# AI-ON/Few-Shot-Music-Generation

Measured on AMD Instinct MI355X. Metric: episodes/s (LSTM-baseline train step, synthetic vocab=10k seq_len=128 5-way/5-shot h=512), higher is better.
Workload: dtype f32 (bf16x3-split products, fp32 accumulate)

## Files before the change

### few-shot-music-generation_amd/csrc/api_backward.hip

```cpp
#include "fsmg_model.h"

using namespace fsmg;
using namespace fsmg_host;

namespace fsmg_host {

int dhout_chunk(fsmg_model* h, const Lane& ln, int B, int t0, int t1, OpBatch* defer = nullptr) {
    ScopedTimer tm(h, "gemm_dhout");
    const int64_t r0 = (int64_t)t0 * B, m = (int64_t)(t1 - t0) * B;
    GemmArgs g{};
    g.A = dlogits_buf(h) + (size_t)r0 * h->V1p; g.lda = h->V1p; g.B = h->P + h->off_w; g.ldb = h->V1p;
    g.C = h->dH + (size_t)r0 * h->Hp; g.ldc = h->Hp; g.M = (int)m; g.N = h->Hp; g.K = h->V1p; g.ksplit = 1;
    if (h->fs_call) g.row_scale = h->crow + r0;
    return gemm(h, ln, OP_KC, OP_KC, g, defer);
}

GemmArgs dw_args(fsmg_model* h, int B) {
    GemmArgs g{};
    g.A = h->Hs[h->L - 1] + (size_t)B * h->Hp; g.lda = h->Hp; g.B = dlogits_buf(h); g.ldb = h->V1p;
    g.C = h->G + h->off_w; g.ldc = h->V1p; g.M = h->Hp; g.N = h->V1p; g.K = (int)((int64_t)h->T * B);
    g.colsum = h->G + h->off_d; g.ksplit = 1;
    if (h->fs_call) { g.A = h->Hsc; g.colsum_w = h->crow; }
    return g;
}
int dw_gemm(fsmg_model* h, const Lane& ln, int B, OpBatch* defer = nullptr) {
    ScopedTimer tm(h, "gemm_dw");
    return gemm(h, ln, OP_XC, OP_XC, dw_args(h, B), defer);
}

int bptt_fills(fsmg_model* h, OpBatch& fills, int B, bool xcd, bool rs, bool chain, int rpx) {
    const int T = h->T, Hp = h->Hp, G4 = h->G4;
    GEMMCK(fills.add(h->dC, 0u, (long long)B * Hp));
    if (xcd) {
        GEMMCK(fills.add(h->inboxX, 0xFFFFFFFFu, lstm_xcd_inbox_floats(B, Hp, rpx), h->d_inbox_dirty));
        GEMMCK(fills.add(h->tickets, 0u, (long long)8 * fsmg_model::TICKET_LAUNCHES));
        h->ticket_next = 0;
    } else if (rs) {
        GEMMCK(fills.add(h->inbox, 0xFFFFFFFFu, lstm_bwd_rs_inbox_floats(B, Hp)));
    } else if (chain) {
        const long long Bp16 = (B + 15) / 16 * 16;
        GEMMCK(fills.add(h->dzF_all, 0xFFFFFFFFu, (long long)T * Bp16 * G4));
    }
    return FSMG_OK;
}

int backward(fsmg_model* h, int B, int part) {
    ScopedRange rng_(part == 2 ? "fsmg.backward(2)" : "fsmg.backward");
    const int T = h->T, Hp = h->Hp, G4 = h->G4;
    const int64_t rows = (int64_t)T * B;
    const Lane mainl = main_lane(h);
    hipStream_t s = h->stream;
    const bool ov = use_overlap(h);
    const bool xcd = use_xcd(h, B, true);
    const bool rs = !xcd && h->persist && h->inbox != nullptr && lstm_bwd_rs_supported(B, Hp) && lstm_bwd_rs_inbox_floats(B, Hp) <= h->inbox_floats;
    const bool chain = xcd || rs || (h->persist && h->dzF_all != nullptr && lstm_bwd_chain_supported(B, Hp) &&
                              (int64_t)T * ((B + 15) / 16 * 16) * G4 <= h->dzfa_floats);
    if (!xcd && h->cs_stale) return fail(h, FSMG_ERR_STATE, "internal: backward pass on the column-split kernels with stale fragment copies of K_h (ensure_cs not called)");
    const int nch = ov ? (chain ? h->nchunk_persist : h->nchunk) : 1;
    const Lane auxl = aux_lane(h, false, chain);
    GemmArgs gdw = dw_args(h, B);
    int dw_split = 1;
    if (h->xov_call && (h->xov_parts & 2) && xcd && !ov) dw_split = std::max(1, std::min(std::min(h->xov_dw_split, MAX_SPLIT), gdw.K / 256));
    while (dw_split > 1 && (int64_t)dw_split * gdw.M * gdw.N > h->slab_cap) --dw_split;
    if (dw_split > 1) {
        gdw.C = mainl.slabs; gdw.c_slab = (int64_t)gdw.M * gdw.N; gdw.ksplit = dw_split;
        gdw.colsum = mainl.colsum_slabs; gdw.colsum_slab = gdw.N;
    }
    const bool xov = h->xov_call && (h->xov_parts & 2) && xcd && !ov && dw_split > 1 && xov_fits(gdw);
    const int rpx = xov ? lstm_xcd16_packed_rows(B, Hp) : 0;
    const bool cut = !ov && !xov;
    if (part == 2 && !cut) return FSMG_OK;
    const bool cut_late = cut && h->dp_split == 2 && part != 0;
    bool dx_sq_done = false, top_fills_done = false;
    const bool defer_ok = part == 0 && (cut || xov);
    if (part != 2) h->arena_off = 0;
    h->last_bwd_xcd = xcd;
    FillBatch fills(h);
    OpBatch late(h);
    OpBatch late2(h);
    OpBatch* const d_now = defer_ok ? &fills : nullptr;
    OpBatch* const d_late = defer_ok ? &late : nullptr;
    const bool aside = h->tail_aside && defer_ok && h->eager_call && h->aux != nullptr && !h->timing && !ov;
    h->side_pending = false;
    if (part != 2) GEMMCK(fills.add(h->G + h->off_emb, 0u, (long long)h->V1 * h->Ep));
    if (ov) GEMMCK(fills.flush());
    if (part == 2) {
    } else if (ov) {
        HIPCK(h, hipEventRecord(h->ev_fork, s));
        HIPCK(h, hipStreamWaitEvent(h->aux, h->ev_fork, 0));
        for (int c = nch - 1; c >= 0; --c) {
            const int t0 = chunk_begin(h, c, nch), t1 = chunk_begin(h, c + 1, nch);
            GEMMCK(dhout_chunk(h, auxl, B, t0, t1));
            HIPCK(h, hipEventRecord(h->ev_chunk[c], h->aux));
        }
        GEMMCK(dw_gemm(h, auxl, B));
        HIPCK(h, hipEventRecord(h->ev_join, h->aux));
        HIPCK(h, hipEventRecord(h->ev_bucket[0], h->aux));
        h->bucket0_recorded = true;
    } else if (xov) {
        GEMMCK(fills.add(h->xov_ctl + fsmg_model::XOV_CTL, 0u, 4 + gemm_items(gdw)));
        GEMMCK(fills.flush());
        GEMMCK(dhout_chunk(h, mainl, B, 0, T, d_now));
        HIPCK(h, hipEventRecord(h->ev_fork, s));
        HIPCK(h, hipStreamWaitEvent(h->aux, h->ev_fork, 0));
        GEMMCK(gemm_restricted(h, h->aux, OP_XC, OP_XC, gdw, xov_first_free(B, Hp), h->xov_ctl + fsmg_model::XOV_CTL));
        HIPCK(h, hipEventRecord(h->ev_join, h->aux));
    } else {
        GEMMCK(dhout_chunk(h, mainl, B, 0, T, d_now));
        if (defer_ok) {
            GEMMCK(bptt_fills(h, fills, B, xcd, rs, chain, 0));
            GEMMCK(fills.flush());
            top_fills_done = true;
        }
        GEMMCK(dw_gemm(h, mainl, B, d_late));
    }
    if (part == 1 && cut && !cut_late) return fills.flush();
    auto tail_kernels = [&](hipStream_t ts) -> int {
        ScopedTimer tm(h, "embed_grad");
        if (ts != s) {
            HIPCK(h, hipEventRecord(h->ev_side_fork, s));
            HIPCK(h, hipStreamWaitEvent(ts, h->ev_side_fork, 0));
            late.s = ts;
        }
        const bool loss_in_batch = late.r.count > 0;
        if (loss_in_batch) GEMMCK(late.mean(h->ce, rows, h->G + h->n_flat + 1));
        GEMMCK(late.flush());
        const int nb = sqnorm_blocks(rows * h->Ep);
        const SumPartialsArgs sp{h->partials, nb, h->G + h->n_flat + 0, h->d_err, loss_in_batch ? nullptr : h->ce, (int)rows, h->G + h->n_flat + 1};
        const bool sum_rides = dx_sq_done && h->dXpart != nullptr && h->tok_first != nullptr;
        HIPCK(h, launch_embed_grad(ts, h->X, (int)rows, h->dXemb, h->Ep, h->G + h->off_emb, h->tok_first, h->tok_count, h->dXpart, sum_rides ? &sp : nullptr));
        h->tok_table_open = false;
        if (!dx_sq_done) HIPCK(h, launch_sqnorm_partials(ts, h->dXemb, rows * h->Ep, h->partials));
        if (!sum_rides) HIPCK(h, launch_sum_partials(ts, sp.partials, sp.n, sp.dst, sp.flag_src, sp.ce, sp.ce_n, sp.loss_out));
        if (ts != s) {
            HIPCK(h, hipEventRecord(h->ev_side, ts));
            late.s = s;
            h->side_pending = true;
        }
        return FSMG_OK;
    };
    GemmArgs pend{};
    bool pend_on = false;
    int* const pend_ctl = h->xov_ctl;
    for (int l = h->L - 1; l >= 0; --l) {
        const bool top = l == h->L - 1;
        if (part == 2 && cut_late && l > 0) continue;
        const bool skip_chain = part == 2 && cut_late;
        if (!skip_chain) {
        if (top && ov) HIPCK(h, hipStreamWaitEvent(s, h->ev_chunk[nch - 1], 0));
        const bool packed = xov && (top || pend_on);
        if (!(top && top_fills_done)) {
            GEMMCK(bptt_fills(h, fills, B, xcd, rs, chain, packed ? rpx : 0));
            GEMMCK(fills.flush());
        }
        for (int c = nch - 1; c >= 0; --c) {
            const int t0 = chunk_begin(h, c, nch), t1 = chunk_begin(h, c + 1, nch);
            if (top && ov) HIPCK(h, hipStreamWaitEvent(s, h->ev_chunk[c], 0));
            ScopedTimer tm(h, "lstm_bwd");
            if (xcd) {
                LstmBwdXcdArgs a{};
                a.rpx = packed ? rpx : 0; a.Hp = Hp; a.bx3 = h->xcd_bx3 ? 1 : 0; a.variant = h->xcd_variant_bwd >= 0 ? h->xcd_variant_bwd : (h->xcd_variant >= 0 ? h->xcd_variant : lstm_xcd_default_variant(B, false, Hp, 0, h->xcd_bx3));
                a.KhXb = h->khx + (size_t)(2 * l + 1) * lstm_xcd_weight_floats((int)Hp, h->xcd_bx3); a.inbox = h->inboxX; a.Z = h->Z[l]; a.Cs = h->Cs[l];
                a.dc = h->dC; a.dH = h->dH; a.tickets = next_tickets(h); a.err_flag = h->d_err; a.B = B; a.T = T; a.t0 = t0; a.t1 = t1; a.spin_limit = h->chain_spin_limit;
                HIPCK(h, launch_lstm_bwd_xcd(s, a));
                ++h->n_xcd_launches;
                continue;
            }
            if (rs) {
                LstmBwdRsArgs a{};
                a.KhF = h->khf + (size_t)(2 * l + 1) * Hp * G4; a.inbox = h->inbox; a.Z = h->Z[l]; a.Cs = h->Cs[l];
                a.dc = h->dC; a.dH = h->dH; a.err_flag = h->d_err; a.B = B; a.Hp = Hp; a.T = T; a.t0 = t0; a.t1 = t1; a.spin_limit = h->chain_spin_limit;
                HIPCK(h, launch_lstm_bwd_rs(s, a));
                ++h->n_persist_launches;
                continue;
            }
            if (chain) {
                LstmBwdChainArgs a{};
                a.KhF = h->khf + (size_t)(2 * l + 1) * Hp * G4; a.dzF_all = h->dzF_all; a.Z = h->Z[l]; a.Cs = h->Cs[l];
                a.dc = h->dC; a.dH = h->dH; a.err_flag = h->d_err; a.B = B; a.Hp = Hp; a.T = T; a.t0 = t0; a.t1 = t1; a.spin_limit = h->chain_spin_limit;
                HIPCK(h, launch_lstm_bwd_chain(s, a));
                ++h->n_persist_launches;
                continue;
            }
            for (int t = t1 - 1; t >= t0; --t) {
                LstmBwdArgs a{};
                const size_t Bp16 = (size_t)(B + 15) / 16 * 16;
                a.KhF = h->khf + (size_t)(2 * l + 1) * Hp * G4;
                a.dzF_next = (t + 1 < T) ? h->dzF + (size_t)((t + 1) & 1) * Bp16 * G4 : nullptr;
                a.dzF_cur = h->dzF + (size_t)(t & 1) * Bp16 * G4;
                a.gates = h->Z[l] + (size_t)t * B * G4;
                a.c_t = h->Cs[l] + (size_t)(t + 1) * B * Hp;
                a.c_prev = h->Cs[l] + (size_t)t * B * Hp;
                a.dc = h->dC;
                a.dh_top = h->dH + (size_t)t * B * Hp;
                a.B = B; a.Hp = Hp;
                HIPCK(h, launch_lstm_bwd_step(s, a));
            }
            h->n_step_launches += t1 - t0;
        }
        if (xov && top) {
            ScopedTimer tm(h, "gemm_dw");
            GEMMCK(gemm_cleanup(h, s, OP_XC, OP_XC, gdw, h->xov_ctl + fsmg_model::XOV_CTL));
            HIPCK(h, hipStreamWaitEvent(s, h->ev_join, 0));
            if (dw_split > 1) {
                const int64_t mn = (int64_t)gdw.M * gdw.N;
                if (d_late) {
                    GEMMCK(late.room(2));
                    GEMMCK(late.reduce(mainl.slabs, mn, dw_split, h->G + h->off_w, mn));
                    GEMMCK(late.reduce(mainl.colsum_slabs, gdw.N, dw_split, h->G + h->off_d, gdw.N));
                    h->slabs_owner = &late;
                } else {
                    HIPCK(h, launch_reduce_slabs(s, mainl.slabs, mn, dw_split, h->G + h->off_w, mn));
                    HIPCK(h, launch_reduce_slabs(s, mainl.colsum_slabs, gdw.N, dw_split, h->G + h->off_d, gdw.N));
                    HIPCK(h, hipEventRecord(h->ev_bucket[0], s));
                    h->bucket0_recorded = true;
                }
            }
        }
        if (pend_on) {
            ScopedTimer tm(h, "gemm_dk");
            GEMMCK(gemm_cleanup(h, s, OP_XC, OP_XC, pend, pend_ctl));
            HIPCK(h, hipStreamWaitEvent(s, h->ev_join, 0));
            pend_on = false;
        }
        }
        if (part == 1 && cut_late && l == 0) return FSMG_OK;
        const int in_p = h->in_dim[l];
        OpBatch* dk_defer = d_late;
        auto dk_gemm = [&](bool* probe, bool* wait_for_chain = nullptr) -> int {
            {
                ScopedTimer tm(h, "gemm_dk");
                GemmArgs m{};
                if (l == 0) { m.A = h->P + h->off_emb; m.lda = h->Ep; m.gather = h->X; }
                else { m.A = h->Hs[l - 1] + (size_t)B * Hp; m.lda = Hp; }
                m.A2 = h->Hs[l]; m.lda2 = Hp; m.m_split = in_p;
                m.B = h->Z[l]; m.ldb = G4; m.C = h->G + h->off_kx[l]; m.ldc = G4; m.M = in_p + Hp; m.N = G4; m.K = (int)rows;
                m.colsum = h->G + h->off_b[l]; m.ksplit = 1;
                const bool merged = h->merge_dk && in_p % 256 == 0 && Hp % 4 == 0 && h->off_kh[l] == h->off_kx[l] + (int64_t)in_p * G4 &&
                                    (l > 0 || 4LL * h->V1 * h->Ep < 0xfffff000LL) && 4LL * Hp * rows < 0xfffff000LL && 4LL * G4 * rows < 0xfffff000LL &&
                                    (((uintptr_t)m.A | (uintptr_t)m.A2 | (uintptr_t)m.B) & 15) == 0 && gemm_dma_enabled() && use_h_gemm(h, OP_XC, OP_XC, m, mainl);
                if (merged && wait_for_chain != nullptr) {
                    GEMMCK(gemm_prepare_queue(h, m, h->xov_dw_split, dk_defer, wait_for_chain));
                    if (*wait_for_chain) { pend = m; return FSMG_OK; }
                }
                if (merged) {
                    if (probe) { *probe = true; return FSMG_OK; }
                    GEMMCK(gemm(h, mainl, OP_XC, OP_XC, m, dk_defer));
                } else {
                GemmArgs g{};
                g.A = h->Hs[l]; g.lda = Hp; g.B = h->Z[l]; g.ldb = G4;
                g.C = h->G + h->off_kh[l]; g.ldc = G4; g.M = Hp; g.N = G4; g.K = (int)rows;
                g.colsum = h->G + h->off_b[l]; g.ksplit = 1;
                if (probe) { *probe = use_h_gemm(h, OP_XC, OP_XC, g, mainl); return FSMG_OK; }
                GEMMCK(gemm(h, mainl, OP_XC, OP_XC, g, dk_defer));
                GemmArgs k{};
                if (l == 0) { k.A = h->P + h->off_emb; k.lda = h->Ep; k.gather = h->X; }
                else { k.A = h->Hs[l - 1] + (size_t)B * Hp; k.lda = Hp; }
                k.B = h->Z[l]; k.ldb = G4; k.C = h->G + h->off_kx[l]; k.ldc = G4;
                k.M = in_p; k.N = G4; k.K = (int)rows; k.ksplit = 1;
                GEMMCK(gemm(h, mainl, OP_XC, OP_XC, k, dk_defer));
                }
            }
            return FSMG_OK;
        };
        auto dx_gemm = [&]() -> int {
            {
                ScopedTimer tm(h, "gemm_dx");
                GemmArgs g{};
                g.A = h->Z[l]; g.lda = G4; g.B = h->P + h->off_kx[l]; g.ldb = G4;
                g.C = (l == 0) ? h->dXemb : h->dH; g.ldc = in_p;
                g.M = (int)rows; g.N = in_p; g.K = G4; g.ksplit = 1;
                if (l == 0) GEMMCK(gemm(h, mainl, OP_KC, OP_KC, g, d_late, h->partials, &dx_sq_done));
                else GEMMCK(gemm(h, mainl, OP_KC, OP_KC, g, d_now));
            }
            return FSMG_OK;
        };
        bool dk_h = false;
        if (aside && l == 0) GEMMCK(dk_gemm(&dk_h));
        if (aside && l == 0 && dk_h) {
            GEMMCK(dk_gemm(nullptr));
            GEMMCK(dx_gemm());
            GEMMCK(tail_kernels(s));
        } else if (aside && l == 0) {
            dk_defer = &late2;
            GEMMCK(dx_gemm());
            GEMMCK(tail_kernels(h->aux));
            GEMMCK(dk_gemm(nullptr));
            HIPCK(h, hipStreamWaitEvent(s, h->ev_side, 0));
            h->side_pending = false;
            GEMMCK(late2.flush());
        } else if (xov && l > 0 && defer_ok && (h->xov_parts & 4) && Hp == 1024) {
            GEMMCK(dk_gemm(nullptr, &pend_on));
            if (pend_on) {
                GEMMCK(fills.add(pend_ctl, 0u, 4 + gemm_items(pend)));
                GEMMCK(fills.flush());
                HIPCK(h, hipEventRecord(h->ev_fork, s));
                HIPCK(h, hipStreamWaitEvent(h->aux, h->ev_fork, 0));
                GEMMCK(gemm_restricted(h, h->aux, OP_XC, OP_XC, pend, xov_first_free(B, Hp), pend_ctl));
                HIPCK(h, hipEventRecord(h->ev_join, h->aux));
            }
            GEMMCK(dx_gemm());
        } else {
            GEMMCK(dk_gemm(nullptr));
            GEMMCK(dx_gemm());
        }
    }
    if (!aside) GEMMCK(tail_kernels(s));
    if (ov) HIPCK(h, hipStreamWaitEvent(s, h->ev_join, 0));
    h->have_grads = true;
    return FSMG_OK;
}

}
```

### few-shot-music-generation_amd/csrc/api_debug.hip

```cpp
#include "fsmg_model.h"

using namespace fsmg;
using namespace fsmg_host;


extern "C" {

int fsmg_debug_clock_begin(fsmg_handle h, int32_t microseconds) {
    if (!h || microseconds <= 0 || microseconds > 1000000) return FSMG_ERR_INVALID;
    BEGIN_CALL(h, true);
    if (!h->probe) HIPCK(h, hipStreamCreateWithFlags(&h->probe, hipStreamNonBlocking));
    if (!h->d_probe) HIPCK(h, hipMalloc((void**)&h->d_probe, 64));
    HIPCK(h, hipMemsetAsync(h->d_probe, 0, 64, h->probe));
    HIPCK(h, launch_clock_probe(h->probe, (long long)microseconds * 100, h->d_probe));
    return FSMG_OK;
}
int fsmg_debug_clock_end(fsmg_handle h, float* ghz) {
    if (!h || !ghz) return FSMG_ERR_INVALID;
    if (!h->probe || !h->d_probe) return fail(h, FSMG_ERR_STATE, "fsmg_debug_clock_end without fsmg_debug_clock_begin");
    BEGIN_CALL(h, true);
    unsigned long long v[2] = {0, 0};
    HIPCK(h, hipStreamSynchronize(h->probe));
    HIPCK(h, hipMemcpy(v, h->d_probe, sizeof(v), hipMemcpyDeviceToHost));
    *ghz = v[1] ? (float)((double)v[0] / (double)v[1] * 0.1) : 0.0f;
    return FSMG_OK;
}

int fsmg_debug_dims(fsmg_handle h, int32_t dims[5]) {
    if (!h || !dims) return FSMG_ERR_INVALID;
    dims[0] = h->Ep; dims[1] = h->Hp; dims[2] = h->V1p; dims[3] = h->lastB; dims[4] = h->T;
    return FSMG_OK;
}

int fsmg_debug_read(fsmg_handle h, const char* what, float* host, int64_t count) {
    if (!h || !what || !host || count <= 0) return FSMG_ERR_INVALID;
    BEGIN_CALL(h);
    const int64_t B = h->lastB, T = h->T, Hp = h->Hp, G4 = h->G4, rows = T * B;
    const float* src = nullptr; int64_t cap = 0;
    auto layer_of = [&](const char* prefix) -> int {
        const size_t n = std::strlen(prefix);
        if (std::strncmp(what, prefix, n) != 0) return -1;
        const int l = std::atoi(what + n);
        return (l >= 0 && l < h->L && std::strlen(what) > n) ? l : -1;
    };
    int l;
    if (!std::strcmp(what, "aux_tries")) { host[0] = (float)h->aux_tries; return FSMG_OK; }
    if (!std::strcmp(what, "fused_softmax")) { host[0] = h->fused_softmax ? 1.0f : 0.0f; if (count > 1) host[1] = h->fs_call ? 1.0f : 0.0f; return FSMG_OK; }
    if (!std::strcmp(what, "xcd_bx3")) { host[0] = h->xcd_bx3 ? 1.0f : 0.0f; return FSMG_OK; }
    if (!std::strcmp(what, "gemm_kinds")) {
        for (int64_t i = 0; i < count && i < 4; ++i) host[i] = (float)h->gemm_kinds[i];
        return FSMG_OK;
    }
    if (!std::strcmp(what, "xov_selfcheck")) {
        const float v[3] = {(float)h->xov_selfcheck_runs, (float)h->xov_passes, (float)h->xov_selfcheck_every};
        for (int64_t i = 0; i < count && i < 3; ++i) host[i] = v[i];
        return FSMG_OK;
    }
    if (!std::strcmp(what, "xcd_partitioned")) {
        host[0] = h->xov ? 1.0f : 0.0f;
        if (count > 1) { const int b = h->lastB > 0 ? h->lastB : 45, rpx = lstm_xcd16_packed_rows(b, h->Hp); host[1] = (h->xov && rpx > 0) ? (float)xov_first_free(b, h->Hp) : 8.0f; }
        if (count > 2) host[2] = h->xov_last ? 1.0f : 0.0f;
        return FSMG_OK;
    }
    if (!std::strcmp(what, "logits")) { src = h->logits; cap = rows * h->V1p; }
    else if (!std::strcmp(what, "dlogits")) { src = dlogits_buf(h); cap = rows * h->V1p; }
    else if (!std::strcmp(what, "lse")) { src = h->lse; cap = rows; }
    else if (!std::strcmp(what, "ce")) { src = h->ce; cap = rows; }
    else if (!std::strcmp(what, "dx")) { src = h->dXemb; cap = rows * h->Ep; }
    else if (!std::strcmp(what, "dh")) { src = h->dH; cap = rows * Hp; }
    else if (!std::strcmp(what, "gnorm")) { src = h->d_gnorm; cap = 1; }
    else if (!std::strcmp(what, "tail")) { src = h->G + h->n_flat; cap = FSMG_GRAD_TAIL; }
    else if ((l = layer_of("gates")) >= 0) { src = h->Z[l]; cap = rows * G4; }
    else if ((l = layer_of("h")) >= 0) { src = h->Hs[l]; cap = (T + 1) * B * Hp; }
    else if ((l = layer_of("c")) >= 0) { src = h->Cs[l]; cap = (T + 1) * B * Hp; }
    else return fail(h, FSMG_ERR_NAME, std::string("unknown debug buffer '") + what + "'");
    if (count > cap) return fail(h, FSMG_ERR_SIZE, "debug read larger than the buffer");
    HIPCK(h, hipStreamSynchronize(h->stream));
    HIPCK(h, hipMemcpy(host, src, sizeof(float) * count, hipMemcpyDeviceToHost));
    return FSMG_OK;
}

int fsmg_debug_step_profile(fsmg_handle h, int32_t which, uint64_t* stamps, int64_t cap, int32_t* n_blocks,
                            int32_t* n_waves) {
    if (!h || !stamps || !n_blocks || !n_waves || h->lastB <= 0 || h->T < 3) return FSMG_ERR_INVALID;
    BEGIN_CALL(h);
    { const int rc_cs = ensure_cs(h); if (rc_cs != FSMG_OK) return rc_cs; }
    const int B = h->lastB, Hp = h->Hp, G4 = h->G4, l = h->L - 1, t = h->T / 2;
    const int nb = which == 0 ? (G4 / 16) * ((B + 15) / 16) : (Hp / 16) * ((B + 15) / 16);
    const int nw = which == 0 ? 4 : 8;
    const int64_t n = (int64_t)nb * nw * 8;
    if (cap < n) return fail(h, FSMG_ERR_SIZE, "stamp buffer too small");
    unsigned long long* d = nullptr;
    HIPCK(h, hipMalloc((void**)&d, sizeof(unsigned long long) * n));
    HIPCK(h, hipMemsetAsync(d, 0, sizeof(unsigned long long) * n, h->stream));
    for (int rep = 0; rep < 3; ++rep) {
        if (which == 0) {
            LstmFwdArgs a{};
            const size_t Bp16 = (size_t)(B + 15) / 16 * 16;
            a.KhF = h->khf + (size_t)(2 * l) * Hp * G4; a.hF_prev = h->HF[l] + (size_t)t * Bp16 * Hp;
            a.hF_next = h->HF[l] + (size_t)(t + 1) * Bp16 * Hp; a.z = h->Z[l] + (size_t)t * B * G4;
            a.c_prev = h->Cs[l] + (size_t)t * B * Hp; a.c_next = h->Cs[l] + (size_t)(t + 1) * B * Hp;
            a.h_next = h->Hs[l] + (size_t)(t + 1) * B * Hp; a.B = B; a.Hp = Hp;
            HIPCK(h, launch_lstm_fwd_step(h->stream, a, d));
        } else {
            LstmBwdArgs a{};
            const size_t Bp16 = (size_t)(B + 15) / 16 * 16;
            a.KhF = h->khf + (size_t)(2 * l + 1) * Hp * G4; a.dzF_next = h->dzF + (size_t)((t + 1) & 1) * Bp16 * G4;
            a.dzF_cur = h->dzF + (size_t)(t & 1) * Bp16 * G4; a.gates = h->Z[l] + (size_t)t * B * G4;
            a.c_t = h->Cs[l] + (size_t)(t + 1) * B * Hp; a.c_prev = h->Cs[l] + (size_t)t * B * Hp; a.dc = h->dC;
            a.dh_top = h->dH + (size_t)t * B * Hp; a.B = B; a.Hp = Hp;
            HIPCK(h, launch_lstm_bwd_step(h->stream, a, d));
        }
    }
    HIPCK(h, hipStreamSynchronize(h->stream));
    HIPCK(h, hipMemcpy(stamps, d, sizeof(unsigned long long) * n, hipMemcpyDeviceToHost));
    hipFree(d);
    *n_blocks = nb; *n_waves = nw;
    return FSMG_OK;
}

int fsmg_timing_enable(fsmg_handle h, int32_t on) {
    if (!h) return FSMG_ERR_INVALID;
    BEGIN_CALL(h);
    drain_timers(h);
    h->timing = on != 0;
    return FSMG_OK;
}
int fsmg_timing_select(fsmg_handle h, const char* kernel_class) {
    if (!h) return FSMG_ERR_INVALID;
    BEGIN_CALL(h);
// ... 23 lines not shown
```

### few-shot-music-generation_amd/csrc/api_forward.hip

```cpp
#include "fsmg_model.h"

using namespace fsmg;
using namespace fsmg_host;

namespace fsmg_host {

int stage_tokens(fsmg_model* h, const int32_t* support, int n_sup, const int32_t* query, int n_qry, int on_device) {
    const size_t T = h->T;
    if (on_device && h->eager_call) {
        h->cur_sup = support; h->cur_qry = query;
        return FSMG_OK;
    }
    const hipMemcpyKind kind = on_device ? hipMemcpyDeviceToDevice : hipMemcpyHostToDevice;
    if (n_sup > 0) HIPCK(h, hipMemcpyAsync(h->d_tok, support, sizeof(int) * n_sup * T, kind, h->stream));
    if (n_qry > 0) HIPCK(h, hipMemcpyAsync(h->d_tok + n_sup * T, query, sizeof(int) * n_qry * T, kind, h->stream));
    h->cur_sup = h->d_tok; h->cur_qry = h->d_tok + n_sup * T;
    return FSMG_OK;
}

int reset_tok_table(fsmg_model* h) {
    if (!h->tok_first) return FSMG_OK;
    OpBatch ops(h);
    GEMMCK(ops.add(h->tok_first, 0x7FFFFFFFu, h->V1));
    GEMMCK(ops.add(h->tok_count, 0u, h->V1));
    return ops.flush();
}

int token_prep(fsmg_model* h, int n_sup, int n_qry, bool train) {
    const bool table = train && h->tok_first != nullptr;
    HIPCK(h, launch_token_prep(h->stream, h->cur_sup, n_sup, h->cur_qry, n_qry, h->T, h->V, h->V,
                               h->X, h->Y, h->d_err, table ? h->tok_first : nullptr, table ? h->tok_count : nullptr));
    return FSMG_OK;
}

GemmArgs logits_args(fsmg_model* h, int B, int t0, int t1) {
    const int Hp = h->Hp;
    const int64_t r0 = (int64_t)t0 * B, m = (int64_t)(t1 - t0) * B;
    GemmArgs g{};
    g.A = h->Hs[h->L - 1] + (size_t)B * Hp + (size_t)r0 * Hp; g.lda = Hp;
    g.B = h->P + h->off_w; g.ldb = h->V1p;
    g.C = h->logits + (size_t)r0 * h->V1p; g.ldc = h->V1p; g.M = (int)m; g.N = h->V1p; g.K = Hp;
    g.bias = h->P + h->off_d; g.ksplit = 1; g.nt_store = 1;
    return g;
}
inline void fused_softmax_args(fsmg_model* h, GemmArgs& g) {
    g.ce_part = h->ce_part; g.ce_nvocab = h->V1; g.ce_store = 1;
}
int ce_finish(fsmg_model* h, hipStream_t s, int B, int64_t rows) {
    ScopedTimer tm(h, "ce");
    HIPCK(h, launch_ce_finish(s, h->ce_part, h->ce_nparts, h->Y, (int)rows, (float)(1.0 / ((double)rows + 1e-12)), h->logits, h->V1p,
                              h->lse, h->ce, h->crow, h->Hs[h->L - 1] + (size_t)B * h->Hp, h->Hsc, h->Hp, h->d_err, h->d_counters + 4));
    return FSMG_OK;
}
int ce_rows(fsmg_model* h, hipStream_t s, int B, int t0, int t1, int64_t rows_total) {
    ScopedTimer tm(h, "ce");
    const int64_t r0 = (int64_t)t0 * B, m = (int64_t)(t1 - t0) * B;
    HIPCK(h, launch_ce_rows(s, h->logits + (size_t)r0 * h->V1p, h->V1p, (int)m, h->V1, h->Y + r0, h->lse + r0,
                            h->ce + r0, dlogits_buf(h) + (size_t)r0 * h->V1p, (float)(1.0 / ((double)rows_total + 1e-12))));
    return FSMG_OK;
}

int logits_and_ce(fsmg_model* h, const Lane& ln, int B, int t0, int t1, int64_t rows_total, bool want_dlogits) {
    const int64_t r0 = (int64_t)t0 * B, m = (int64_t)(t1 - t0) * B;
    GemmArgs g = logits_args(h, B, t0, t1);
    if (!want_dlogits) {
        ScopedTimer tm(h, "gemm_logits");
        g.ce_part = h->ce_part + (size_t)r0 * h->ce_nparts; g.ce_tgt = h->Y + r0; g.ce_tgt_logit = h->tgt_logit + r0;
        g.ce_nvocab = h->V1; g.bx3 = h->bx3;
        if (use_h_gemm(h, OP_KC, OP_XC, g, ln)) g.bx3 = 3;
        else if (use_ws_gemm(h, OP_KC, OP_XC, g, ln)) { g.bx3 = 2; g.group_m = 4; }
        HIPCK(h, launch_gemm(h, ln.s, OP_KC, OP_XC, g, ln.lds_pad));
        HIPCK(h, launch_ce_combine(ln.s, h->ce_part + (size_t)r0 * h->ce_nparts, h->ce_nparts,
                                   h->tgt_logit + r0, (int)m, h->ce + r0));
        return FSMG_OK;
    }
    {
        ScopedTimer tm(h, "gemm_logits");
        GEMMCK(gemm(h, ln, OP_KC, OP_XC, g));
    }
    return ce_rows(h, ln.s, B, t0, t1, rows_total);
}

int xov_selfcheck(fsmg_model* h, int B) {
    --h->xov_selfcheck_left;
    ++h->xov_selfcheck_runs;
    const int64_t rows = (int64_t)h->T * B;
    if (!h->xov_selfcheck_fault) {
        GemmArgs g = logits_args(h, B, 0, h->T);
        if (h->fs_call) fused_softmax_args(h, g);
        g.C = h->dlogits; g.bx3 = 3; g.ksplit = 1;
        HIPCK(h, launch_gemm(h, h->stream, OP_KC, OP_XC, g, 0));
    }
    HIPCK(h, launch_compare_words(h->stream, h->logits, h->dlogits, rows * h->V1p, h->d_err, h->d_counters + 3));
    return FSMG_OK;
}

int forward(fsmg_model* h, int B, int rows_per_group, int ngroups, float* loss_out, bool want_dlogits, int head) {
    ScopedRange rng_(want_dlogits ? "fsmg.forward(train)" : head == HEAD_LOGITS ? "fsmg.forward(score)" : head == HEAD_NONE ? "fsmg.forward(cache)" : "fsmg.forward(eval)");
    const int T = h->T, Hp = h->Hp, G4 = h->G4;
    const int64_t rows = (int64_t)T * B;
    const Lane mainl = main_lane(h);
    hipStream_t s = h->stream;
    const bool ov = head == HEAD_LOSS && use_overlap(h);
    const bool xcd = use_xcd(h, B);
    const bool chain1 = !xcd && h->persist && !h->force_fwd_rt && lstm_fwd_chain_supported(B, Hp);
    const bool chain_rt = !xcd && h->persist && !chain1 && lstm_fwd_chain_rt_supported(B, Hp);
    const bool chain = chain1 || chain_rt;
    if (!xcd && h->cs_stale) return fail(h, FSMG_ERR_STATE, "internal: forward pass on the column-split kernels with stale fragment copies of K_h (ensure_cs not called)");
    const int nch_ov = ov ? ((chain || xcd) ? h->nchunk_persist : h->nchunk) : 1;
    GemmArgs ghead = logits_args(h, B, 0, T);
    h->fs_call = false;
    if (want_dlogits && h->fused_softmax && !ov && h->bx3 && h->inplace_dlogits && h->Hsc != nullptr && mainl.lds_pad == 0) {
        h->fs_call = true;
        h->fs_call = use_h_gemm(h, OP_XC, OP_XC, dw_args(h, B), mainl);
    }
    if (h->fs_call) fused_softmax_args(h, ghead);
    const bool xov = h->xov_call && (h->xov_parts & 1) && xcd && want_dlogits && !ov && xov_fits(ghead);
    const int xfree = xov_first_free(B, Hp);
    const int rpx = xov ? lstm_xcd16_packed_rows(B, Hp) : 0;
    if (xov) xov_gate(h, ghead, B);
    for (int l = 0; l < h->L; ++l) {
        const size_t Bp16 = (size_t)(B + 15) / 16 * 16;
        const bool top = l == h->L - 1;
        FillBatch fills(h);
        GEMMCK(fills.add(h->Hs[l], 0u, (long long)B * Hp));
        GEMMCK(fills.add(h->Cs[l], 0u, (long long)B * Hp));
        if (!xcd) GEMMCK(fills.add(h->HF[l], 0u, (long long)Bp16 * Hp));
        {
            ScopedTimer tm(h, "gemm_zx");
            GemmArgs g{};
            if (l == 0) { g.A = h->P + h->off_emb; g.lda = h->Ep; g.gather = h->X; g.K = h->Ep; }
            else { g.A = h->Hs[l - 1] + (size_t)B * Hp; g.lda = Hp; g.K = Hp; }
            g.B = h->P + h->off_kx[l]; g.ldb = G4;
            g.C = h->Z[l]; g.ldc = G4; g.M = (int)rows; g.N = G4;
            g.bias = h->P + h->off_b[l]; g.ksplit = 1;
            GEMMCK(gemm(h, mainl, OP_KC, OP_XC, g));
        }
        auto chain_fills = [&]() -> int {
            if (chain)
                GEMMCK(fills.add(h->HF[l] + Bp16 * Hp, 0xFFFFFFFFu, (long long)T * Bp16 * Hp));
            if (xcd) {
                GEMMCK(fills.add(h->tickets, 0u, (long long)8 * fsmg_model::TICKET_LAUNCHES));
                h->ticket_next = 0;
                const long long step_f = lstm_xcd_hx_floats(B, 0, Hp, h->xcd_bx3, xov && top ? rpx : 0);
                GEMMCK(fills.add(h->HX, 0u, step_f));
                GEMMCK(fills.add(h->HX + step_f, 0xFFFFFFFFu, step_f * T));
                if (xov && top) {
                    GEMMCK(fills.add(h->xov_ctl, 0u, 4 + gemm_items(ghead)));
                    GEMMCK(fills.add(h->xov_prog, 0u, T));
                }
            }
            return fills.flush();
        };
        GEMMCK(chain_fills());
        if (l == 0) GEMMCK(settle_pending(h));
        if (xov && top) {
            HIPCK(h, hipEventRecord(h->ev_fork, s));
            HIPCK(h, hipStreamWaitEvent(h->aux, h->ev_fork, 0));
            GEMMCK(gemm_restricted(h, h->aux, OP_KC, OP_XC, ghead, xfree, h->xov_ctl));
            HIPCK(h, hipEventRecord(h->ev_join, h->aux));
        }
        const int nch = nch_ov;
        for (int c = 0; c < nch; ++c) {
            const int t0 = chunk_begin(h, c, nch);
            const int t1 = chunk_begin(h, c + 1, nch);
            if (xcd) {
                ScopedTimer tm(h, "lstm_fwd");
                LstmFwdXcdArgs a{};
                a.rpx = (xov && top) ? rpx : 0; a.progress = (xov && top) ? h->xov_prog : nullptr; a.Hp = Hp;
                a.progress_every = h->xov_pub; a.bx3 = h->xcd_bx3 ? 1 : 0;
                a.variant = h->xcd_variant >= 0 ? h->xcd_variant : lstm_xcd_default_variant(B, true, Hp, a.rpx, h->xcd_bx3);
                a.KhX = h->khx + (size_t)(2 * l) * lstm_xcd_weight_floats((int)Hp, h->xcd_bx3); a.HX = h->HX; a.Z = h->Z[l]; a.Cs = h->Cs[l]; a.Hs = h->Hs[l];
                a.tickets = next_tickets(h); a.err_flag = h->d_err; a.B = B; a.T = T; a.t0 = t0; a.t1 = t1; a.spin_limit = h->chain_spin_limit;
                HIPCK(h, launch_lstm_fwd_xcd(s, a));
                ++h->n_xcd_launches;
            } else if (chain) {
                ScopedTimer tm(h, "lstm_fwd");
                LstmFwdChainArgs a{};
                a.KhF = h->khf + (size_t)(2 * l) * Hp * G4; a.HF = h->HF[l]; a.Z = h->Z[l]; a.Cs = h->Cs[l]; a.Hs = h->Hs[l];
                a.err_flag = h->d_err; a.B = B; a.Hp = Hp; a.T = T; a.t0 = t0; a.t1 = t1; a.spin_limit = h->chain_spin_limit;
                HIPCK(h, chain_rt ? launch_lstm_fwd_chain_rt(s, a) : launch_lstm_fwd_chain(s, a));
                ++h->n_persist_launches;
            } else {
                ScopedTimer tm(h, "lstm_fwd");
                for (int t = t0; t < t1; ++t) {
                    LstmFwdArgs a{};
                    a.KhF = h->khf + (size_t)(2 * l) * Hp * G4;
                    a.hF_prev = h->HF[l] + (size_t)t * Bp16 * Hp;
                    a.hF_next = h->HF[l] + (size_t)(t + 1) * Bp16 * Hp;
                    a.z = h->Z[l] + (size_t)t * B * G4;
                    a.c_prev = h->Cs[l] + (size_t)t * B * Hp;
                    a.c_next = h->Cs[l] + (size_t)(t + 1) * B * Hp;
                    a.h_next = h->Hs[l] + (size_t)(t + 1) * B * Hp;
                    a.B = B; a.Hp = Hp;
                    HIPCK(h, launch_lstm_fwd_step(s, a));
                }
                h->n_step_launches += t1 - t0;
            }
            if (top && ov) {
                HIPCK(h, hipEventRecord(h->ev_chunk[c], s));
                HIPCK(h, hipStreamWaitEvent(h->aux, h->ev_chunk[c], 0));
                GEMMCK(logits_and_ce(h, aux_lane(h, !want_dlogits, chain || xcd), B, t0, t1, rows, want_dlogits));
            }
        }
    }
    if (head == HEAD_NONE) {
    } else if (head == HEAD_LOGITS) {
        ScopedTimer tm(h, "gemm_logits");
        ghead.bx3 = h->bx3;
        if (use_h_gemm(h, OP_KC, OP_XC, ghead, mainl)) ghead.bx3 = 3;
        else if (use_ws_gemm(h, OP_KC, OP_XC, ghead, mainl)) { ghead.bx3 = 2; ghead.group_m = 4; }
        HIPCK(h, launch_gemm(h, s, OP_KC, OP_XC, ghead, 0));
    } else if (ov) {
        HIPCK(h, hipEventRecord(h->ev_join, h->aux));
        HIPCK(h, hipStreamWaitEvent(s, h->ev_join, 0));
    } else if (xov) {
        {
            ScopedTimer tm(h, "gemm_logits");
            GEMMCK(gemm_cleanup(h, s, OP_KC, OP_XC, ghead, h->xov_ctl));
            HIPCK(h, hipStreamWaitEvent(s, h->ev_join, 0));
        }
        ++h->xov_passes;
        if (h->xov_selfcheck_every > 0 && h->xov_selfcheck_left <= 0 && h->xov_passes % h->xov_selfcheck_every == 0) h->xov_selfcheck_left = 1;
        if (h->xov_selfcheck_left > 0) GEMMCK(xov_selfcheck(h, B));
        if (h->fs_call) GEMMCK(ce_finish(h, s, B, rows));
        else GEMMCK(ce_rows(h, s, B, 0, T, rows));
    } else if (h->fs_call) {
        {
            ScopedTimer tm(h, "gemm_logits");
            ghead.bx3 = h->bx3;
            if (use_h_gemm(h, OP_KC, OP_XC, ghead, mainl)) ghead.bx3 = 3;
            else if (use_ws_gemm(h, OP_KC, OP_XC, ghead, mainl)) { ghead.bx3 = 2; ghead.group_m = 4; }
            HIPCK(h, launch_gemm(h, s, OP_KC, OP_XC, ghead, 0));
        }
        GEMMCK(ce_finish(h, s, B, rows));
    } else {
        GEMMCK(logits_and_ce(h, mainl, B, 0, T, rows, want_dlogits));
// ... 11 lines not shown
```

### few-shot-music-generation_amd/csrc/api_handle.hip

```cpp
#include <mutex>
#include "fsmg_model.h"

using namespace fsmg;
using namespace fsmg_host;

namespace fsmg_host {

thread_local std::string g_create_error;

static int pick_concurrent_aux(fsmg_model* h, int priority, int max_tries) {
    if (max_tries <= 0) {
        if (hipStreamCreateWithPriority(&h->aux, hipStreamNonBlocking, priority) != hipSuccess) return fail(h, FSMG_ERR_HIP, "aux stream create failed");
        h->aux_tries = 0;
        return FSMG_OK;
    }
    int* d = nullptr;
    if (hipMalloc((void**)&d, 256) != hipSuccess) return fail(h, FSMG_ERR_NOMEM, "hipMalloc(queue probe) failed");
    auto probe = [&](hipStream_t cand, long long ticks) -> int {
        int seen = 0;
        const int init[2] = {0, -1};
        if (hipStreamSynchronize(h->stream) != hipSuccess || hipMemcpy(d, init, sizeof(init), hipMemcpyHostToDevice) != hipSuccess ||
            launch_queue_probe(h->stream, d, d + 1, 0, ticks) != hipSuccess || launch_queue_probe(cand, d, d + 1, 1, 0) != hipSuccess ||
            hipStreamSynchronize(cand) != hipSuccess || hipStreamSynchronize(h->stream) != hipSuccess ||
            hipMemcpy(&seen, d + 1, sizeof(int), hipMemcpyDeviceToHost) != hipSuccess) return -1;
// ... 51 lines not shown
        if (h->aux != nullptr) {
            HIPCK(h, hipStreamWaitEvent(h->aux, last->ev_turn, 0));
            HIPCK(h, hipStreamWaitEvent(h->aux, last->ev_turn_aux, 0));
        }
    }
    last = h;
    return FSMG_OK;
}
static void forget_turn(fsmg_model* h) {
    std::lock_guard<std::mutex> lk(turn_mutex());
    if (g_turn_last[h->device & 15] == h) g_turn_last[h->device & 15] = nullptr;
}

int begin_call(fsmg_model* h, bool keep_pending) {
    HIPCK(h, hipSetDevice(h->device));
    const int rc = take_turn(h);
    if (rc != FSMG_OK) return rc;
    return keep_pending ? FSMG_OK : settle_pending(h);
}

}

extern "C" {

int fsmg_version(void) { return FSMG_VERSION; }

const char* fsmg_last_error(fsmg_handle h) { return h ? h->err.c_str() : g_create_error.c_str(); }

int fsmg_create(const fsmg_config* cfg, fsmg_handle* out) {
    if (!cfg || !out) return fail(nullptr, FSMG_ERR_INVALID, "null config/out");
    *out = nullptr;
    if (cfg->config_version != FSMG_CONFIG_VERSION)
        return fail(nullptr, FSMG_ERR_INVALID, "fsmg_config.config_version is " + std::to_string(cfg->config_version) + ", this library expects " +
                                                   std::to_string(FSMG_CONFIG_VERSION) + " (caller built against another include/fsmg.h)");
    if (cfg->gemm < 0 || cfg->gemm > FSMG_GEMM_F32 || cfg->schedule < 0 || cfg->schedule > FSMG_SCHEDULE_XCD_PARTITIONED ||
        cfg->recurrence < 0 || cfg->recurrence > FSMG_RECURRENCE_XCD_LOCAL)
        return fail(nullptr, FSMG_ERR_INVALID, "fsmg_config.gemm / schedule / recurrence out of range");
    if (cfg->input_size <= 0 || cfg->max_len <= 0 || cfg->embedding_size <= 0 || cfg->hidden_size <= 0 ||
        cfg->n_layers <= 0 || cfg->n_layers > 16 || cfg->embedding_size > 1024 || !(cfg->n_decay > 0.f) ||
        !(cfg->max_grad_norm > 0.f))
        return fail(nullptr, FSMG_ERR_INVALID, "config out of range (sizes must be > 0, embedding_size <= 1024, n_layers <= 16)");
    int ndev = 0;
    if (hipGetDeviceCount(&ndev) != hipSuccess || ndev <= 0)
        return fail(nullptr, FSMG_ERR_NO_DEVICE, "no HIP device visible: libfsmg has no CPU fallback");
    if (cfg->device < 0 || cfg->device >= ndev) return fail(nullptr, FSMG_ERR_NO_DEVICE, "device ordinal out of range");
    hipDeviceProp_t prop;
    if (hipSetDevice(cfg->device) != hipSuccess || hipGetDeviceProperties(&prop, cfg->device) != hipSuccess)
        return fail(nullptr, FSMG_ERR_NO_DEVICE, "cannot select HIP device");
    if (std::strncmp(prop.gcnArchName, "gfx950", 6) != 0)
        return fail(nullptr, FSMG_ERR_NO_DEVICE, std::string("libfsmg is built for gfx950 only, device is ") + prop.gcnArchName);

    fsmg_model* h = new (std::nothrow) fsmg_model();
    if (!h) return fail(nullptr, FSMG_ERR_NOMEM, "host allocation failed");
    h->cfg = *cfg;
    h->device = cfg->device;
    compute_dims(*cfg, h);
    h->n_flat = build_layout(h);
    auto bail = [&](int code, const std::string& msg) { g_create_error = msg; fsmg_destroy(h); return code; };

    if (cfg->stream) { h->stream = (hipStream_t)cfg->stream; h->own_stream = false; }
    else {
        if (hipStreamCreateWithFlags(&h->stream, hipStreamNonBlocking) != hipSuccess) return bail(FSMG_ERR_HIP, "hipStreamCreate failed");
        h->own_stream = true;
    }
    {
        if (const char* eg = std::getenv("FSMG_GRAPH")) h->cfg.use_graph = (eg[0] != '0');
        h->overlap = (int64_t)h->V1 >= 8LL * h->H * h->L;
        if (cfg->schedule == FSMG_SCHEDULE_SINGLE_STREAM) { h->overlap = false; h->overlap_forced = true; }
        if (cfg->schedule == FSMG_SCHEDULE_TWO_STREAM) { h->overlap = true; h->overlap_forced = true; }
        if (cfg->schedule == FSMG_SCHEDULE_XCD_PARTITIONED) h->xov = true;
        if (cfg->gemm == FSMG_GEMM_F32) h->bx3 = 0;
        if (cfg->recurrence == FSMG_RECURRENCE_PER_STEP) h->persist = false;
        if (cfg->recurrence == FSMG_RECURRENCE_COLUMN_SPLIT) h->xcd = false;
        if (cfg->recurrence == FSMG_RECURRENCE_XCD_LOCAL) h->pair_mode = 2;
        if (cfg->dp_split_backward) h->dp_split = cfg->dp_split_backward == 2 ? 2 : 1;
        const char* env = std::getenv("FSMG_OVERLAP");
        if (env) { h->overlap = env[0] != '0'; h->overlap_forced = true; }
        if (const char* e = std::getenv("FSMG_GEMM")) h->bx3 = std::strcmp(e, "f32") != 0;
        if (const char* e = std::getenv("FSMG_GEMM_H")) h->gemm_h = std::atoi(e);
        if (const char* e = std::getenv("FSMG_GEMM_WS")) h->gemm_ws = std::atoi(e);
        if (const char* e = std::getenv("FSMG_MAX_SPLIT")) h->max_split = std::max(1, std::atoi(e));
        if (const char* e = std::getenv("FSMG_XCD_OVERLAP")) h->xov = std::atoi(e) != 0;
        if (const char* e = std::getenv("FSMG_XOV_PARTS")) h->xov_parts = std::max(1, std::min(7, std::atoi(e)));
        if (const char* e = std::getenv("FSMG_EAGER")) h->eager = (e[0] != '0');
        if (const char* e = std::getenv("FSMG_MERGE_DK")) h->merge_dk = (e[0] != '0');
        if (const char* e = std::getenv("FSMG_UPD_SPLIT")) h->upd_split = (e[0] != '0');
        if (const char* e = std::getenv("FSMG_TAIL_ASIDE")) h->tail_aside = (e[0] != '0');
        if (const char* e = std::getenv("FSMG_LAZY_CS")) h->lazy_cs = (e[0] != '0');
        if (const char* e = std::getenv("FSMG_FUSED_SOFTMAX")) h->fused_softmax = (e[0] != '0');

        if (const char* e = std::getenv("FSMG_INPLACE_DLOGITS")) h->inplace_dlogits = (e[0] != '0');
        if (const char* e = std::getenv("FSMG_XOV_SELFCHECK")) h->xov_selfcheck_left = std::max(0, std::atoi(e));
        if (const char* e = std::getenv("FSMG_XOV_SELFCHECK_EVERY")) h->xov_selfcheck_every = std::max(0, std::atoi(e));
        if (const char* e = std::getenv("FSMG_PERSISTENT")) h->persist = (e[0] != '0');
        h->persist_cfg = h->persist;
        if (const char* e = std::getenv("FSMG_FALLBACK_STEPS")) h->fallback_steps = std::max(1, std::atoi(e));
        if (const char* e = std::getenv("FSMG_XCD")) h->xcd = (e[0] != '0');
        if (const char* e = std::getenv("FSMG_XCD_PAIR")) h->pair_mode = std::max(0, std::min(2, std::atoi(e)));
        if (const char* e = std::getenv("FSMG_FWD_RT")) h->force_fwd_rt = (e[0] != '0');
        if (const char* e = std::getenv("FSMG_CHAIN_SPIN_LIMIT")) h->chain_spin_limit = std::max(0, std::atoi(e));
        if (const char* e = std::getenv("FSMG_XCD_VARIANT")) h->xcd_variant = std::atoi(e);
        if (const char* e = std::getenv("FSMG_XCD_VARIANT_BWD")) h->xcd_variant_bwd = std::atoi(e);
        if (hipEventCreateWithFlags(&h->ev_turn, hipEventDisableTiming) != hipSuccess ||
            hipEventCreateWithFlags(&h->ev_turn_aux, hipEventDisableTiming) != hipSuccess) return bail(FSMG_ERR_HIP, "event create failed");
        if (turnstile_on()) {
            std::lock_guard<std::mutex> lk(turn_mutex());
            fsmg_model* last = g_turn_last[h->device & 15];
            if (last != nullptr && last->stream != nullptr && !last->capturing.load()) { (void)hipStreamSynchronize(last->stream); if (last->aux) (void)hipStreamSynchronize(last->aux); }
        }
        {
            static const int tries = std::getenv("FSMG_AUX_TRIES") ? std::max(0, std::min(32, std::atoi(std::getenv("FSMG_AUX_TRIES")))) : 8;
            if (pick_concurrent_aux(h, 0, tries) != FSMG_OK) { std::string e = h->err; return bail(FSMG_ERR_HIP, e); }
            if (h->aux_tries < 0) {
                fprintf(stderr, "[fsmg] no second stream of this process runs beside the handle's stream (%d candidates, probed for 300 us and again for 5 ms: "
                                "they share its hardware queue -- GPU_MAX_HW_QUEUES? -- or the device was busy with another process): serial order, no overlapped "
                                "tails for this handle (fsmg_stats.aux_stream_tries = -1; fsmg_debug_set(\"reprobe_aux\", 1) asks again)\n", tries);
                h->overlap = false; h->overlap_forced = true; h->tail_aside = false; h->upd_split = false;
            }
        }
        for (int c = 0; c < fsmg_model::NCHUNK; ++c)
            if (hipEventCreateWithFlags(&h->ev_chunk[c], hipEventDisableTiming) != hipSuccess) return bail(FSMG_ERR_HIP, "event create failed");
        if (hipEventCreateWithFlags(&h->ev_bucket[0], hipEventDisableTiming) != hipSuccess ||
            hipEventCreateWithFlags(&h->ev_bucket[1], hipEventDisableTiming) != hipSuccess ||
            hipEventCreateWithFlags(&h->ev_fork, hipEventDisableTiming) != hipSuccess ||
            hipEventCreateWithFlags(&h->ev_upd_fork, hipEventDisableTiming) != hipSuccess ||
            hipEventCreateWithFlags(&h->ev_upd, hipEventDisableTiming) != hipSuccess ||
            hipEventCreateWithFlags(&h->ev_side_fork, hipEventDisableTiming) != hipSuccess ||
            hipEventCreateWithFlags(&h->ev_side, hipEventDisableTiming) != hipSuccess ||

            hipEventCreateWithFlags(&h->ev_join, hipEventDisableTiming) != hipSuccess) return bail(FSMG_ERR_HIP, "event create failed");
    }
    const int64_t sb = state_bytes_for(h->n_flat);
    if (cfg->state_arena) {
        if (cfg->state_arena_bytes < (uint64_t)sb || ((uintptr_t)cfg->state_arena & 255u))
            return bail(FSMG_ERR_INVALID, "state_arena too small or not 256-byte aligned");
        h->state = (char*)cfg->state_arena; h->own_state = false;
    } else {
        if (hipMalloc((void**)&h->state, sb) != hipSuccess) return bail(FSMG_ERR_NOMEM, "hipMalloc(state) failed");
        h->own_state = true;
    }
    h->P = (float*)h->state; h->G = h->P + h->n_flat;
    h->M = h->G + h->n_flat + FSMG_GRAD_TAIL; h->Vv = h->M + h->n_flat;
    if (hipMemsetAsync(h->state, 0, sb, h->stream) != hipSuccess) return bail(FSMG_ERR_HIP, "memset(state) failed");

    char* small = nullptr;
    const size_t tok_words = (size_t)round_up(h->V1, 64);
    const size_t prog_words = (size_t)round_up(h->T + 8, 64);
    const size_t small_bytes = 256 * 4 + sizeof(float) * RING_CAP + sizeof(int) * 8 * fsmg_model::TICKET_LAUNCHES + sizeof(int) * 2 * fsmg_model::XOV_CTL +
                               sizeof(int) * 2 * tok_words + sizeof(int) * prog_words;
    if (hipMalloc((void**)&small, small_bytes) != hipSuccess) return bail(FSMG_ERR_NOMEM, "hipMalloc(scalars) failed");
    hipMemsetAsync(small, 0, small_bytes, h->stream);
    h->d_step = (long long*)small; h->d_err = (int*)(small + 256); h->d_gnorm = (float*)(small + 512);
    h->d_inbox_dirty = (int*)(small + 768);
    h->d_decided = (float*)(small + 896);
    { static const int one = 1; hipStreamSynchronize(h->stream); hipMemcpy(h->d_inbox_dirty, &one, sizeof(int), hipMemcpyHostToDevice); }
    h->d_ring = (float*)(small + 1024);
    if (hipHostMalloc((void**)&h->host_counters, 64, hipHostMallocMapped) != hipSuccess ||
        hipHostGetDevicePointer((void**)&h->d_counters, h->host_counters, 0) != hipSuccess)
        return bail(FSMG_ERR_NOMEM, "hipHostMalloc(mapped step counters) failed");
    std::memset(h->host_counters, 0, 64);
    h->tickets = (int*)(small + 1024 + sizeof(float) * RING_CAP);
    h->xov_ctl = h->tickets + 8 * fsmg_model::TICKET_LAUNCHES;
    h->tok_first = h->xov_ctl + 2 * fsmg_model::XOV_CTL; h->tok_count = h->tok_first + tok_words;
    h->xov_prog = h->tok_count + tok_words;
    if (reset_tok_table(h) != FSMG_OK) return bail(FSMG_ERR_HIP, "fill of the token occurrence table failed");

// ... 58 lines not shown
    if (h->ev_side_fork) hipEventDestroy(h->ev_side_fork);
    if (h->ev_side) hipEventDestroy(h->ev_side);
    if (h->ev_turn) hipEventDestroy(h->ev_turn);
    if (h->ev_turn_aux) hipEventDestroy(h->ev_turn_aux);
    comm_destroy(h);
    if (h->probe) { hipStreamSynchronize(h->probe); hipStreamDestroy(h->probe); }
    if (h->d_probe) hipFree(h->d_probe);
    if (h->aux) hipStreamDestroy(h->aux);
    if (h->own_stream && h->stream) hipStreamDestroy(h->stream);
    delete h;
    return FSMG_OK;
}

int fsmg_synchronize(fsmg_handle h) {
    if (!h) return FSMG_ERR_INVALID;
    BEGIN_CALL(h);
    HIPCK(h, hipStreamSynchronize(h->stream));
    return FSMG_OK;
}

int fsmg_read_losses(fsmg_handle h, float* out, int32_t n) {
    if (!h || !out || n <= 0 || n > RING_CAP) return FSMG_ERR_INVALID;
    BEGIN_CALL(h);
    std::vector<float> ring(RING_CAP);
    long long step = 0;
    HIPCK(h, hipStreamSynchronize(h->stream));
    HIPCK(h, hipMemcpy(ring.data(), h->d_ring, sizeof(float) * RING_CAP, hipMemcpyDeviceToHost));
    HIPCK(h, hipMemcpy(&step, h->d_step, sizeof(step), hipMemcpyDeviceToHost));
    poll_skipped(h);
    if (step < n) return fail(h, FSMG_ERR_INVALID, "fewer train steps than requested losses");
    for (int i = 0; i < n; ++i) out[i] = ring[(step - n + i) % RING_CAP];
    return FSMG_OK;
}

int fsmg_get_stats(fsmg_handle h, fsmg_stats* out) {
    if (!h || !out) return FSMG_ERR_INVALID;
    BEGIN_CALL(h);
    HIPCK(h, hipStreamSynchronize(h->stream));
    poll_skipped(h);
    std::memset(out, 0, sizeof(*out));
    out->timeouts = h->n_timeouts;
    out->steps_skipped_timeout = h->host_counters ? h->host_counters[0] : 0;
    out->steps_skipped_token_range = h->host_counters ? h->host_counters[1] : 0;
    out->steps_skipped_peer_failure = h->host_counters ? h->host_counters[2] : 0;
    out->xov_selfcheck_mismatches = h->host_counters ? h->host_counters[3] : 0;
    out->softmax_range_rows = h->host_counters ? h->host_counters[4] : 0;
    out->steps_skipped_softmax_range = h->host_counters ? h->host_counters[5] : 0;
    out->aux_stream_tries = h->aux_tries; out->reserved0 = 0;
    out->xcd_launches = h->n_xcd_launches;
    out->persistent_launches = h->n_persist_launches;
    out->step_launches = h->n_step_launches;
    out->persistent_path = h->persist ? 1 : 0;
    out->fallback_steps_left = h->fallback_left;
    return FSMG_OK;
}

int fsmg_debug_set(fsmg_handle h, const char* what, int64_t value) {
    if (!h || !what) return FSMG_ERR_INVALID;
    BEGIN_CALL(h);
    HIPCK(h, hipStreamSynchronize(h->stream));
    if (h->aux) HIPCK(h, hipStreamSynchronize(h->aux));
    if (!std::strcmp(what, "chain_spin_limit")) h->chain_spin_limit = (int)std::max<int64_t>(0, std::min<int64_t>(value, 1 << 30));
    else if (!std::strcmp(what, "fallback_steps")) h->fallback_steps = (int)std::max<int64_t>(1, std::min<int64_t>(value, 1 << 30));
    else if (!std::strcmp(what, "eager")) h->eager = value != 0;
    else if (!std::strcmp(what, "persistent")) { h->persist = h->persist_cfg = value != 0; h->fallback_left = 0; }
    else if (!std::strcmp(what, "inplace_dlogits")) h->inplace_dlogits = value != 0;
    else if (!std::strcmp(what, "upd_split")) h->upd_split = value != 0;
    else if (!std::strcmp(what, "reprobe_aux")) {
        if (value != 0 && h->aux_tries < 0) {
            HIPCK(h, hipStreamSynchronize(h->stream));
            if (h->aux) HIPCK(h, hipStreamSynchronize(h->aux));
            hipStream_t old = h->aux; h->aux = nullptr;
            const int rc = pick_concurrent_aux(h, 0, 8);
            if (rc != FSMG_OK) { if (h->aux == nullptr) h->aux = old; return rc; }
            if (old) hipStreamDestroy(old);
            if (h->aux_tries > 0) {
                h->overlap = true; h->overlap_forced = false; h->tail_aside = true;
                if (h->xov_eligible && h->xcd_bx3) h->xov = true;
                drop_graphs(h);
            }
        }
    }
    else if (!std::strcmp(what, "tail_aside")) h->tail_aside = value != 0;
    else if (!std::strcmp(what, "fused_softmax")) h->fused_softmax = value != 0;

    else if (!std::strcmp(what, "xov_selfcheck")) h->xov_selfcheck_left = (int)std::max<int64_t>(0, std::min<int64_t>(value, 1 << 30));
    else if (!std::strcmp(what, "xov_selfcheck_fault")) h->xov_selfcheck_fault = value != 0;
    else if (!std::strcmp(what, "xov_selfcheck_every")) h->xov_selfcheck_every = (int)std::max<int64_t>(0, std::min<int64_t>(value, 1 << 30));
    else return fail(h, FSMG_ERR_NAME, std::string("unknown knob '") + what + "'");
    drop_graphs(h);
    return FSMG_OK;
}

}
```

### few-shot-music-generation_amd/csrc/api_step.hip

```cpp
#include "fsmg_model.h"

using namespace fsmg;
using namespace fsmg_host;

namespace fsmg_host {

int validate_shape(fsmg_model* h, int N, int K, int Q) {
    if (N <= 0 || K < 0 || Q < 0 || (int64_t)N * (K + Q) <= 0 || (int64_t)N * (K + Q) > (1 << 20))
        return fail(h, FSMG_ERR_INVALID, "bad episode shape N/K/Q");
    return FSMG_OK;
}

template <class Stage>
int forward_backward_core(fsmg_model* h, int32_t N, int32_t K, int32_t Q, Stage&& stage, bool with_update = false) {
    int rc = validate_shape(h, N, K, Q);
    if (rc != FSMG_OK) return rc;
    const int B = N * (K + Q);
    if (h->fallback_left > 0 && --h->fallback_left == 0 && h->persist != h->persist_cfg) {
        h->persist = h->persist_cfg;
        drop_graphs(h);
    }
    if ((rc = ensure_scratch(h, B)) != FSMG_OK) return rc;
    if ((rc = select_xcd_format(h, B)) != FSMG_OK) return rc;
    choose_schedule(h, B, true);
    h->xov_last = h->xov_call;
    if (!h->eager_call && (rc = settle_pending(h)) != FSMG_OK) return rc;
    if ((rc = ensure_khf(h)) != FSMG_OK) return rc;
    if (pass_reads_cs(h, B, true) && (rc = ensure_cs(h)) != FSMG_OK) return rc;
    if (h->tok_table_open && (rc = reset_tok_table(h)) != FSMG_OK) return rc;
    h->tok_table_open = true;
    if ((rc = stage()) != FSMG_OK) return rc;
    const int n_sup = N * K, n_qry = N * Q;
    h->bucket0_recorded = false;
    const std::string shape_key = std::to_string(n_sup) + ":" + std::to_string(n_qry);
    if (h->dp_split && !with_update) {
        rc = run_graphed(h, "fb1:" + shape_key, [&]() -> int {
            int r = token_prep(h, n_sup, n_qry, true);
            if (r == FSMG_OK) r = forward(h, B, B, 1, h->G + h->n_flat + 1, true);
            if (r == FSMG_OK) r = backward(h, B, 1);
            return r;
        });
        if (rc != FSMG_OK) return rc;
        if (!h->bucket0_recorded) { HIPCK(h, hipEventRecord(h->ev_bucket[0], h->stream)); h->bucket0_recorded = true; }
        rc = run_graphed(h, "fb2:" + shape_key, [&]() -> int { return backward(h, B, 2); });
    } else {
        rc = run_graphed(h, (with_update ? "fbu:" : "fb:") + shape_key, [&]() -> int {
            int r = token_prep(h, n_sup, n_qry, true);
            if (r == FSMG_OK) r = forward(h, B, B, 1, h->G + h->n_flat + 1, true);
            if (r == FSMG_OK) r = backward(h, B);
            if (r == FSMG_OK && with_update) r = apply_update(h, 1.0f);
            return r;
        });
    }
    if (rc != FSMG_OK) return rc;
    h->tok_table_open = false;
    if (!with_update) {
        if (!h->bucket0_recorded) HIPCK(h, hipEventRecord(h->ev_bucket[0], h->stream));
        HIPCK(h, hipEventRecord(h->ev_bucket[1], h->stream));
    }
    h->lastB = B;
    h->have_grads = !with_update;
    return FSMG_OK;
}

template <class FB>
int dp_train_step(fsmg_model* h, float* loss, FB&& forward_backward) {
    for (int attempt = 0; attempt < 2; ++attempt) {
        int rc = forward_backward();
        int local_rc = FSMG_OK; std::string local_msg;
        if (rc != FSMG_OK) {
            local_rc = rc; local_msg = h->err;
            if (launch_fill32(h->stream, h->G + h->n_flat + 4, 0x3f800000u, 1) != hipSuccess) return local_rc;
            if (hipEventRecord(h->ev_bucket[0], h->stream) != hipSuccess || hipEventRecord(h->ev_bucket[1], h->stream) != hipSuccess) return local_rc;
            h->have_grads = true;
        }
        rc = exchange_gradients(h);
        const float scale = 1.0f / (float)h->world;
        if (rc == FSMG_OK) {
            uint32_t bits; std::memcpy(&bits, &scale, 4);
            rc = run_graphed(h, "up:" + std::to_string(bits) + (h->last_bwd_xcd ? "x" : "s"), [&]() -> int { return apply_update(h, scale); });
        }
        if (rc == FSMG_OK) rc = after_update(h, scale, loss);
        if (local_rc != FSMG_OK) { h->err = local_msg; return local_rc; }
        if (is_retry(rc) && h->retry_armed && attempt == 0) { h->retry_armed = false; continue; }
        return rc;
    }
    return FSMG_OK;
}

template <class Stage>
int fused_train_step(fsmg_model* h, int32_t N, int32_t K, int32_t Q, float* loss, Stage&& stage) {
    if (h->comm != nullptr) return dp_train_step(h, loss, [&]() { return forward_backward_core(h, N, K, Q, stage, false); });
    int rc = forward_backward_core(h, N, K, Q, stage, true);
    if (rc == FSMG_OK) rc = after_update(h, 1.0f, loss);
    if (is_retry(rc) && h->retry_armed) {
        h->retry_armed = false;
        rc = forward_backward_core(h, N, K, Q, stage, true);
        if (rc == FSMG_OK) rc = after_update(h, 1.0f, loss);
    }
    return rc;
}

}

extern "C" {

int fsmg_forward_backward(fsmg_handle h, const int32_t* support, const int32_t* query, int32_t N, int32_t K,
                          int32_t Q, int32_t tokens_on_device) {
    if (!h || !support || !query) return FSMG_ERR_INVALID;
    BEGIN_CALL(h, true);
    return forward_backward_core(h, N, K, Q, [&]() { return stage_tokens(h, support, N * K, query, N * Q, tokens_on_device); });
}

// ... 265 lines not shown
```

### few-shot-music-generation_amd/csrc/api_update.hip

```cpp
#include "fsmg_model.h"

using namespace fsmg;
using namespace fsmg_host;

namespace fsmg_host {

int repack_recurrent_weights(fsmg_model* h, hipStream_t s);
int ensure_khf(fsmg_model* h) {
    if (!h->khf_dirty) return FSMG_OK;
    const int rc = repack_recurrent_weights(h, h->stream);
    if (rc != FSMG_OK) return rc;
    h->khf_dirty = false;
    return FSMG_OK;
}

int repack_recurrent_weights(fsmg_model* h, hipStream_t s, const StepIncArgs* inc, bool* inc_done) {
    if (inc_done) *inc_done = false;
    const bool x_ok = h->khx == nullptr || h->Hp == 512 || h->Hp == 1024 || h->Hp == 256;
    if (h->L <= REPACK_MAX_LAYERS && x_ok) {
        RepackAllArgs a{};
        a.n = h->L; a.Hp = h->Hp; a.bx3 = h->xcd_bx3 ? 1 : 0;
        const bool captured = inc != nullptr && h->cfg.use_graph && !(h->timing || h->ov_call || h->xov_call || h->eager_call);
        const bool lazy = h->lazy_cs && h->khx != nullptr && h->persist && h->xcd && !captured;
        a.mode = lazy ? 1 : 0;
        h->cs_stale = lazy;
        for (int l = 0; l < h->L; ++l) {
            a.Kh[l] = h->P + h->off_kh[l];
            a.cf[l] = h->khf + (size_t)(2 * l) * h->Hp * h->G4; a.cb[l] = h->khf + (size_t)(2 * l + 1) * h->Hp * h->G4;
            a.xf[l] = h->khx ? h->khx + (size_t)(2 * l) * lstm_xcd_weight_floats((int)h->Hp, h->xcd_bx3) : nullptr;
            a.xb[l] = h->khx ? h->khx + (size_t)(2 * l + 1) * lstm_xcd_weight_floats((int)h->Hp, h->xcd_bx3) : nullptr;
        }
        HIPCK(h, launch_repack_kh_all(s, a, inc));
        if (inc_done) *inc_done = inc != nullptr;
        return FSMG_OK;
    }
    h->cs_stale = false;
    for (int l = 0; l < h->L; ++l) {
        HIPCK(h, launch_repack_kh(s, h->P + h->off_kh[l], h->khf + (size_t)(2 * l) * h->Hp * h->G4,
                                  h->khf + (size_t)(2 * l + 1) * h->Hp * h->G4, h->Hp));
        if (h->khx) HIPCK(h, launch_repack_kh_xcd(s, h->P + h->off_kh[l], h->khx + (size_t)(2 * l) * lstm_xcd_weight_floats((int)h->Hp, h->xcd_bx3),
                                                  h->khx + (size_t)(2 * l + 1) * lstm_xcd_weight_floats((int)h->Hp, h->xcd_bx3), h->Hp, h->xcd_bx3));
    }
    return FSMG_OK;
}
int repack_recurrent_weights(fsmg_model* h, hipStream_t s) { return repack_recurrent_weights(h, s, nullptr, nullptr); }

int ensure_cs(fsmg_model* h) {
    if (!h->cs_stale) return FSMG_OK;
    RepackAllArgs a{};
    a.n = h->L; a.Hp = h->Hp; a.bx3 = h->xcd_bx3 ? 1 : 0; a.mode = 2;
    for (int l = 0; l < h->L; ++l) {
        a.Kh[l] = h->P + h->off_kh[l];
        a.cf[l] = h->khf + (size_t)(2 * l) * h->Hp * h->G4; a.cb[l] = h->khf + (size_t)(2 * l + 1) * h->Hp * h->G4;
    }
    HIPCK(h, launch_repack_kh_all(h->stream, a, nullptr));
    h->cs_stale = false;
    return FSMG_OK;
}

int apply_update(fsmg_model* h, float grad_scale) {
    ScopedRange rng_("fsmg.clip+adam");
    hipStream_t s = h->stream;
    ScopedTimer tm(h, "update");
    const bool slices = h->cfg.clip_norm_mode == FSMG_CLIP_TF1_SLICES;
    const int64_t skip = slices ? round_up((int64_t)h->V1 * h->Ep, FLAT_ALIGN) : 0;
    const int64_t n = h->n_flat - skip;
    const int nb = sqnorm_blocks(n);
    HIPCK(h, launch_sqnorm_partials(s, h->G + skip, n, h->partials));
    UpdateArgs a{};
    a.p = h->P; a.m = h->M; a.v = h->Vv; a.g = h->G; a.n = h->n_flat;
    a.partials = h->partials; a.n_partials = nb; a.tail = h->G + h->n_flat; a.use_slices = slices ? 1 : 0;
    a.grad_scale = grad_scale; a.lr = h->cfg.lr; a.n_decay = h->cfg.n_decay; a.clip = h->cfg.max_grad_norm;
    a.step = h->d_step; a.gnorm_out = h->d_gnorm; a.err_flag = h->d_err;
    const bool split = h->upd_split && h->eager_call && h->aux != nullptr && !h->timing && h->off_w > 0 && h->off_w < h->n_flat;
    if (split) {
        GEMMCK(settle_pending(h));
        a.n = h->off_w; a.publish = h->d_decided;
        HIPCK(h, launch_adam_update(s, a));
        HIPCK(h, hipEventRecord(h->ev_upd_fork, s));
        HIPCK(h, hipStreamWaitEvent(h->aux, h->ev_upd_fork, 0));
        UpdateArgs b = a;
        b.p = h->P + h->off_w; b.m = h->M + h->off_w; b.v = h->Vv + h->off_w; b.g = h->G + h->off_w; b.n = h->n_flat - h->off_w;
        b.publish = nullptr; b.consume = h->d_decided; b.gnorm_out = nullptr;
        HIPCK(h, launch_adam_update(h->aux, b));
        HIPCK(h, hipEventRecord(h->ev_upd, h->aux));
        h->upd_pending = true;
    } else {
        HIPCK(h, launch_adam_update(s, a));
    }
    StepIncArgs inc{};
    inc.step = h->d_step; inc.loss_src = h->G + h->n_flat + 1; inc.loss_scale = grad_scale; inc.ring = h->d_ring; inc.ring_cap = RING_CAP;
    inc.err_flag = h->d_err; inc.counters = h->d_counters; inc.handoff_dirty = h->d_inbox_dirty; inc.clear_ok = h->last_bwd_xcd ? 1 : 0;
    bool inc_done = false;
    GEMMCK(repack_recurrent_weights(h, s, &inc, &inc_done));
    if (!inc_done) HIPCK(h, launch_step_increment(s, inc));
    h->have_grads = false;
    return FSMG_OK;
}

int sgd_update(fsmg_model* h, float lr) {
    hipStream_t s = h->stream;
    ScopedTimer tm(h, "update");
    const bool slices = h->cfg.clip_norm_mode == FSMG_CLIP_TF1_SLICES;
    const int64_t skip = slices ? round_up((int64_t)h->V1 * h->Ep, FLAT_ALIGN) : 0;
    const int64_t n = h->n_flat - skip;
    HIPCK(h, launch_sqnorm_partials(s, h->G + skip, n, h->partials));
    UpdateArgs a{};
    a.p = h->P; a.g = h->G; a.n = h->n_flat;
    a.partials = h->partials; a.n_partials = sqnorm_blocks(n); a.tail = h->G + h->n_flat; a.use_slices = slices ? 1 : 0;
    a.lr = lr; a.clip = h->cfg.max_grad_norm; a.gnorm_out = h->d_gnorm; a.err_flag = h->d_err;
    HIPCK(h, launch_sgd_update(s, a));
    h->khf_dirty = true;
    h->have_grads = false;
    return ensure_khf(h);
}

int save_theta(fsmg_model* h) {
    if (!h->P_saved) {
        HIPCK(h, hipStreamSynchronize(h->stream));
        if (hipMalloc((void**)&h->P_saved, sizeof(float) * (size_t)h->n_flat) != hipSuccess)
            return fail(h, FSMG_ERR_NOMEM, "hipMalloc(saved parameters) failed");
    }
    HIPCK(h, launch_copy_words(h->stream, h->P_saved, h->P, h->n_flat));
    return FSMG_OK;
}
int restore_theta(fsmg_model* h) {
    HIPCK(h, launch_copy_words(h->stream, h->P, h->P_saved, h->n_flat));
    h->khf_dirty = true;
    return ensure_khf(h);
}

void on_timeout(fsmg_model* h) {
    ++h->n_timeouts;
    h->retry_armed = true;
    if (h->persist) {
        h->persist = false;
        hipStreamSynchronize(h->stream);
        if (h->aux) hipStreamSynchronize(h->aux);
        drop_graphs(h);
    }
    h->fallback_left = h->fallback_steps;
    if (h->host_counters && h->host_counters[3] != h->seen_selfcheck_mismatch) {
        h->seen_selfcheck_mismatch = h->host_counters[3];
        if (h->xov) {
            h->xov = false;
            fprintf(stderr, "[fsmg] XCD-partitioned order: %lld 16-byte words of the gated projection differed from the serial recomputation "
                            "(stale operand rows in an XCD's L2?): the step is repeated, serial order from here on\n", (long long)h->host_counters[3]);
        }
    }
    if (h->xov_last && ++h->xov_strikes >= 2 && h->xov) {
        h->xov = false;
        fprintf(stderr, "[fsmg] the XCD-partitioned order timed out twice on this handle (its two launches are not running side by side?): serial order from here on\n");
    }
    if (h->d_inbox_dirty) {
// ... 71 lines not shown
```

### few-shot-music-generation_amd/csrc/elementwise.hip

```cpp
#include <algorithm>
#include "fsmg_kernels.h"
#include <cstdlib>

namespace fsmg {
namespace {

__device__ __forceinline__ float wave_sum(float v) {
#pragma unroll
    for (int o = 32; o > 0; o >>= 1) v += __shfl_xor(v, o, 64);
    return v;
}
__device__ __forceinline__ double wave_sum_d(double v) {
#pragma unroll
    for (int o = 32; o > 0; o >>= 1) v += __shfl_xor(v, o, 64);
    return v;
}
__device__ __forceinline__ float wave_max(float v) {
#pragma unroll
    for (int o = 32; o > 0; o >>= 1) v = fmaxf(v, __shfl_xor(v, o, 64));
    return v;
}

__global__ __launch_bounds__(256) void k_fill32(uint32_t* __restrict__ p, uint32_t word, long long n) {
    const long long n4 = n >> 2;
    const uint4 w4 = make_uint4(word, word, word, word);
    for (long long i = (long long)blockIdx.x * 256 + threadIdx.x; i < n4; i += (long long)gridDim.x * 256)
        reinterpret_cast<uint4*>(p)[i] = w4;
    if (blockIdx.x == 0 && threadIdx.x < (n & 3)) p[(n4 << 2) + threadIdx.x] = word;
}

__global__ __launch_bounds__(256) void k_fill32_if(const int* __restrict__ cond, uint32_t* __restrict__ p, uint32_t word, long long n) {
    if (*cond == 0) return;
    const long long n4 = n >> 2;
    const uint4 w4 = make_uint4(word, word, word, word);
    for (long long i = (long long)blockIdx.x * 256 + threadIdx.x; i < n4; i += (long long)gridDim.x * 256)
        reinterpret_cast<uint4*>(p)[i] = w4;
    if (blockIdx.x == 0 && threadIdx.x < (n & 3)) p[(n4 << 2) + threadIdx.x] = word;
}

constexpr int SQ_CHUNK = 256 * 16;
__global__ __launch_bounds__(256) void k_multi_op(const MultiOps r) {
    const MultiOp& o = r.op[blockIdx.y];
    if (o.kind == MULTI_FILL) {
        if (o.cond != nullptr && *o.cond == 0) return;
        uint32_t* p = (uint32_t*)o.dst;
        const uint32_t word = o.word;
        const long long n = o.n, n4 = n >> 2;
        const uint4 w4 = make_uint4(word, word, word, word);
        for (long long i = (long long)blockIdx.x * 256 + threadIdx.x; i < n4; i += (long long)gridDim.x * 256)
            reinterpret_cast<uint4*>(p)[i] = w4;
        if (blockIdx.x == 0 && threadIdx.x < (n & 3)) p[(n4 << 2) + threadIdx.x] = word;
        return;
    }
    __shared__ double sh[4];
    if (o.kind == MULTI_MEAN) {
        if (blockIdx.x != 0) return;
        const int tid = threadIdx.x, lane = tid & 63, wave = tid >> 6;
        const float* x = (const float*)o.src;
        const int n = (int)o.n;
        double l = 0.0;
        for (int i0 = tid; i0 < n; i0 += 256 * 16) {
            float b[16];
#pragma unroll
            for (int k = 0; k < 16; ++k) b[k] = (i0 + 256 * k < n) ? x[i0 + 256 * k] : 0.0f;
#pragma unroll
            for (int k = 0; k < 16; ++k) if (i0 + 256 * k < n) l += (double)b[k];
        }
        l = wave_sum_d(l);
        if (lane == 0) sh[wave] = l;
        __syncthreads();
        if (tid == 0) *(float*)o.dst = (float)(((sh[0] + sh[1]) + (sh[2] + sh[3])) / ((double)n + 1e-12));
        return;
    }
    const int tid = threadIdx.x, lane = tid & 63, wave = tid >> 6;
    const float* sl = (const float*)o.src;
    float* out = (float*)o.dst;
    const long long n = o.n, nchunks = (n + SQ_CHUNK - 1) / SQ_CHUNK;
    const bool vec = (o.stride & 3) == 0 && (n & 3) == 0;
    if (o.sq == nullptr && vec) {
        const long long n4 = n >> 2;
        for (long long i = (long long)blockIdx.x * 256 + tid; i < n4; i += (long long)gridDim.x * 256) {
            float4 v = *reinterpret_cast<const float4*>(sl + 4 * i);
            int z = 1;
            for (; z + 3 < o.nslab; z += 4) {
                const float4 w0 = *reinterpret_cast<const float4*>(sl + z * o.stride + 4 * i);
                const float4 w1 = *reinterpret_cast<const float4*>(sl + (z + 1) * o.stride + 4 * i);
                const float4 w2 = *reinterpret_cast<const float4*>(sl + (z + 2) * o.stride + 4 * i);
                const float4 w3 = *reinterpret_cast<const float4*>(sl + (z + 3) * o.stride + 4 * i);
                v.x += w0.x; v.y += w0.y; v.z += w0.z; v.w += w0.w;
                v.x += w1.x; v.y += w1.y; v.z += w1.z; v.w += w1.w;
                v.x += w2.x; v.y += w2.y; v.z += w2.z; v.w += w2.w;
                v.x += w3.x; v.y += w3.y; v.z += w3.z; v.w += w3.w;
            }
            for (; z < o.nslab; ++z) {
                const float4 w = *reinterpret_cast<const float4*>(sl + z * o.stride + 4 * i);
                v.x += w.x; v.y += w.y; v.z += w.z; v.w += w.w;
            }
            if (o.row_scale != nullptr) {
                const float c = o.row_scale[(4 * i) / o.row_len];
                v.x *= c; v.y *= c; v.z *= c; v.w *= c;
            }
            *reinterpret_cast<float4*>(out + 4 * i) = v;
        }
        return;
    }
    for (long long c = blockIdx.x; c < nchunks; c += gridDim.x) {
        const long long base = c * SQ_CHUNK;
        double s = 0.0;
        if (vec && base + SQ_CHUNK <= n) {
            float4 v[4];
#pragma unroll
            for (int i = 0; i < 4; ++i) v[i] = *reinterpret_cast<const float4*>(sl + base + 4 * (tid + 256 * i));
            int z = 1;
            for (; z + 1 < o.nslab; z += 2) {
                float4 w0[4], w1[4];
#pragma unroll
                for (int i = 0; i < 4; ++i) {
                    w0[i] = *reinterpret_cast<const float4*>(sl + z * o.stride + base + 4 * (tid + 256 * i));
                    w1[i] = *reinterpret_cast<const float4*>(sl + (z + 1) * o.stride + base + 4 * (tid + 256 * i));
                }
#pragma unroll
                for (int i = 0; i < 4; ++i) {
                    v[i].x += w0[i].x; v[i].y += w0[i].y; v[i].z += w0[i].z; v[i].w += w0[i].w;
                    v[i].x += w1[i].x; v[i].y += w1[i].y; v[i].z += w1[i].z; v[i].w += w1[i].w;
                }
            }
            if (z < o.nslab) {
#pragma unroll
                for (int i = 0; i < 4; ++i) {
                    const float4 w = *reinterpret_cast<const float4*>(sl + z * o.stride + base + 4 * (tid + 256 * i));
                    v[i].x += w.x; v[i].y += w.y; v[i].z += w.z; v[i].w += w.w;
                }
            }
#pragma unroll
            for (int i = 0; i < 4; ++i) {
                *reinterpret_cast<float4*>(out + base + 4 * (tid + 256 * i)) = v[i];
                s += ((double)v[i].x * v[i].x + (double)v[i].y * v[i].y) + ((double)v[i].z * v[i].z + (double)v[i].w * v[i].w);
            }
        } else {
#pragma unroll
            for (int i = 0; i < 4; ++i) {
                const long long idx = base + 4 * (tid + 256 * i);
                float q[4] = {0.f, 0.f, 0.f, 0.f};
                int k = 0;
                for (long long j = idx; j < n && j < idx + 4; ++j, ++k) {
                    float v = sl[j];
                    for (int z = 1; z < o.nslab; ++z) v += sl[z * o.stride + j];
                    out[j] = v;
                    q[k] = v;
                }
                if (k == 4) s += ((double)q[0] * q[0] + (double)q[1] * q[1]) + ((double)q[2] * q[2] + (double)q[3] * q[3]);
                else for (int e = 0; e < k; ++e) s += (double)q[e] * q[e];
            }
        }
        if (o.sq != nullptr) {
            s = wave_sum_d(s);
            if (lane == 0) sh[wave] = s;
            __syncthreads();
            if (tid == 0) o.sq[c] = (sh[0] + sh[1]) + (sh[2] + sh[3]);
            __syncthreads();
        }
    }
}

__global__ void k_token_prep(const int* __restrict__ support, int n_support, const int* __restrict__ query,
                             int n_query, int T, int vocab, int start_word, int* __restrict__ X,
                             int* __restrict__ Y, int* __restrict__ err_flag, int* __restrict__ tok_first, int* __restrict__ tok_count) {
    __shared__ int s_key[512], s_cnt[512], s_min[512];
    const int B = n_support + n_query;
    const long long total = (long long)B * T;
    for (long long i0 = (long long)blockIdx.x * blockDim.x; i0 < total; i0 += (long long)gridDim.x * blockDim.x) {
        const long long i = i0 + threadIdx.x;
        const bool valid = i < total;
        const int b = valid ? (int)(i / T) : 0, t = valid ? (int)(i % T) : 0;
        int tok = 0;
        if (valid) {
            const int* row = (b < n_support) ? support + (long long)b * T : query + (long long)(b - n_support) * T;
            tok = row[t];
            if (tok < 0 || tok >= vocab) {
                atomicOr(err_flag, 1);
                tok = min(max(tok, 0), vocab - 1);
            }
            Y[(long long)t * B + b] = tok;
            if (t + 1 < T) X[(long long)(t + 1) * B + b] = tok;
            if (t == 0) X[b] = start_word;
        }
        if (tok_first != nullptr) {
            for (int j = threadIdx.x; j < 512; j += blockDim.x) { s_key[j] = -1; s_cnt[j] = 0; s_min[j] = 0x7FFFFFFF; }
            __syncthreads();
            if (valid && t + 1 < T) {
                const int pos = (int)((long long)(t + 1) * B + b);
                unsigned slot = ((unsigned)tok * 2654435761u) >> 23;
                bool placed = false;
#pragma unroll 1
                for (int probe = 0; probe < 8 && !placed; ++probe) {
                    const int prev = atomicCAS(&s_key[slot], -1, tok);
                    if (prev == -1 || prev == tok) { atomicAdd(&s_cnt[slot], 1); atomicMin(&s_min[slot], pos); placed = true; }
                    else slot = (slot + 1) & 511u;
                }
                if (!placed) { atomicMin(tok_first + tok, pos); atomicAdd(tok_count + tok, 1); }
            }
            __syncthreads();
            for (int j = threadIdx.x; j < 512; j += blockDim.x)
                if (s_key[j] >= 0) { atomicMin(tok_first + s_key[j], s_min[j]); atomicAdd(tok_count + s_key[j], s_cnt[j]); }
            __syncthreads();
            if (valid && t == 0) { atomicMin(tok_first + start_word, b); atomicAdd(tok_count + start_word, 1); }
        }
    }
}

__global__ void k_gather_rows(const int* __restrict__ table, const int* __restrict__ idx, int n_rows, int T, int n_songs,
                              int* __restrict__ out, int* __restrict__ err_flag) {
    const long long total = (long long)n_rows * T;
    for (long long i = (long long)blockIdx.x * blockDim.x + threadIdx.x; i < total; i += (long long)gridDim.x * blockDim.x) {
        const int r = (int)(i / T), t = (int)(i % T);
        int song = idx[r];
        if (song < 0 || song >= n_songs) { atomicOr(err_flag, 1); song = 0; }
        out[i] = table[(long long)song * T + t];
    }
}

__global__ __launch_bounds__(256) void k_ce_rows(const float* logits, int ld, int n_vocab,
                                                 const int* __restrict__ tgt, float* __restrict__ lse,
                                                 float* __restrict__ ce, float* dlogits, float inv_n) {
    __shared__ float sh[4];
    __shared__ float s_lse;
    const int r = blockIdx.x, tid = threadIdx.x, lane = tid & 63, wave = tid >> 6;
    const float* row = logits + (long long)r * ld;
    const int nv4 = n_vocab & ~3;
    float m = -INFINITY;
    for (int v = 4 * tid; v < nv4; v += 1024) {
        const float4 x = *reinterpret_cast<const float4*>(row + v);
        m = fmaxf(fmaxf(m, fmaxf(x.x, x.y)), fmaxf(x.z, x.w));
    }
    if (tid < n_vocab - nv4) m = fmaxf(m, row[nv4 + tid]);
    m = wave_max(m);
    if (lane == 0) sh[wave] = m;
    __syncthreads();
    m = fmaxf(fmaxf(sh[0], sh[1]), fmaxf(sh[2], sh[3]));
    __syncthreads();
    float s = 0.0f;
    for (int v = 4 * tid; v < nv4; v += 1024) {
        const float4 x = *reinterpret_cast<const float4*>(row + v);
        s += (expf(x.x - m) + expf(x.y - m)) + (expf(x.z - m) + expf(x.w - m));
    }
    if (tid < n_vocab - nv4) s += expf(row[nv4 + tid] - m);
    s = wave_sum(s);
    if (lane == 0) sh[wave] = s;
    __syncthreads();
    const int t = tgt[r];
    if (tid == 0) {
        const float l = m + logf((sh[0] + sh[1]) + (sh[2] + sh[3]));
        lse[r] = l;
        ce[r] = l - row[t];
        s_lse = l;
    }
    if (dlogits == nullptr) return;
    __syncthreads();
    const float l = s_lse;
    float* drow = dlogits + (long long)r * ld;
    for (int v = 4 * tid; v < ld; v += 1024) {
        const float4 x = *reinterpret_cast<const float4*>(row + v);
        float4 d;
        d.x = (v + 0 < n_vocab) ? (expf(x.x - l) - (v + 0 == t ? 1.0f : 0.0f)) * inv_n : 0.0f;
        d.y = (v + 1 < n_vocab) ? (expf(x.y - l) - (v + 1 == t ? 1.0f : 0.0f)) * inv_n : 0.0f;
        d.z = (v + 2 < n_vocab) ? (expf(x.z - l) - (v + 2 == t ? 1.0f : 0.0f)) * inv_n : 0.0f;
        d.w = (v + 3 < n_vocab) ? (expf(x.w - l) - (v + 3 == t ? 1.0f : 0.0f)) * inv_n : 0.0f;
        __builtin_nontemporal_store(d.x, drow + v); __builtin_nontemporal_store(d.y, drow + v + 1);
        __builtin_nontemporal_store(d.z, drow + v + 2); __builtin_nontemporal_store(d.w, drow + v + 3);
    }
}

template <int NV, bool NT>
__device__ __forceinline__ void ce_row_reg(float* sh, const int r, const float* logits, int ld, int n_vocab, const int* __restrict__ tgt,
                                           float* __restrict__ lse, float* __restrict__ ce, float* dlogits, float inv_n) {
    const int tid = threadIdx.x, lane = tid & 63, wave = tid >> 6;
    const float* row = logits + (long long)r * ld;
    float4 x[NV];
    float m = -INFINITY;
#pragma unroll
    for (int i = 0; i < NV; ++i) {
        const int v = 4 * tid + 1024 * i;
        x[i] = make_float4(-INFINITY, -INFINITY, -INFINITY, -INFINITY);
        if (v < ld) {
            const float4 q = *reinterpret_cast<const float4*>(row + v);
            x[i].x = (v + 0 < n_vocab) ? q.x : -INFINITY; x[i].y = (v + 1 < n_vocab) ? q.y : -INFINITY;
            x[i].z = (v + 2 < n_vocab) ? q.z : -INFINITY; x[i].w = (v + 3 < n_vocab) ? q.w : -INFINITY;
        }
        m = fmaxf(fmaxf(m, fmaxf(x[i].x, x[i].y)), fmaxf(x[i].z, x[i].w));
    }
    m = wave_max(m);
    if (lane == 0) sh[wave] = m;
    __syncthreads();
    m = fmaxf(fmaxf(sh[0], sh[1]), fmaxf(sh[2], sh[3]));
    const int t = tgt[r];
    float s = 0.0f, xt = 0.0f;
#pragma unroll
    for (int i = 0; i < NV; ++i) {
        const int v = 4 * tid + 1024 * i;
        if (t >= v && t < v + 4) xt = (t == v) ? x[i].x : (t == v + 1) ? x[i].y : (t == v + 2) ? x[i].z : x[i].w;
        x[i].x = expf(x[i].x - m); x[i].y = expf(x[i].y - m); x[i].z = expf(x[i].z - m); x[i].w = expf(x[i].w - m);
        s += (x[i].x + x[i].y) + (x[i].z + x[i].w);
    }
    s = wave_sum(s);
    xt = wave_sum(xt);
    if (lane == 0) { sh[4 + wave] = s; }
    __syncthreads();
    s = (sh[4] + sh[5]) + (sh[6] + sh[7]);
    const int tw = ((t >> 2) & 255) >> 6;
    if (wave == tw && lane == 0) {
        const float l = m + logf(s);
        lse[r] = l;
        ce[r] = l - xt;
    }
    if (dlogits == nullptr) return;
    const float scale = inv_n / s;
    float* drow = dlogits + (long long)r * ld;
#pragma unroll
    for (int i = 0; i < NV; ++i) {
        const int v = 4 * tid + 1024 * i;
        if (v < ld) {
            float4 d;
            d.x = x[i].x * scale - (v + 0 == t ? inv_n : 0.0f);
            d.y = x[i].y * scale - (v + 1 == t ? inv_n : 0.0f);
            d.z = x[i].z * scale - (v + 2 == t ? inv_n : 0.0f);
            d.w = x[i].w * scale - (v + 3 == t ? inv_n : 0.0f);
            if (NT) {
                __builtin_nontemporal_store(d.x, drow + v); __builtin_nontemporal_store(d.y, drow + v + 1);
                __builtin_nontemporal_store(d.z, drow + v + 2); __builtin_nontemporal_store(d.w, drow + v + 3);
            } else {
                *reinterpret_cast<float4*>(drow + v) = d;
            }
        }
    }
}

template <int NV, bool NT>
__global__ __launch_bounds__(256) void k_ce_rows_reg(const float* logits, int ld, int n_vocab,
                                                     const int* __restrict__ tgt, float* __restrict__ lse,
                                                     float* __restrict__ ce, float* dlogits, float inv_n) {
    __shared__ float sh[8];
    ce_row_reg<NV, NT>(sh, blockIdx.x, logits, ld, n_vocab, tgt, lse, ce, dlogits, inv_n);
}

__global__ __launch_bounds__(256) void k_ce_combine(const float2* __restrict__ part, int nparts,
                                                    const float* __restrict__ tgt_logit, int rows, float* __restrict__ ce) {
    const int lane = threadIdx.x & 63, row = blockIdx.x * 4 + (threadIdx.x >> 6);
    if (row >= rows) return;
    const float2* p = part + (long long)row * nparts;
    float m = -INFINITY;
    for (int i = lane; i < nparts; i += 64) m = fmaxf(m, p[i].x);
    m = wave_max(m);
    float s = 0.0f;
    for (int i = lane; i < nparts; i += 64) {
        const float2 v = p[i];
        if (v.x > -INFINITY) s += v.y * expf(v.x - m);
    }
    s = wave_sum(s);
    if (lane == 0) ce[row] = m + logf(s) - tgt_logit[row];
}

__global__ __launch_bounds__(256) void k_ce_finish(const float2* __restrict__ part, int nparts,
                                                   const int* __restrict__ tgt, int rows, float inv_n, float* E, int ld,
                                                   float* __restrict__ lse, float* __restrict__ ce, float* __restrict__ crow,
                                                   const float* __restrict__ hs, float* __restrict__ hs_scaled, int hp,
                                                   int* err_flag, unsigned long long* range_counter) {
    const int lane = threadIdx.x & 63, row = blockIdx.x * 4 + (threadIdx.x >> 6);
    if (blockIdx.x == 0 && threadIdx.x < 32) crow[rows + threadIdx.x] = 0.0f;
    if (row >= rows) return;
    const float2* p = part + (long long)row * nparts;
    float S = 0.0f;
    for (int i = lane; i < nparts; i += 64) S += p[i].y;
    S = wave_sum(S);
    const float c = inv_n / S;
    if (lane == 0) {
        float* e = E + (long long)row * ld + tgt[row];
        const float et = *e;
        const float l = logf(S);
        lse[row] = l;
        ce[row] = l - logf(et);
        crow[row] = c;
        if (!(S >= CE_SUM_MIN && S <= CE_SUM_MAX && et >= CE_TGT_MIN)) {
            atomicCAS(err_flag, 0, 4);
            crow[row] = 0.0f;
            atomicAdd_system(range_counter, 1ull);
            __threadfence_system();
        } else {
            *e = et - S;
        }
    }
    const float* hrow = hs + (long long)row * hp;
    float* orow = hs_scaled + (long long)row * hp;
    for (int i = 4 * lane; i < hp; i += 256) {
        float4 v = *reinterpret_cast<const float4*>(hrow + i);
        v.x *= c; v.y *= c; v.z *= c; v.w *= c;
        *reinterpret_cast<float4*>(orow + i) = v;
    }
}

__global__ __launch_bounds__(256) void k_scale_rows(float* C, const float* __restrict__ row_scale, long long n4, int n_per_row4) {
    for (long long i = (long long)blockIdx.x * 256 + threadIdx.x; i < n4; i += (long long)gridDim.x * 256) {
        const float c = row_scale[i / n_per_row4];
        float4 v = reinterpret_cast<float4*>(C)[i];
        v.x *= c; v.y *= c; v.z *= c; v.w *= c;
        reinterpret_cast<float4*>(C)[i] = v;
    }
}

__global__ __launch_bounds__(256) void k_loss_reduce(const float* __restrict__ ce, int T, int B, int rpg,
                                                     float* __restrict__ out) {
    __shared__ double sh[4];
    const int g = blockIdx.x, tid = threadIdx.x, lane = tid & 63, wave = tid >> 6;
    const int n = T * rpg;
    double s = 0.0;
    for (int i = tid; i < n; i += 256) {
        const int t = i / rpg, b = g * rpg + i % rpg;
        s += (double)ce[(long long)t * B + b];
    }
    s = wave_sum_d(s);
    if (lane == 0) sh[wave] = s;
    __syncthreads();
    if (tid == 0) out[g] = (float)(((sh[0] + sh[1]) + (sh[2] + sh[3])) / ((double)n + 1e-12));
}

__device__ __forceinline__ void sum_partials_body(const double* __restrict__ partials, int n, float* dst,
                                                  const int* flag_src, const float* __restrict__ ce, int ce_n, float* loss_out) {
    __shared__ double sh[4];
    const int tid = threadIdx.x, lane = tid & 63, wave = tid >> 6;
    double s = 0.0;
    for (int i = tid; i < n; i += 256) s += partials[i];
    s = wave_sum_d(s);
    if (lane == 0) sh[wave] = s;
    __syncthreads();
    if (tid == 0) {
        dst[0] = (float)((sh[0] + sh[1]) + (sh[2] + sh[3]));
        if (flag_src != nullptr) {
            dst[2] = (*flag_src == 2) ? 1.0f : 0.0f; dst[3] = (*flag_src == 1) ? 1.0f : 0.0f; dst[4] = 0.0f;
            dst[5] = (*flag_src == 4) ? 1.0f : 0.0f;
        }
    }
    if (ce == nullptr) return;
    __syncthreads();
    double l = 0.0;
    for (int i0 = tid; i0 < ce_n; i0 += 256 * 16) {
        float b[16];
#pragma unroll
        for (int k = 0; k < 16; ++k) b[k] = (i0 + 256 * k < ce_n) ? ce[i0 + 256 * k] : 0.0f;
#pragma unroll
        for (int k = 0; k < 16; ++k) if (i0 + 256 * k < ce_n) l += (double)b[k];
    }
    l = wave_sum_d(l);
    if (lane == 0) sh[wave] = l;
    __syncthreads();
    if (tid == 0) *loss_out = (float)(((sh[0] + sh[1]) + (sh[2] + sh[3])) / ((double)ce_n + 1e-12));
}


constexpr int EMBED_HEAVY = 48;
__global__ __launch_bounds__(256) void k_embed_grad_chunks(const int* __restrict__ X, int n, const float* __restrict__ dX, int Ep,
                                                           float* __restrict__ part, const int* __restrict__ tok_count, const SumPartialsArgs sp) {
    if (blockIdx.x == (unsigned)((n + 255) / 256)) { sum_partials_body(sp.partials, sp.n, sp.dst, sp.flag_src, sp.ce, sp.ce_n, sp.loss_out); return; }
    __shared__ unsigned long long mask[4];
    __shared__ __attribute__((aligned(16))) float wsum[4][1024];
    const int base = blockIdx.x * 256, tid = threadIdx.x, lane = tid & 63, wave = tid >> 6, i = base + tid;
    const int tok = (i < n) ? X[i] : -1;
    bool pending = (i < n) && tok_count[tok] > EMBED_HEAVY;
    for (;;) {
        const unsigned long long pb = __ballot(pending);
        if (lane == 0) mask[wave] = pb;
        __syncthreads();
        int first = -1;
#pragma unroll
        for (int w = 0; w < 4; ++w) if (first < 0 && mask[w]) first = 64 * w + __ffsll((long long)mask[w]) - 1;
        __syncthreads();
        if (first < 0) break;
        const int tk = X[base + first];
        const bool hit = pending && tok == tk;
        const unsigned long long hb = __ballot(hit);
        if (lane == 0) mask[wave] = hb;
        __syncthreads();
        {
            float4 a4[4];
#pragma unroll
            for (int c = 0; c < 4; ++c) a4[c] = make_float4(0.f, 0.f, 0.f, 0.f);
            unsigned long long mk = mask[wave];
            const int nf4 = Ep >> 2;
            while (mk) {
                int bits[4];
#pragma unroll
                for (int k = 0; k < 4; ++k) { bits[k] = mk ? __ffsll((long long)mk) - 1 : -1; mk &= mk - 1; }
                float4 v[4][4];
#pragma unroll
                for (int k = 0; k < 4; ++k) {
                    const float4* src = reinterpret_cast<const float4*>(dX + (long long)(base + 64 * wave + max(bits[k], 0)) * Ep);
#pragma unroll
                    for (int c = 0; c < 4; ++c) v[k][c] = (bits[k] >= 0 && lane + 64 * c < nf4) ? src[lane + 64 * c] : make_float4(0.f, 0.f, 0.f, 0.f);
                }
#pragma unroll
                for (int k = 0; k < 4; ++k)
                    if (bits[k] >= 0) {
#pragma unroll
                        for (int c = 0; c < 4; ++c) { a4[c].x += v[k][c].x; a4[c].y += v[k][c].y; a4[c].z += v[k][c].z; a4[c].w += v[k][c].w; }
                    }
            }
#pragma unroll
            for (int c = 0; c < 4; ++c)
                if (lane + 64 * c < nf4) reinterpret_cast<float4*>(&wsum[wave][0])[lane + 64 * c] = a4[c];
        }
        __syncthreads();
#pragma unroll
        for (int c = 0; c < 4; ++c)
            if (tid + 256 * c < Ep) {
                const int col = tid + 256 * c;
                part[(long long)(base + first) * Ep + col] = ((wsum[0][col] + wsum[1][col]) + wsum[2][col]) + wsum[3][col];
            }
        if (hit) pending = false;
        __syncthreads();
    }
}

__global__ __launch_bounds__(256) void k_embed_grad(const int* __restrict__ X, int n, const float* __restrict__ dX,
                                                    int Ep, float* __restrict__ dEmb, int* __restrict__ tok_first, int* __restrict__ tok_count,
                                                    const float* __restrict__ part) {
    __shared__ unsigned long long mask[4];
    const int r = blockIdx.x, tid = threadIdx.x, lane = tid & 63, wave = tid >> 6;
    const int tok = X[r];
    int want = n + 1;
    if (tok_first != nullptr) {
        if (tok_first[tok] != r) return;
        want = tok_count[tok];
        if (part != nullptr && want > EMBED_HEAVY) {
            float acc[4] = {0.f, 0.f, 0.f, 0.f};
            int found = 0;
            for (int base = r & ~255; base < n && found < want; base += 256) {
                const int i = base + tid;
                const bool hit = (i < n) && (X[i] == tok);
                const unsigned long long bal = __ballot(hit);
                if (lane == 0) mask[wave] = bal;
                __syncthreads();
                int first = -1;
#pragma unroll
                for (int w = 0; w < 4; ++w) {
                    found += __popcll(mask[w]);
                    if (first < 0 && mask[w]) first = 64 * w + __ffsll((long long)mask[w]) - 1;
                }
                if (first >= 0) {
                    const float* src = part + (long long)(base + first) * Ep;
#pragma unroll
                    for (int c = 0; c < 4; ++c)
                        if (tid + 256 * c < Ep) acc[c] += src[tid + 256 * c];
                }
                __syncthreads();
            }
#pragma unroll
            for (int c = 0; c < 4; ++c)
                if (tid + 256 * c < Ep) dEmb[(long long)tok * Ep + tid + 256 * c] = acc[c];
            if (tid == 0) { tok_first[tok] = 0x7FFFFFFF; tok_count[tok] = 0; }
            return;
        }
    } else {
        int dup = 0;
        for (int i = tid; i < r; i += 256) dup |= (X[i] == tok);
        if (__syncthreads_or(dup)) return;
    }

    float acc[4] = {0.f, 0.f, 0.f, 0.f};
    int found = 0;
    for (int base = r; base < n && found < want; base += 256) {
        const int i = base + tid;
        const bool hit = (i < n) && (X[i] == tok);
        const unsigned long long bal = __ballot(hit);
        if (lane == 0) mask[wave] = bal;
        __syncthreads();
#pragma unroll
        for (int w = 0; w < 4; ++w) {
            unsigned long long mk = mask[w];
            found += __popcll(mk);
            while (mk) {
                const int bit = __ffsll((long long)mk) - 1;
                mk &= mk - 1;
                const float* src = dX + (long long)(base + 64 * w + bit) * Ep;
#pragma unroll
                for (int c = 0; c < 4; ++c)
                    if (tid + 256 * c < Ep) acc[c] += src[tid + 256 * c];
            }
        }
        __syncthreads();
    }
#pragma unroll
    for (int c = 0; c < 4; ++c)
        if (tid + 256 * c < Ep) dEmb[(long long)tok * Ep + tid + 256 * c] = acc[c];
    if (tok_first != nullptr && tid == 0) { tok_first[tok] = 0x7FFFFFFF; tok_count[tok] = 0; }
}

__global__ __launch_bounds__(256) void k_sqnorm_partials(const float* __restrict__ x, long long n,
                                                         double* __restrict__ partials) {
    __shared__ double sh[4];
    const int tid = threadIdx.x, lane = tid & 63, wave = tid >> 6;
    const long long base = (long long)blockIdx.x * SQ_CHUNK;
    double s = 0.0;
#pragma unroll
    for (int i = 0; i < 4; ++i) {
        const long long idx = base + 4 * (tid + 256 * i);
        if (idx + 3 < n) {
            const float4 v = *reinterpret_cast<const float4*>(x + idx);
            s += ((double)v.x * v.x + (double)v.y * v.y) + ((double)v.z * v.z + (double)v.w * v.w);
        } else {
            for (long long j = idx; j < n && j < idx + 4; ++j) s += (double)x[j] * x[j];
        }
    }
    s = wave_sum_d(s);
    if (lane == 0) sh[wave] = s;
    __syncthreads();
    if (tid == 0) partials[blockIdx.x] = (sh[0] + sh[1]) + (sh[2] + sh[3]);
}

__global__ __launch_bounds__(256) void k_adam_update(const UpdateArgs a) {
    __shared__ double sh[4];
    __shared__ float s_scale, s_alpha;
    const int tid = threadIdx.x, lane = tid & 63, wave = tid >> 6;
    if (a.consume != nullptr) {
        if (a.consume[0] == 0.0f) return;
        if (tid == 0) { s_scale = a.consume[1]; s_alpha = a.consume[2]; }
    } else {
    if ((a.err_flag != nullptr && *a.err_flag != 0) || a.tail[2] != 0.0f || a.tail[3] != 0.0f || a.tail[4] != 0.0f || a.tail[5] != 0.0f) {
        if (a.publish != nullptr && blockIdx.x == 0 && tid == 0) a.publish[0] = 0.0f;
        return;
    }
    double s = 0.0;
    for (int i = tid; i < a.n_partials; i += 256) s += a.partials[i];
    s = wave_sum_d(s);
    if (lane == 0) sh[wave] = s;
    __syncthreads();
    if (tid == 0) {
        double sq = ((sh[0] + sh[1]) + (sh[2] + sh[3])) * (double)a.grad_scale * (double)a.grad_scale;
        if (a.use_slices) sq += (double)a.tail[0] * (double)a.grad_scale * (double)a.grad_scale;
        const double gnorm = sqrt(sq);
        const double clip = (double)a.clip;
        s_scale = (float)(clip / fmax(gnorm, clip) * (double)a.grad_scale);
        const long long step = *a.step;
        const double t = (double)(step + 1);
        const double lr_s = (double)a.lr * pow(0.5, (double)step / (double)a.n_decay);
        s_alpha = (float)(lr_s * sqrt(1.0 - pow(0.999, t)) / (1.0 - pow(0.9, t)));
        if (a.gnorm_out != nullptr && blockIdx.x == 0) *a.gnorm_out = (float)gnorm;
        if (a.publish != nullptr && blockIdx.x == 0) { a.publish[0] = 1.0f; a.publish[1] = s_scale; a.publish[2] = s_alpha; }
    }
    }
    __syncthreads();
    const float scale = s_scale, alpha = s_alpha;
    const float b1 = 0.9f, b2 = 0.999f, eps = 1e-8f;
    const long long n4 = a.n >> 2;
    for (long long i = (long long)blockIdx.x * 256 + tid; i < n4; i += (long long)gridDim.x * 256) {
        float4 g = reinterpret_cast<const float4*>(a.g)[i];
        float4 m = reinterpret_cast<float4*>(a.m)[i];
        float4 v = reinterpret_cast<float4*>(a.v)[i];
        float4 p = reinterpret_cast<float4*>(a.p)[i];
#define FSMG_ADAM1(c)                                         \
        {                                                     \
            const float gc = g.c * scale;                     \
            m.c = b1 * m.c + (1.0f - b1) * gc;                \
            v.c = b2 * v.c + (1.0f - b2) * gc * gc;           \
            p.c = p.c - alpha * m.c / (sqrtf(v.c) + eps);     \
        }
        FSMG_ADAM1(x) FSMG_ADAM1(y) FSMG_ADAM1(z) FSMG_ADAM1(w)
#undef FSMG_ADAM1
        reinterpret_cast<float4*>(a.m)[i] = m;
        reinterpret_cast<float4*>(a.v)[i] = v;
        reinterpret_cast<float4*>(a.p)[i] = p;
    }
}

__global__ __launch_bounds__(256) void k_sgd_update(const UpdateArgs a) {
    __shared__ double sh[4];
    __shared__ float s_scale;
    if ((a.err_flag != nullptr && *a.err_flag != 0) || a.tail[2] != 0.0f || a.tail[3] != 0.0f || a.tail[4] != 0.0f || a.tail[5] != 0.0f) return;
    const int tid = threadIdx.x, lane = tid & 63, wave = tid >> 6;
    double s = 0.0;
    for (int i = tid; i < a.n_partials; i += 256) s += a.partials[i];
    s = wave_sum_d(s);
    if (lane == 0) sh[wave] = s;
    __syncthreads();
    if (tid == 0) {
        double sq = (sh[0] + sh[1]) + (sh[2] + sh[3]);
        if (a.use_slices) sq += (double)a.tail[0];
        const double gnorm = sqrt(sq), clip = (double)a.clip;
        s_scale = (float)(clip / fmax(gnorm, clip)) * a.lr;
        if (a.gnorm_out != nullptr && blockIdx.x == 0) *a.gnorm_out = (float)gnorm;
    }
    __syncthreads();
    const float step = s_scale;
    const long long n4 = a.n >> 2;
    for (long long i = (long long)blockIdx.x * 256 + tid; i < n4; i += (long long)gridDim.x * 256) {
        const float4 g = reinterpret_cast<const float4*>(a.g)[i];
        float4 p = reinterpret_cast<float4*>(a.p)[i];
        p.x -= step * g.x; p.y -= step * g.y; p.z -= step * g.z; p.w -= step * g.w;
        reinterpret_cast<float4*>(a.p)[i] = p;
    }
// ... 24 lines not shown
__global__ __launch_bounds__(256) void k_compare_words(const uint4* __restrict__ a, const uint4* __restrict__ b, long long n4, int* err_flag,
                                                       unsigned long long* counter) {
    if (*err_flag != 0) return;
    unsigned bad = 0;
    for (long long i = (long long)blockIdx.x * 256 + threadIdx.x; i < n4; i += (long long)gridDim.x * 256) {
        const uint4 x = a[i], y = b[i];
        bad += (x.x != y.x) | (x.y != y.y) | (x.z != y.z) | (x.w != y.w);
    }
    const unsigned long long votes = __ballot(bad != 0);
    if (votes == 0) return;
    unsigned total = bad;
    for (int o = 32; o > 0; o >>= 1) total += __shfl_xor(total, o);
    if ((threadIdx.x & 63) == __ffsll((long long)votes) - 1) {
        atomicAdd_system(counter, (unsigned long long)total);
        *err_flag = 2;
        __threadfence_system();
    }
}

__global__ void k_queue_probe(int* flag, int* out, int role, long long ticks) {
    if (threadIdx.x != 0) return;
    if (role == 1) { __hip_atomic_store(flag, 1, __ATOMIC_RELAXED, __HIP_MEMORY_SCOPE_AGENT); return; }
    const unsigned long long t0 = __builtin_amdgcn_s_memrealtime();
    int seen = 0;
    while ((long long)(__builtin_amdgcn_s_memrealtime() - t0) < ticks) {
        if (__hip_atomic_load(flag, __ATOMIC_RELAXED, __HIP_MEMORY_SCOPE_AGENT) != 0) { seen = 1; break; }
        __builtin_amdgcn_s_sleep(16);
    }
    out[0] = seen;
}

__global__ void k_unigram_update(const int* __restrict__ words, long long n, unsigned* __restrict__ counts, int vocab, int* err_flag) {
    for (long long i = (long long)blockIdx.x * blockDim.x + threadIdx.x; i < n; i += (long long)gridDim.x * blockDim.x) {
        const int w = words[i];
        if (w < 0 || w >= vocab) { atomicOr(err_flag, 1); continue; }
        atomicAdd(counts + w, 1u);
    }
}
__global__ __launch_bounds__(1024) void k_unigram_nll(const int* __restrict__ words, long long n, const unsigned* __restrict__ counts, int vocab,
                                                      float* out, int* err_flag) {
    __shared__ double sh[16];
    __shared__ float s_total;
    const int tid = threadIdx.x, lane = tid & 63, wave = tid >> 6;
    double s = 0.0;
    for (int i = tid; i < vocab; i += 1024) s += (double)counts[i];
    s = wave_sum_d(s);
    if (lane == 0) sh[wave] = s;
    __syncthreads();
    if (tid == 0) { double t = 0.0; for (int w = 0; w < 16; ++w) t += sh[w]; s_total = (float)t; }
    __syncthreads();
    const float total = s_total;
    double l = 0.0;
    for (long long i = tid; i < n; i += 1024) {
        const int w = words[i];
        if (w < 0 || w >= vocab) { atomicOr(err_flag, 1); continue; }
        l += (double)logf((float)counts[w] / total);
    }
    l = wave_sum_d(l);
    __syncthreads();
    if (lane == 0) sh[wave] = l;
    __syncthreads();
    if (tid == 0) { double t = 0.0; for (int w = 0; w < 16; ++w) t += sh[w]; out[0] = (float)(-t / (double)(n > 0 ? n : 1)); out[1] = total; }
}
__global__ __launch_bounds__(1024) void k_unigram_argmax(const unsigned* __restrict__ counts, int vocab, int* out) {
    __shared__ unsigned sc[1024];
    __shared__ int si[1024];
    const int tid = threadIdx.x;
    unsigned best = 0; int bi = 0x7FFFFFFF;
    for (int i = tid; i < vocab; i += 1024) { const unsigned c = counts[i]; if (c > best || (c == best && i < bi)) { best = c; bi = i; } }
    sc[tid] = best; si[tid] = bi;
    __syncthreads();
    for (int o = 512; o > 0; o >>= 1) {
        if (tid < o) {
            const unsigned c = sc[tid + o]; const int i = si[tid + o];
            if (c > sc[tid] || (c == sc[tid] && i < si[tid])) { sc[tid] = c; si[tid] = i; }
        }
        __syncthreads();
    }
    if (tid == 0) *out = si[0];
}

}

hipError_t launch_token_prep(hipStream_t s, const int* support, int n_support, const int* query, int n_query,
                             int T, int vocab, int start_word, int* X, int* Y, int* err_flag, int* tok_first, int* tok_count) {
    const long long total = (long long)(n_support + n_query) * T;
    if (total <= 0) return hipSuccess;
    int blocks = (int)((total + 255) / 256);
    if (blocks > 1024) blocks = 1024;
    hipLaunchKernelGGL(k_token_prep, dim3(blocks), dim3(256), 0, s, support, n_support, query, n_query, T, vocab,
                       start_word, X, Y, err_flag, tok_first, tok_count);
    return hipGetLastError();
}

hipError_t launch_ce_rows(hipStream_t s, const float* logits, int ld, int rows, int n_vocab, const int* tgt,
                          float* lse, float* ce, float* dlogits, float inv_n) {
    if (rows <= 0) return hipSuccess;
    static const int nt = std::getenv("FSMG_CE_NT") ? (std::atoi(std::getenv("FSMG_CE_NT")) != 0) : 1;
    if (ld <= 6 * 1024) {
        if (nt) hipLaunchKernelGGL((k_ce_rows_reg<6, true>), dim3(rows), dim3(256), 0, s, logits, ld, n_vocab, tgt, lse, ce, dlogits, inv_n);
        else hipLaunchKernelGGL((k_ce_rows_reg<6, false>), dim3(rows), dim3(256), 0, s, logits, ld, n_vocab, tgt, lse, ce, dlogits, inv_n);
    } else if (ld <= 12 * 1024) {
        if (nt) hipLaunchKernelGGL((k_ce_rows_reg<12, true>), dim3(rows), dim3(256), 0, s, logits, ld, n_vocab, tgt, lse, ce, dlogits, inv_n);
        else hipLaunchKernelGGL((k_ce_rows_reg<12, false>), dim3(rows), dim3(256), 0, s, logits, ld, n_vocab, tgt, lse, ce, dlogits, inv_n);
    }
    else hipLaunchKernelGGL(k_ce_rows, dim3(rows), dim3(256), 0, s, logits, ld, n_vocab, tgt, lse, ce, dlogits, inv_n);
    return hipGetLastError();
}

hipError_t launch_ce_combine(hipStream_t s, const float2* part, int nparts, const float* tgt_logit, int rows, float* ce) {
    if (rows <= 0) return hipSuccess;
    hipLaunchKernelGGL(k_ce_combine, dim3((rows + 3) / 4), dim3(256), 0, s, part, nparts, tgt_logit, rows, ce);
    return hipGetLastError();
}

hipError_t launch_ce_finish(hipStream_t s, const float2* part, int nparts, const int* tgt, int rows, float inv_n,
                            float* E, int ld, float* lse, float* ce, float* crow, const float* hs, float* hs_scaled, int hp,
                            int* err_flag, long long* range_counter) {
    if (rows <= 0) return hipSuccess;
    if ((hp & 3) != 0 || err_flag == nullptr || range_counter == nullptr) return hipErrorInvalidValue;
    hipLaunchKernelGGL(k_ce_finish, dim3((rows + 3) / 4), dim3(256), 0, s, part, nparts, tgt, rows, inv_n, E, ld, lse, ce, crow,
                       hs, hs_scaled, hp, err_flag, (unsigned long long*)range_counter);
    return hipGetLastError();
}

hipError_t launch_scale_rows(hipStream_t s, float* C, const float* row_scale, int M, int N) {
    if (M <= 0 || N <= 0) return hipSuccess;
    if ((N & 3) != 0) return hipErrorInvalidValue;
    const long long n4 = (long long)M * N / 4;
    hipLaunchKernelGGL(k_scale_rows, dim3((int)std::min<long long>((n4 + 255) / 256, 2048)), dim3(256), 0, s, C, row_scale, n4, N / 4);
    return hipGetLastError();
}

hipError_t launch_loss_reduce(hipStream_t s, const float* ce, int T, int B, int rows_per_group, int ngroups,
                              float* out) {
    hipLaunchKernelGGL(k_loss_reduce, dim3(ngroups), dim3(256), 0, s, ce, T, B, rows_per_group, out);
    return hipGetLastError();
}

hipError_t launch_embed_grad(hipStream_t s, const int* X, int n, const float* dX, int Ep, float* dEmb, int* tok_first, int* tok_count, float* part,
                             const SumPartialsArgs* sum) {
    if (n <= 0) return sum != nullptr ? hipErrorInvalidValue : hipSuccess;
    if (Ep > 1024) return hipErrorInvalidValue;
    if (tok_first == nullptr || tok_count == nullptr || (Ep & 3) != 0 || ((uintptr_t)dX & 15) != 0) part = nullptr;
    if (part == nullptr && sum != nullptr) return hipErrorInvalidValue;
    if (part != nullptr) {
        SumPartialsArgs sp{};
        if (sum != nullptr) sp = *sum;
        hipLaunchKernelGGL(k_embed_grad_chunks, dim3((n + 255) / 256 + (sum != nullptr ? 1 : 0)), dim3(256), 0, s, X, n, dX, Ep, part, tok_count, sp);
    }
    hipLaunchKernelGGL(k_embed_grad, dim3(n), dim3(256), 0, s, X, n, dX, Ep, dEmb, tok_first, tok_count, part);
    return hipGetLastError();
}

hipError_t launch_multi_op(hipStream_t s, const MultiOps& r) {
    if (r.count <= 0) return hipSuccess;
    long long bx = 1;
    for (int k = 0; k < r.count; ++k) {
        const long long want = r.op[k].kind == MULTI_FILL ? (r.op[k].n / 4 + 255) / 256 : r.op[k].kind == MULTI_MEAN ? 1 :
                               (r.op[k].sq == nullptr ? (r.op[k].n / 4 + 255) / 256 : (r.op[k].n + SQ_CHUNK - 1) / SQ_CHUNK);
        bx = std::max(bx, want);
    }
    bx = std::max<long long>(1, std::min<long long>(bx, 1024));
    hipLaunchKernelGGL(k_multi_op, dim3((int)bx, r.count), dim3(256), 0, s, r);
    return hipGetLastError();
}

hipError_t launch_gather_rows(hipStream_t s, const int* table, const int* idx, int n_rows, int T, int n_songs, int* out, int* err_flag) {
    if (n_rows <= 0) return hipSuccess;
    const long long total = (long long)n_rows * T;
    hipLaunchKernelGGL(k_gather_rows, dim3((int)std::min<long long>((total + 255) / 256, 1024)), dim3(256), 0, s, table, idx, n_rows, T, n_songs, out, err_flag);
    return hipGetLastError();
}

hipError_t launch_fill32_if(hipStream_t s, const int* cond, void* p, uint32_t word, long long n_words) {
    if (n_words <= 0) return hipSuccess;
    long long blocks = (n_words / 4 + 255) / 256;
    if (blocks > 2048) blocks = 2048;
    if (blocks < 1) blocks = 1;
    hipLaunchKernelGGL(k_fill32_if, dim3((int)blocks), dim3(256), 0, s, cond, (uint32_t*)p, word, n_words);
    return hipGetLastError();
}

hipError_t launch_fill32(hipStream_t s, void* p, uint32_t word, long long n_words) {
    if (n_words <= 0) return hipSuccess;
    long long blocks = (n_words / 4 + 255) / 256;
    if (blocks > 2048) blocks = 2048;
    if (blocks < 1) blocks = 1;
    hipLaunchKernelGGL(k_fill32, dim3((int)blocks), dim3(256), 0, s, (uint32_t*)p, word, n_words);
    return hipGetLastError();
}

int sqnorm_blocks(long long n) { return (int)((n + SQ_CHUNK - 1) / SQ_CHUNK); }

hipError_t launch_sqnorm_partials(hipStream_t s, const float* x, long long n, double* partials) {
    const int nb = sqnorm_blocks(n);
    if (nb <= 0) return hipSuccess;
    hipLaunchKernelGGL(k_sqnorm_partials, dim3(nb), dim3(256), 0, s, x, n, partials);
    return hipGetLastError();
}

hipError_t launch_adam_update(hipStream_t s, const UpdateArgs& a) {
    long long n4 = a.n >> 2;
    int blocks = (int)((n4 + 255) / 256);
    if (blocks > 2048) blocks = 2048;
    if (blocks < 1) blocks = 1;
    hipLaunchKernelGGL(k_adam_update, dim3(blocks), dim3(256), 0, s, a);
    return hipGetLastError();
}

hipError_t launch_sgd_update(hipStream_t s, const UpdateArgs& a) {
    long long n4 = a.n >> 2;
    int blocks = (int)((n4 + 255) / 256);
    if (blocks > 2048) blocks = 2048;
    if (blocks < 1) blocks = 1;
    hipLaunchKernelGGL(k_sgd_update, dim3(blocks), dim3(256), 0, s, a);
    return hipGetLastError();
}

hipError_t launch_step_increment(hipStream_t s, const StepIncArgs& a) {
    hipLaunchKernelGGL(k_step_increment, dim3(1), dim3(64), 0, s, a);
    return hipGetLastError();
}

hipError_t launch_sum_partials(hipStream_t s, const double* partials, int n, float* dst, const int* flag_src,
                               const float* ce, int ce_n, float* loss_out) {
    hipLaunchKernelGGL(k_sum_partials, dim3(1), dim3(256), 0, s, partials, n, dst, flag_src, ce, ce_n, loss_out);
    return hipGetLastError();
}

hipError_t launch_queue_probe(hipStream_t s, int* flag, int* out, int role, long long realtime_ticks) {
    hipLaunchKernelGGL(k_queue_probe, dim3(1), dim3(64), 0, s, flag, out, role, realtime_ticks);
    return hipGetLastError();
}
// ... 33 lines not shown
```

### few-shot-music-generation_amd/csrc/fsmg_kernels.h

```cpp
#pragma once
#include <hip/hip_runtime.h>
#include <stdint.h>

namespace fsmg {

enum { OP_KC = 0, OP_XC = 1 };
struct GemmArgs {
    const float* A; int lda;
    const float* B; int ldb;
    float* C; int ldc;
    int M, N, K;
    const float* bias;
    const int* gather;
    float* colsum;
    int ksplit;
    long long c_slab;
    long long colsum_slab;
    float2* ce_part; const int* ce_tgt; float* ce_tgt_logit; int ce_nvocab;
    int ce_store;
    const float* colsum_w;
    const float* row_scale;
    int nt_store;
    int xcd_first; int* work; int* claim; int work_limit; const int* stop;
    const int* gate; int gate_expect; int gate_rows; int gate_last; int* gate_err; int gate_spin;
// ... 70 lines not shown

struct LstmBwdRsArgs {
    const float* KhF;
    float* inbox;
    float* Z;
    const float* Cs;
    float* dc;
    const float* dH;
    int* err_flag;
    int B, Hp, T, t0, t1;
    int spin_limit;
};
bool lstm_bwd_rs_supported(int B, int Hp);
long long lstm_bwd_rs_inbox_floats(int B, int Hp);
hipError_t launch_lstm_bwd_rs(hipStream_t s, const LstmBwdRsArgs& a);
hipError_t launch_repack_kh(hipStream_t s, const float* Kh, float* fwd, float* bwd, int Hp);

enum { XCD_DEFER_OUTPUTS = 16,
       XCD_NO_POLL_SLEEP = 32,
       XCD_CHAINS = 64,
       XCD_PROBE = 128,
       XCD_LOCAL_PLAIN = 256,
       XCD_LATE_DRAIN = 1024,
       XCD_GROUP_STORES = 2048,
       XCD_PROBE_DELAY = 8192,
       XCD_STREAM = 512 };
int lstm_xcd_default_variant(int B, bool forward, int Hp = 512, int rpx = 0, bool bx3 = false);
struct LstmFwdXcdArgs {
    const float* KhX;
    float* HX;
    float* Z;
    float* Cs;
    float* Hs;
    int* tickets;
    int* err_flag;
    int B, T, t0, t1;
    int spin_limit;
    unsigned long long* prof;
    int rpx;
    int variant;
    int Hp;
    int bx3;
    int* progress;
    int progress_lag;
    int progress_every;
};
struct LstmBwdXcdArgs {
    const float* KhXb;
    float* inbox;
    float* Z;
    const float* Cs;
    float* dc;
    const float* dH;
    int* tickets;
    int* err_flag;
    int B, T, t0, t1;
    int spin_limit;
    unsigned long long* prof;
    int rpx;
    int variant;
    int Hp;
    int bx3;
};
bool lstm_xcd_supported(int B, int Hp);
int lstm_xcd_max_rows(int Hp);
long long lstm_xcd_hx_floats(int B, int T, int Hp = 512, bool bx3 = false, int rpx = 0);
long long lstm_xcd_inbox_floats(int B, int Hp = 512, int rpx = 0);
int lstm_xcd16_packed_rows(int B, int Hp = 512);
inline int lstm_xcd_active_blocks(int B, int rpx, int Hp = 512) { return (Hp == 1024 ? 64 : 32) * ((B + rpx - 1) / rpx); }
long long lstm_xcd_weight_floats(int Hp = 512, bool bx3 = false);
bool lstm_xcd_bx3_pays(int B, int Hp);
int lstm_xcd_packed_rows(int B);
hipError_t launch_repack_kh_xcd(hipStream_t s, const float* Kh, float* fwd, float* bwd, int Hp = 512, bool bx3 = false);
constexpr int REPACK_MAX_LAYERS = 4;
struct StepIncArgs;
struct RepackAllArgs { int n; int Hp; const float* Kh[REPACK_MAX_LAYERS]; float* cf[REPACK_MAX_LAYERS]; float* cb[REPACK_MAX_LAYERS]; float* xf[REPACK_MAX_LAYERS]; float* xb[REPACK_MAX_LAYERS];
                       int bx3;
                       int mode;  };
hipError_t launch_repack_kh_all(hipStream_t s, const RepackAllArgs& a, const StepIncArgs* inc = nullptr);
hipError_t launch_lstm_fwd_xcd(hipStream_t s, const LstmFwdXcdArgs& a);
hipError_t launch_lstm_bwd_xcd(hipStream_t s, const LstmBwdXcdArgs& a);

enum { MULTI_FILL = 0, MULTI_REDUCE = 1, MULTI_MEAN = 2 };
constexpr int MULTI_MAX_OPS = 16;
struct MultiOp { int kind; void* dst; const void* src; long long n; long long stride; int nslab; uint32_t word; const int* cond; double* sq;
                 const float* row_scale; int row_len;  };
struct MultiOps { MultiOp op[MULTI_MAX_OPS]; int count; };
hipError_t launch_multi_op(hipStream_t s, const MultiOps& r);
hipError_t launch_gather_rows(hipStream_t s, const int* table, const int* idx, int n_rows, int T, int n_songs, int* out, int* err_flag);
hipError_t launch_fill32(hipStream_t s, void* p, uint32_t word, long long n_words);
hipError_t launch_copy_words(hipStream_t s, void* dst, const void* src, long long n_words);
hipError_t launch_fill32_if(hipStream_t s, const int* cond, void* p, uint32_t word, long long n_words);
hipError_t launch_token_prep(hipStream_t s, const int* support, int n_support, const int* query, int n_query,
                             int T, int vocab, int start_word, int* X, int* Y, int* err_flag, int* tok_first = nullptr, int* tok_count = nullptr);
hipError_t launch_ce_rows(hipStream_t s, const float* logits, int ld, int rows, int n_vocab, const int* tgt,
                          float* lse, float* ce, float* dlogits, float inv_n);
constexpr float CE_SUM_MIN = 8.0e-27f, CE_SUM_MAX = 1.0e30f, CE_TGT_MIN = 1.0e-30f;
hipError_t launch_ce_finish(hipStream_t s, const float2* part, int nparts, const int* tgt, int rows, float inv_n,
                            float* E, int ld, float* lse, float* ce, float* crow, const float* hs, float* hs_scaled, int hp,
                            int* err_flag, long long* range_counter);
hipError_t launch_scale_rows(hipStream_t s, float* C, const float* row_scale, int M, int N);
hipError_t launch_ce_combine(hipStream_t s, const float2* part, int nparts, const float* tgt_logit, int rows, float* ce);
hipError_t launch_loss_reduce(hipStream_t s, const float* ce, int T, int B, int rows_per_group, int ngroups,
                              float* out);
struct SumPartialsArgs { const double* partials; int n; float* dst; const int* flag_src; const float* ce; int ce_n; float* loss_out; };
hipError_t launch_embed_grad(hipStream_t s, const int* X, int n, const float* dX, int Ep, float* dEmb, int* tok_first = nullptr, int* tok_count = nullptr,
                             float* part = nullptr, const SumPartialsArgs* sum = nullptr);
int sqnorm_blocks(long long n);
hipError_t launch_sqnorm_partials(hipStream_t s, const float* x, long long n, double* partials);

struct UpdateArgs {
    float* p; float* m; float* v; const float* g; long long n;
    const double* partials; int n_partials;
    const float* tail;
    int use_slices;
    float grad_scale;
    float lr, n_decay, clip;
    const long long* step;
    float* gnorm_out;
    const int* err_flag;
    float* publish; const float* consume;
};
hipError_t launch_adam_update(hipStream_t s, const UpdateArgs& a);
hipError_t launch_sgd_update(hipStream_t s, const UpdateArgs& a);
struct StepIncArgs { long long* step; const float* loss_src; float loss_scale; float* ring; int ring_cap; int* err_flag; long long* counters;
                     int* handoff_dirty; int clear_ok; };
__device__ __forceinline__ void step_increment_body(const StepIncArgs& a) {
    const int e = a.err_flag != nullptr ? *a.err_flag : 0;
    if (a.handoff_dirty != nullptr) {
        if (e == 2) *a.handoff_dirty = 1;
        else if (a.clear_ok) *a.handoff_dirty = 0;
    }
    const bool peer_timeout = a.loss_src != nullptr && a.loss_src[1] != 0.0f;
    const bool peer_token = a.loss_src != nullptr && a.loss_src[2] != 0.0f;
    const bool peer_failed = a.loss_src != nullptr && a.loss_src[3] != 0.0f;
    const bool peer_range = a.loss_src != nullptr && a.loss_src[4] != 0.0f;
    if (e != 0 || peer_timeout || peer_token || peer_failed || peer_range) {
        if (a.counters != nullptr) {
            if (e == 2 || peer_timeout) a.counters[0] += 1; else if (e == 1 || peer_token) a.counters[1] += 1;
            else if (e == 4 || peer_range) a.counters[5] += 1; else a.counters[2] += 1;
            __threadfence_system();
        }
        if (a.err_flag != nullptr) *a.err_flag = 0;
        return;
    }
    const long long s = *a.step;
    if (a.ring != nullptr && a.loss_src != nullptr) a.ring[s % a.ring_cap] = *a.loss_src * a.loss_scale;
    *a.step = s + 1;
}
hipError_t launch_step_increment(hipStream_t s, const StepIncArgs& a);
hipError_t launch_sum_partials(hipStream_t s, const double* partials, int n, float* dst, const int* flag_src = nullptr,
                               const float* ce = nullptr, int ce_n = 0, float* loss_out = nullptr);
hipError_t launch_compare_words(hipStream_t s, const void* a, const void* b, long long n_words, int* err_flag, long long* counter);
hipError_t launch_queue_probe(hipStream_t s, int* flag, int* out, int role, long long realtime_ticks);
hipError_t launch_clock_probe(hipStream_t s, long long realtime_ticks, unsigned long long* out);
hipError_t launch_unigram_update(hipStream_t s, const int* words, long long n, unsigned* counts, int vocab, int* err_flag);
hipError_t launch_unigram_nll(hipStream_t s, const int* words, long long n, const unsigned* counts, int vocab, float* out, int* err_flag);
hipError_t launch_unigram_argmax(hipStream_t s, const unsigned* counts, int vocab, int* out);
hipError_t launch_gen_cell(hipStream_t s, const float* Kx, int in_dim, const float* Kh, const float* bias, int Hp, const float* emb, int ldemb,
                           const int* tok, int ldtok, int pos, const float* x, const float* h_in, float* h_out, float* c, int B);
hipError_t launch_gen_logits(hipStream_t s, const float* W, int ldw, const float* bias, int ncols, const float* h, int Hp, int B,
                             float* logits, int ldl);
struct GenFilters {
    float top_p, min_p, theta;
    int window;
};
hipError_t launch_gen_pick(hipStream_t s, const float* logits, int ldl, int ncols, int B, float temperature, int top_k, const GenFilters* f,
                           uint64_t seed, int t, int ctr_t, int* tok, int ldtok, int pos_out, int* out_tok, float* out_lp, int num);
hipError_t launch_gen_primer(hipStream_t s, const int* primer, int B, int P, int vocab, int start, int* tok, int ldtok, int* err,
                             int rows_per_primer = 1);
hipError_t launch_beam_init(hipStream_t s, float* cum, int R, int W);
hipError_t launch_beam_rowtop(hipStream_t s, const float* logits, int ldl, int ncols, int R, int W, const float* cum, float* cand_s,
                              float* cand_lp, int* cand_v);
hipError_t launch_beam_select(hipStream_t s, int G, int W, int ncols, const float* cand_s, const float* cand_lp, const int* cand_v,
                              float* cum, int* tok, int ldtok, int pos_out, int* par, int* htok, float* hlp);
hipError_t launch_beam_reorder(hipStream_t s, int L, int R, int W, int Hp, const int* par, const float* h_src, float* h_dst,
                               const float* c_src, float* c_dst);
hipError_t launch_beam_backtrace(hipStream_t s, int R, int W, int num, const int* par, const int* htok, const float* hlp, const float* cum,
                                 int* out_tok, float* out_lp, float* out_score);
hipError_t launch_feed_logprob(hipStream_t s, const float* logits, int ldl, int ncols, int R, const int* tok, int ldtok, int pos_tgt,
                               float* out_lp, int n, int i);
hipError_t launch_dstate_rows(hipStream_t s, int L, int Rd, int Rs, int Hp, const int* rows, int div, const float* h_src, float* h_dst,
                              const float* c_src, float* c_dst, const int* tok_src, int ld_src, int off_src, int* tok_dst, int ld_dst,
                              int off_dst, int ntok);
hipError_t launch_dstate_reset(hipStream_t s, long long n_state, float* hh, float* cc, long long n_tok, int* tok, int start);
hipError_t launch_dstate_tokens(hipStream_t s, const int* tokens, int R, int n, int ncols, int start, int* tok, int ldtok, int off, int* err);

constexpr int SCORE_REG_COLS = 10 * 1024;
hipError_t launch_score_rows(hipStream_t s, const float* logits, int ld, int rows, int n_vocab, const int* tgt, int B, int T,
                             float* out_lp, int* out_rank, float* out_ent, int* out_arg);
// ... 23 lines not shown
```

### few-shot-music-generation_amd/csrc/fsmg_model.h

```cpp
#pragma once
#include <atomic>
#include <hip/hip_runtime.h>
#include <dlfcn.h>

#include <algorithm>
#include <cmath>
#include <cstdlib>
#include <new>
#include <cstdio>
#include <cstring>
#include <functional>
#include <map>
#include <mutex>
#include <string>
#include <vector>

#include "../../include/fsmg.h"
#include "fsmg_kernels.h"

namespace fsmg_host {
using namespace fsmg;
struct OpBatch;

inline int64_t round_up(int64_t x, int64_t m) { return (x + m - 1) / m * m; }
// ... 70 lines not shown
    std::vector<float*> HF;
    float* dzF = nullptr;
    float* dzF_all = nullptr;
    int64_t dzfa_floats = 0;
    float* inbox = nullptr;
    int64_t inbox_floats = 0;
    int chain_spin_limit = 1 << 18;
    bool retry_armed = false;
    bool persist_cfg = true;
    int fallback_steps = 200;
    int fallback_left = 0;
    long long* host_counters = nullptr;
    long long* d_counters = nullptr;
    long long seen_timeouts = 0, seen_token_errors = 0, seen_peer_failures = 0, seen_range_skips = 0;
    bool force_fwd_rt = false;
    bool persist = true;
    float* khf = nullptr;
    float* P_saved = nullptr;
    static constexpr int MAX_TABLES = 4;
    int* table[MAX_TABLES] = {};
    int64_t table_rows[MAX_TABLES] = {};
    int* d_idx = nullptr; int idx_cap = 0;
    int* d_gather = nullptr; int64_t gather_cap = 0;
    bool xcd = true;
    static constexpr int xcd_max_rows = 128;
    int dp_split = 0;
    int pair_mode = 2;
    int xcd_variant = -1;
    int xcd_variant_bwd = -1;
    float* khx = nullptr;
    bool xcd_bx3 = false;
    bool xcd_bx3_forced = false;
    float* HX = nullptr; int64_t hx_floats = 0;
    float* inboxX = nullptr; int64_t inboxx_floats = 0;
    int* d_inbox_dirty = nullptr;
    int* tickets = nullptr;
    static constexpr int TICKET_LAUNCHES = 64;
    int ticket_next = 0;
    int64_t n_timeouts = 0, n_persist_launches = 0, n_xcd_launches = 0, n_step_launches = 0;
    bool khf_dirty = true;
    bool lazy_cs = true;
    bool cs_stale = false;
    float* slabs = nullptr;
    float* arena = nullptr;
    int64_t arena_cap = 0, arena_off = 0;
    bool warned_split = false;
    int* tok_first = nullptr; int* tok_count = nullptr;
    bool tok_table_open = false;
    bool last_bwd_xcd = false;
    bool eager = true, eager_call = false;
    const int* cur_sup = nullptr; const int* cur_qry = nullptr;
    float* colsum_slabs = nullptr;
    float* slabs2 = nullptr;
    float* colsum_slabs2 = nullptr;
    hipStream_t probe = nullptr;
    unsigned long long* d_probe = nullptr;
    hipStream_t aux = nullptr;
    int aux_tries = 0;
    static constexpr int NCHUNK = 16;
    static constexpr int nchunk = 8;
    static constexpr int nchunk_persist = 4;
    static constexpr int aux_blocks_persist = 2;
    static constexpr int aux_blocks_per_cu = 2;
    hipEvent_t ev_chunk[NCHUNK] = {};
    hipEvent_t ev_fork = nullptr, ev_join = nullptr;
    bool merge_dk = true;
    hipEvent_t ev_bucket[2] = {};
    bool overlap = true;
    bool overlap_forced = false;
    bool ov_call = false;
    int bx3 = 1;
    int gemm_h = 1;
    int gemm_ws = 1;
    int max_split = fsmg_host::MAX_SPLIT;
    long long gemm_kinds[4] = {};
    bool xov = false, xov_call = false;
    bool xov_eligible = false;
    bool bucket0_recorded = false;
    static constexpr int xov_dw_split = 4;
    static constexpr int xov_pub = 6;
    int xov_strikes = 0;
    bool xov_last = false;
    int xov_parts = 3;
    int* xov_prog = nullptr;
    static constexpr int XOV_CTL = 8192;
    int* xov_ctl = nullptr;
    int64_t slab_cap = 0;
    std::map<std::string, hipGraphExec_t> graphs;
    struct LaunchCounts { int64_t xcd = 0, persist = 0, step = 0; bool bwd_xcd = false; };
    std::map<std::string, LaunchCounts> graph_counts;
    char* gen = nullptr;
    size_t gen_bytes = 0;
    std::vector<fsmg_dstate_s*> dstates;
    std::vector<fsmg_cache_s*> caches;
    char* cat = nullptr;
    size_t cat_bytes = 0;

    void* comm = nullptr; bool own_comm = false; int world = 1, rank = 0;
    hipStream_t comm_stream = nullptr;
    hipEvent_t ev_comm = nullptr;
    int lastB = 0;
    bool have_grads = false;
    bool upd_split = false;
    bool upd_pending = false;
    hipEvent_t ev_upd_fork = nullptr, ev_upd = nullptr;
    float* d_decided = nullptr;
    fsmg_host::OpBatch* slabs_owner = nullptr;
    int xov_selfcheck_left = 2;
    int xov_selfcheck_every = 1000;
    long long xov_passes = 0, xov_selfcheck_runs = 0;
    bool xov_selfcheck_fault = false;
    long long seen_selfcheck_mismatch = 0;
    bool inplace_dlogits = true;
    bool fused_softmax = true;
    bool fs_call = false;
    float* Hsc = nullptr;
    float* crow = nullptr;
    long long seen_softmax_range = 0;
    bool tail_aside = true;
    bool side_pending = false;
    hipEvent_t ev_side_fork = nullptr, ev_side = nullptr;
    hipEvent_t ev_turn = nullptr, ev_turn_aux = nullptr;
    std::atomic<bool> capturing{false};
    std::string err;
    bool timing = false;
    std::string timing_only;
    std::map<std::string, fsmg_host::TimerClass> timers;
};

namespace fsmg_host {

extern thread_local std::string g_create_error;

inline int fail(fsmg_model* h, int code, const std::string& msg) {
    if (h) h->err = msg; else g_create_error = msg;
    return code;
}

#define HIPCK(h, call)                                                                         \
    do {                                                                                       \
        hipError_t e_ = (call);                                                                \
        if (e_ != hipSuccess)                                                                  \
            return fail(h, FSMG_ERR_HIP, std::string(#call) + ": " + hipGetErrorString(e_));  \
    } while (0)

struct Roctx {
    int (*push)(const char*) = nullptr; int (*pop)() = nullptr;
    Roctx() {
        const char* e = std::getenv("FSMG_ROCTX");
        if (!e || e[0] == '0') return;
        void* lib = dlopen("libroctx64.so", RTLD_NOW | RTLD_GLOBAL);
        if (!lib) lib = dlopen("libroctx64.so.4", RTLD_NOW | RTLD_GLOBAL);
        if (!lib) return;
        push = (int (*)(const char*))dlsym(lib, "roctxRangePushA");
        pop = (int (*)())dlsym(lib, "roctxRangePop");
        if (!push || !pop) push = nullptr;
    }
};
inline Roctx& roctx() { static Roctx r; return r; }
struct ScopedRange {
    bool on;
    explicit ScopedRange(const char* name) : on(roctx().push != nullptr) { if (on) roctx().push(name); }
    ~ScopedRange() { if (on) roctx().pop(); }
};

struct ScopedTimer {
// ... 8 lines not shown
    ~ScopedTimer() {
        if (!tc) return;
        hipEventRecord(b, h->stream);
        tc->pending.emplace_back(a, b);
    }
};

inline void drain_timers(fsmg_model* h) {
    hipStreamSynchronize(h->stream);
    for (auto& kv : h->timers) {
        for (auto& pr : kv.second.pending) {
            float ms = 0.f;
            if (hipEventElapsedTime(&ms, pr.first, pr.second) == hipSuccess) {
                kv.second.total_ms += ms;
                kv.second.launches += 1;
            }
            hipEventDestroy(pr.first);
            hipEventDestroy(pr.second);
        }
        kv.second.pending.clear();
    }
}

int begin_call(fsmg_model* h, bool keep_pending = false);
int settle_pending(fsmg_model* h);
std::mutex& turn_mutex();
#define BEGIN_CALL(h, ...)                                                           \
    do {                                                                             \
        const int rc_begin_ = fsmg_host::begin_call(h, ##__VA_ARGS__);               \
        if (rc_begin_ != FSMG_OK) return rc_begin_;                                  \
    } while (0)

void compute_dims(const fsmg_config& c, fsmg_model* m);
int64_t build_layout(fsmg_model* m);
int64_t state_bytes_for(int64_t n_flat);
const ParamDesc* find_param(fsmg_model* h, const char* name);
int upload_tensor(fsmg_model* h, float* flat, const char* name, const float* host, int64_t count);
int download_tensor(fsmg_model* h, const float* flat, const char* name, float* host, int64_t count);

int pick_split(int max_split, int64_t M, int64_t N, int64_t K, int64_t slots = 0, bool bx3 = false, int tile_mn = 0);
int ensure_scratch(fsmg_model* h, int B);
void drop_graphs(fsmg_model* h);

struct Lane { hipStream_t s; float* slabs; float* colsum_slabs; int lds_pad; int slots; };
inline Lane main_lane(fsmg_model* h) { return Lane{h->stream, h->slabs, h->colsum_slabs, 0, gemm_block_slots()}; }
inline Lane aux_lane(fsmg_model* h, bool forward_only = false, bool persistent_chain = false) {
    const int cap = std::min(4, (persistent_chain ? h->aux_blocks_persist : h->aux_blocks_per_cu) + (forward_only ? 1 : 0));
    return Lane{h->aux, h->slabs2, h->colsum_slabs2, gemm_lds_pad_for(cap), 256 * cap};
}

bool use_ws_gemm(fsmg_model* h, int amode, int bmode, const GemmArgs& g, const Lane& ln);
bool use_h_gemm(fsmg_model* h, int amode, int bmode, const GemmArgs& g, const Lane& ln);
inline hipError_t launch_gemm(fsmg_model* h, hipStream_t s, int amode, int bmode, const GemmArgs& g, int lds_pad = 0) {
    if (g.M <= 0 || g.N <= 0) return hipSuccess;
    const hipError_t e = fsmg::launch_gemm(s, amode, bmode, g, lds_pad);
    if (e == hipSuccess) ++h->gemm_kinds[(g.bx3 >= 1 && g.bx3 <= 3 && !(g.xcd_first != 0 && g.bx3 != 3)) ? g.bx3 : 0];
    return e;
}

struct OpBatch;
int gemm(fsmg_model* h, const Lane& ln, int amode, int bmode, GemmArgs g, OpBatch* defer = nullptr, double* sq = nullptr, bool* sq_done = nullptr);
#define GEMMCK(call) do { int rc_ = (call); if (rc_ != FSMG_OK) return rc_; } while (0)

struct OpBatch {
    MultiOps r{};
    fsmg_model* h;
    hipStream_t s;
    explicit OpBatch(fsmg_model* h_) : h(h_), s(h_->stream) { r.count = 0; }
    ~OpBatch() { if (h->slabs_owner == this) h->slabs_owner = nullptr; }
    OpBatch(const OpBatch&) = delete;
    OpBatch& operator=(const OpBatch&) = delete;
    int room(int n) { return (r.count + n > MULTI_MAX_OPS) ? flush() : FSMG_OK; }
    int add(void* p, uint32_t word, long long n_words, const int* cond = nullptr) {
        if (n_words <= 0) return FSMG_OK;
        const int rc = room(1); if (rc != FSMG_OK) return rc;
        MultiOp& o = r.op[r.count++];
        o = MultiOp{}; o.kind = MULTI_FILL; o.dst = p; o.word = word; o.n = n_words; o.cond = cond;
        return FSMG_OK;
    }
    int reduce(const float* slabs, long long stride, int nslab, float* out, long long n, double* sq = nullptr, const float* row_scale = nullptr, int row_len = 0) {
        if (n <= 0) return FSMG_OK;
        if (row_scale != nullptr && (sq != nullptr || row_len <= 0 || ((n | stride | (long long)row_len) & 3) != 0))
            return fail(h, FSMG_ERR_STATE, "internal: a row-scaled slab sum needs n, stride and row_len multiples of 4 and no squared-norm partials");
        const int rc = room(1); if (rc != FSMG_OK) return rc;
        MultiOp& o = r.op[r.count++];
        o = MultiOp{}; o.kind = MULTI_REDUCE; o.dst = out; o.src = slabs; o.stride = stride; o.nslab = nslab; o.n = n; o.sq = sq;
        o.row_scale = row_scale; o.row_len = row_len;
        return FSMG_OK;
    }
    int mean(const float* x, long long n, float* out) {
        if (n <= 0) return FSMG_OK;
        const int rc = room(1); if (rc != FSMG_OK) return rc;
        MultiOp& o = r.op[r.count++];
        o = MultiOp{}; o.kind = MULTI_MEAN; o.dst = out; o.src = x; o.n = n;
        return FSMG_OK;
    }
    int flush() {
        if (h->slabs_owner == this) h->slabs_owner = nullptr;
        if (r.count == 0) return FSMG_OK;
        HIPCK(h, launch_multi_op(s, r));
        r.count = 0;
        return FSMG_OK;
    }
};
typedef OpBatch FillBatch;

template <class F>
int run_graphed(fsmg_model* h, const std::string& key, F&& body) {
    if (!h->cfg.use_graph || h->timing || h->ov_call || h->xov_call || h->eager_call) return body();
    auto it = h->graphs.find(key);
    if (it != h->graphs.end()) {
        const auto& c = h->graph_counts[key];
        h->n_xcd_launches += c.xcd; h->n_persist_launches += c.persist; h->n_step_launches += c.step;
        if (key[0] == 'f') h->last_bwd_xcd = c.bwd_xcd;
    }
    if (it == h->graphs.end()) {
        hipGraph_t graph = nullptr;
        const int64_t x0 = h->n_xcd_launches, p0 = h->n_persist_launches, s0 = h->n_step_launches;
        int rc; hipError_t e;
        {
            std::lock_guard<std::mutex> turn_lk(turn_mutex());
            h->capturing.store(true);
            if (hipStreamBeginCapture(h->stream, hipStreamCaptureModeThreadLocal) != hipSuccess) { h->capturing.store(false); return fail(h, FSMG_ERR_HIP, "hipStreamBeginCapture failed"); }
            rc = body();
            { auto& c = h->graph_counts[key]; c.xcd = h->n_xcd_launches - x0; c.persist = h->n_persist_launches - p0; c.step = h->n_step_launches - s0; c.bwd_xcd = h->last_bwd_xcd; }
            e = hipStreamEndCapture(h->stream, &graph);
            h->capturing.store(false);
        }
        if (rc != FSMG_OK) { if (graph) hipGraphDestroy(graph); return rc; }
        if (e != hipSuccess || graph == nullptr)
            return fail(h, FSMG_ERR_HIP, std::string("hipStreamEndCapture: ") + hipGetErrorString(e));
        hipGraphExec_t exec = nullptr;
        const hipError_t ei = hipGraphInstantiate(&exec, graph, nullptr, nullptr, 0);
        hipGraphDestroy(graph);
        if (ei != hipSuccess) return fail(h, FSMG_ERR_HIP, std::string("hipGraphInstantiate: ") + hipGetErrorString(ei));
        it = h->graphs.emplace(key, exec).first;
    }
    HIPCK(h, hipGraphLaunch(it->second, h->stream));
    return FSMG_OK;
}

inline int chunk_begin(const fsmg_model* h, int c, int nch) { return (int)((int64_t)c * h->T / nch); }
inline bool use_overlap(const fsmg_model* h) { return h->ov_call && !h->timing && h->aux != nullptr && h->T >= std::max(h->nchunk, h->nchunk_persist); }

inline bool use_xcd(const fsmg_model* h, int B, bool backward = false) {
    if (h->Hp == 1024 && h->pair_mode < (backward ? 2 : 1)) return false;
    return h->persist && h->xcd && h->khx != nullptr && h->HX != nullptr && B <= h->xcd_max_rows && lstm_xcd_supported(B, h->Hp) &&
           lstm_xcd_hx_floats(B, h->T, h->Hp, h->xcd_bx3) <= h->hx_floats &&
           ((h->Hp == 1024 && !backward) || lstm_xcd_inbox_floats(B, h->Hp) <= h->inboxx_floats);
}
inline float* dlogits_buf(const fsmg_model* h) { return h->inplace_dlogits ? h->logits : h->dlogits; }
inline int xov_first_free(int B, int Hp = 512) {
    const int rpx = lstm_xcd16_packed_rows(B, Hp);
    return rpx > 0 ? (Hp == 1024 ? 2 : 1) * ((B + rpx - 1) / rpx) : 8;
}

inline int* next_tickets(fsmg_model* h) {
    int* t = h->tickets + 8 * (h->ticket_next % fsmg_model::TICKET_LAUNCHES);
    ++h->ticket_next;
    return t;
}

inline int gemm_items(const GemmArgs& g) { return ((g.M + 255) / 256) * ((g.N + 255) / 256) * std::max(1, g.ksplit); }
inline bool xov_fits(const GemmArgs& g) { return 4 + gemm_items(g) <= fsmg_model::XOV_CTL; }
void choose_schedule(fsmg_model* h, int B, bool train = false);
void xov_gate(fsmg_model* h, GemmArgs& g, int B);
int gemm_prepare_queue(fsmg_model* h, GemmArgs& g, int split, OpBatch* defer, bool* ok);
int select_xcd_format(fsmg_model* h, int B);
int gemm_restricted(fsmg_model* h, hipStream_t s, int amode, int bmode, GemmArgs g, int first, int* ctl);
int gemm_cleanup(fsmg_model* h, hipStream_t s, int amode, int bmode, GemmArgs g, int* ctl);

int stage_tokens(fsmg_model* h, const int32_t* support, int n_sup, const int32_t* query, int n_qry, int on_device);
int reset_tok_table(fsmg_model* h);
int token_prep(fsmg_model* h, int n_sup, int n_qry, bool train = false);
enum { HEAD_LOSS = 0, HEAD_LOGITS = 1, HEAD_NONE = 2 };
int forward(fsmg_model* h, int B, int rows_per_group, int ngroups, float* loss_out, bool want_dlogits, int head = HEAD_LOSS);
GemmArgs dw_args(fsmg_model* h, int B);
int backward(fsmg_model* h, int B, int part = 0);
int repack_recurrent_weights(fsmg_model* h, hipStream_t s, const StepIncArgs* inc, bool* inc_done);
int repack_recurrent_weights(fsmg_model* h, hipStream_t s);
int ensure_khf(fsmg_model* h);
int ensure_cs(fsmg_model* h);
inline bool pass_reads_cs(const fsmg_model* h, int B, bool train) {
    return !use_xcd(h, B) || (train && !use_xcd(h, B, true));
}
int apply_update(fsmg_model* h, float grad_scale);
int sgd_update(fsmg_model* h, float lr);
int save_theta(fsmg_model* h);
int restore_theta(fsmg_model* h);
void on_timeout(fsmg_model* h);
void on_softmax_range(fsmg_model* h);
inline bool is_retry(int rc) { return rc == FSMG_ERR_TIMEOUT || rc == FSMG_ERR_SOFTMAX_RANGE; }
int with_adapted_theta(fsmg_model* h, const int32_t* support, int32_t n_support_rows, int32_t inner_steps, float inner_lr,
                       int32_t support_on_device, const std::function<int()>& at_theta_prime);
int poll_skipped(fsmg_model* h);
int report(fsmg_model* h, int what);
int check_tokens_and_read(fsmg_model* h, const float* d_src, float scale, float* host_out, int n, bool train_tail = false);
int after_update(fsmg_model* h, float grad_scale, float* loss);
int exchange_gradients(fsmg_model* h);
void comm_destroy(fsmg_model* h);

}
```

Before: 640.5.

## Fold fills, token prep and gradient sqnorm into existing kernels for a lean step

Adds a lean_step bitmask, on by default with all bits set, that removes several small launches from the train step. Token prep is deferred into the forward pass and carries the pending buffer fills. The backward's early fills ride on the ce_finish kernel. The gradient squared-norm partials are computed as a by-product of slab reductions and the embed-grad chunk kernel, so the update can skip a separate pass over the full gradient. A wave-per-row embed-grad kernel is also added; together these cut launch overhead and a memory pass over the gradients, at the cost of more complex bookkeeping and a risk of stale or mis-covered partials.

Result: no change. 645.6 (median of 6 runs) (+0.8%).

```diff
diff --git a/few-shot-music-generation_amd/csrc/api_backward.hip b/few-shot-music-generation_amd/csrc/api_backward.hip
--- a/few-shot-music-generation_amd/csrc/api_backward.hip
+++ b/few-shot-music-generation_amd/csrc/api_backward.hip
@@ -41,6 +41,32 @@
         const long long Bp16 = (B + 15) / 16 * 16;
         GEMMCK(fills.add(h->dzF_all, 0xFFFFFFFFu, (long long)T * Bp16 * G4));
     }
+    return FSMG_OK;
+}
+
+bool backward_xov(fsmg_model* h, int B, GemmArgs& gdw, int& dw_split) {
+    const Lane mainl = main_lane(h);
+    const bool ov = use_overlap(h);
+    const bool xcd = use_xcd(h, B, true);
+    gdw = dw_args(h, B);
+    dw_split = 1;
+    if (h->xov_call && (h->xov_parts & 2) && xcd && !ov) dw_split = std::max(1, std::min(std::min(h->xov_dw_split, MAX_SPLIT), gdw.K / 256));
+    while (dw_split > 1 && (int64_t)dw_split * gdw.M * gdw.N > h->slab_cap) --dw_split;
+    if (dw_split > 1) {
+        gdw.C = mainl.slabs; gdw.c_slab = (int64_t)gdw.M * gdw.N; gdw.ksplit = dw_split;
+        gdw.colsum = mainl.colsum_slabs; gdw.colsum_slab = gdw.N;
+    }
+    return h->xov_call && (h->xov_parts & 2) && xcd && !ov && dw_split > 1 && xov_fits(gdw);
+}
+
+int backward_early_fills(fsmg_model* h, int B, OpBatch& fills, bool* added) {
+    *added = false;
+    GemmArgs gdw{};
+    int dw_split = 1;
+    if (!backward_xov(h, B, gdw, dw_split)) return FSMG_OK;
+    GEMMCK(fills.add(h->G + h->off_emb, 0u, (long long)h->V1 * h->Ep));
+    GEMMCK(fills.add(h->xov_ctl + fsmg_model::XOV_CTL, 0u, 4 + gemm_items(gdw)));
+    *added = true;
     return FSMG_OK;
 }
 
@@ -58,15 +84,11 @@
     if (!xcd && h->cs_stale) return fail(h, FSMG_ERR_STATE, "internal: backward pass on the column-split kernels with stale fragment copies of K_h (ensure_cs not called)");
     const int nch = ov ? (chain ? h->nchunk_persist : h->nchunk) : 1;
     const Lane auxl = aux_lane(h, false, chain);
-    GemmArgs gdw = dw_args(h, B);
+    GemmArgs gdw{};
     int dw_split = 1;
-    if (h->xov_call && (h->xov_parts & 2) && xcd && !ov) dw_split = std::max(1, std::min(std::min(h->xov_dw_split, MAX_SPLIT), gdw.K / 256));
-    while (dw_split > 1 && (int64_t)dw_split * gdw.M * gdw.N > h->slab_cap) --dw_split;
-    if (dw_split > 1) {
-        gdw.C = mainl.slabs; gdw.c_slab = (int64_t)gdw.M * gdw.N; gdw.ksplit = dw_split;
-        gdw.colsum = mainl.colsum_slabs; gdw.colsum_slab = gdw.N;
-    }
-    const bool xov = h->xov_call && (h->xov_parts & 2) && xcd && !ov && dw_split > 1 && xov_fits(gdw);
+    const bool xov = backward_xov(h, B, gdw, dw_split);
+    const bool early = h->bwd_fills_early && xov && part != 2;
+    h->bwd_fills_early = false;
     const int rpx = xov ? lstm_xcd16_packed_rows(B, Hp) : 0;
     const bool cut = !ov && !xov;
     if (part == 2 && !cut) return FSMG_OK;
@@ -74,6 +96,12 @@
     bool dx_sq_done = false, top_fills_done = false;
     const bool defer_ok = part == 0 && (cut || xov);
     if (part != 2) h->arena_off = 0;
+    h->gsq_ready = false;
+    h->gsq_on = defer_ok && (lean_bits(h) & 4) && h->upd_follows;
+    if (h->gsq_on) {
+        h->gsq_skip = h->cfg.clip_norm_mode == FSMG_CLIP_TF1_SLICES ? round_up((int64_t)h->V1 * h->Ep, FLAT_ALIGN) : 0;
+        h->gsq_cov.assign((size_t)sqnorm_blocks(h->n_flat - h->gsq_skip), 0);
+    }
     h->last_bwd_xcd = xcd;
     FillBatch fills(h);
     OpBatch late(h);
@@ -82,7 +110,7 @@
     OpBatch* const d_late = defer_ok ? &late : nullptr;
     const bool aside = h->tail_aside && defer_ok && h->eager_call && h->aux != nullptr && !h->timing && !ov;
     h->side_pending = false;
-    if (part != 2) GEMMCK(fills.add(h->G + h->off_emb, 0u, (long long)h->V1 * h->Ep));
+    if (part != 2 && !early) GEMMCK(fills.add(h->G + h->off_emb, 0u, (long long)h->V1 * h->Ep));
     if (ov) GEMMCK(fills.flush());
     if (part == 2) {
     } else if (ov) {
@@ -98,7 +126,7 @@
         HIPCK(h, hipEventRecord(h->ev_bucket[0], h->aux));
         h->bucket0_recorded = true;
     } else if (xov) {
-        GEMMCK(fills.add(h->xov_ctl + fsmg_model::XOV_CTL, 0u, 4 + gemm_items(gdw)));
+        if (!early) GEMMCK(fills.add(h->xov_ctl + fsmg_model::XOV_CTL, 0u, 4 + gemm_items(gdw)));
         GEMMCK(fills.flush());
         GEMMCK(dhout_chunk(h, mainl, B, 0, T, d_now));
         HIPCK(h, hipEventRecord(h->ev_fork, s));
@@ -128,7 +156,24 @@
         const int nb = sqnorm_blocks(rows * h->Ep);
         const SumPartialsArgs sp{h->partials, nb, h->G + h->n_flat + 0, h->d_err, loss_in_batch ? nullptr : h->ce, (int)rows, h->G + h->n_flat + 1};
         const bool sum_rides = dx_sq_done && h->dXpart != nullptr && h->tok_first != nullptr;
-        HIPCK(h, launch_embed_grad(ts, h->X, (int)rows, h->dXemb, h->Ep, h->G + h->off_emb, h->tok_first, h->tok_count, h->dXpart, sum_rides ? &sp : nullptr));
+        SqChunksArgs sc{};
+        bool gsq_done = h->gsq_on && sum_rides && ts == s;
+        if (gsq_done) {
+            const int nb = (int)h->gsq_cov.size();
+            h->gsq_prefix = h->gsq_skip == 0 ? (int)std::min<int64_t>(nb, (round_up((int64_t)h->V1 * h->Ep, FLAT_ALIGN) + SQNORM_CHUNK - 1) / SQNORM_CHUNK) : 0;
+            sc.x = h->G + h->gsq_skip; sc.n = h->n_flat - h->gsq_skip; sc.partials = h->gsq();
+            for (int c = h->gsq_prefix; c < nb && gsq_done; ++c) {
+                if (h->gsq_cov[(size_t)c]) continue;
+                if (sc.nranges > 0 && sc.first[sc.nranges - 1] + sc.count[sc.nranges - 1] == c) { ++sc.count[sc.nranges - 1]; ++sc.total; continue; }
+                if (sc.nranges == SQ_MAX_RANGES) { gsq_done = false; break; }
+                sc.first[sc.nranges] = c; sc.count[sc.nranges] = 1; ++sc.nranges; ++sc.total;
+            }
+        }
+        h->gsq_on = false;
+        HIPCK(h, launch_embed_grad(ts, h->X, (int)rows, h->dXemb, h->Ep, h->G + h->off_emb, h->tok_first, h->tok_count, h->dXpart, sum_rides ? &sp : nullptr,
+                                   (lean_bits(h) & 8) != 0, gsq_done ? &sc : nullptr));
+        h->gsq_ready = gsq_done;
+        h->gsq_extra = gsq_done ? sc.total : 0;
         h->tok_table_open = false;
         if (!dx_sq_done) HIPCK(h, launch_sqnorm_partials(ts, h->dXemb, rows * h->Ep, h->partials));
         if (!sum_rides) HIPCK(h, launch_sum_partials(ts, sp.partials, sp.n, sp.dst, sp.flag_src, sp.ce, sp.ce_n, sp.loss_out));
@@ -283,6 +328,7 @@
             GEMMCK(tail_kernels(s));
         } else if (aside && l == 0) {
             dk_defer = &late2;
+            h->gsq_on = false;
             GEMMCK(dx_gemm());
             GEMMCK(tail_kernels(h->aux));
             GEMMCK(dk_gemm(nullptr));
diff --git a/few-shot-music-generation_amd/csrc/api_debug.hip b/few-shot-music-generation_amd/csrc/api_debug.hip
--- a/few-shot-music-generation_amd/csrc/api_debug.hip
+++ b/few-shot-music-generation_amd/csrc/api_debug.hip
@@ -46,6 +46,9 @@
     int l;
     if (!std::strcmp(what, "aux_tries")) { host[0] = (float)h->aux_tries; return FSMG_OK; }
     if (!std::strcmp(what, "fused_softmax")) { host[0] = h->fused_softmax ? 1.0f : 0.0f; if (count > 1) host[1] = h->fs_call ? 1.0f : 0.0f; return FSMG_OK; }
+    if (!std::strcmp(what, "lean_step")) {
+        host[0] = (float)h->lean_step; if (count > 1) host[1] = (float)h->gsq_used; if (count > 2) host[2] = (float)h->gsq_extra; return FSMG_OK;
+    }
     if (!std::strcmp(what, "xcd_bx3")) { host[0] = h->xcd_bx3 ? 1.0f : 0.0f; return FSMG_OK; }
     if (!std::strcmp(what, "gemm_kinds")) {
         for (int64_t i = 0; i < count && i < 4; ++i) host[i] = (float)h->gemm_kinds[i];
diff --git a/few-shot-music-generation_amd/csrc/api_forward.hip b/few-shot-music-generation_amd/csrc/api_forward.hip
--- a/few-shot-music-generation_amd/csrc/api_forward.hip
+++ b/few-shot-music-generation_amd/csrc/api_forward.hip
@@ -26,11 +26,16 @@
     return ops.flush();
 }
 
-int token_prep(fsmg_model* h, int n_sup, int n_qry, bool train) {
+static int token_prep_launch(fsmg_model* h, int n_sup, int n_qry, bool train, const MultiOps* fills) {
     const bool table = train && h->tok_first != nullptr;
     HIPCK(h, launch_token_prep(h->stream, h->cur_sup, n_sup, h->cur_qry, n_qry, h->T, h->V, h->V,
-                               h->X, h->Y, h->d_err, table ? h->tok_first : nullptr, table ? h->tok_count : nullptr));
-    return FSMG_OK;
+                               h->X, h->Y, h->d_err, table ? h->tok_first : nullptr, table ? h->tok_count : nullptr, fills));
+    return FSMG_OK;
+}
+int token_prep(fsmg_model* h, int n_sup, int n_qry, bool train) {
+    h->prep_deferred = train && (lean_bits(h) & 1);
+    if (h->prep_deferred) { h->prep_nsup = n_sup; h->prep_nqry = n_qry; return FSMG_OK; }
+    return token_prep_launch(h, n_sup, n_qry, train, nullptr);
 }
 
 GemmArgs logits_args(fsmg_model* h, int B, int t0, int t1) {
@@ -48,8 +53,13 @@
 }
 int ce_finish(fsmg_model* h, hipStream_t s, int B, int64_t rows) {
     ScopedTimer tm(h, "ce");
+    FillBatch early(h);
+    h->bwd_fills_early = false;
+    if (lean_bits(h) & 2) GEMMCK(backward_early_fills(h, B, early, &h->bwd_fills_early));
     HIPCK(h, launch_ce_finish(s, h->ce_part, h->ce_nparts, h->Y, (int)rows, (float)(1.0 / ((double)rows + 1e-12)), h->logits, h->V1p,
-                              h->lse, h->ce, h->crow, h->Hs[h->L - 1] + (size_t)B * h->Hp, h->Hsc, h->Hp, h->d_err, h->d_counters + 4));
+                              h->lse, h->ce, h->crow, h->Hs[h->L - 1] + (size_t)B * h->Hp, h->Hsc, h->Hp, h->d_err, h->d_counters + 4,
+                              h->bwd_fills_early ? &early.r : nullptr));
+    early.r.count = 0;
     return FSMG_OK;
 }
 int ce_rows(fsmg_model* h, hipStream_t s, int B, int t0, int t1, int64_t rows_total) {
@@ -101,6 +111,10 @@
     const int64_t rows = (int64_t)T * B;
     const Lane mainl = main_lane(h);
     hipStream_t s = h->stream;
+    const bool prep_here = h->prep_deferred;
+    h->prep_deferred = false;
+    h->bwd_fills_early = false;
+    h->gsq_on = false;
     const bool ov = head == HEAD_LOSS && use_overlap(h);
     const bool xcd = use_xcd(h, B);
     const bool chain1 = !xcd && h->persist && !h->force_fwd_rt && lstm_fwd_chain_supported(B, Hp);
@@ -126,16 +140,6 @@
         GEMMCK(fills.add(h->Hs[l], 0u, (long long)B * Hp));
         GEMMCK(fills.add(h->Cs[l], 0u, (long long)B * Hp));
         if (!xcd) GEMMCK(fills.add(h->HF[l], 0u, (long long)Bp16 * Hp));
-        {
-            ScopedTimer tm(h, "gemm_zx");
-            GemmArgs g{};
-            if (l == 0) { g.A = h->P + h->off_emb; g.lda = h->Ep; g.gather = h->X; g.K = h->Ep; }
-            else { g.A = h->Hs[l - 1] + (size_t)B * Hp; g.lda = Hp; g.K = Hp; }
-            g.B = h->P + h->off_kx[l]; g.ldb = G4;
-            g.C = h->Z[l]; g.ldc = G4; g.M = (int)rows; g.N = G4;
-            g.bias = h->P + h->off_b[l]; g.ksplit = 1;
-            GEMMCK(gemm(h, mainl, OP_KC, OP_XC, g));
-        }
         auto chain_fills = [&]() -> int {
             if (chain)
                 GEMMCK(fills.add(h->HF[l] + Bp16 * Hp, 0xFFFFFFFFu, (long long)T * Bp16 * Hp));
@@ -150,9 +154,27 @@
                     GEMMCK(fills.add(h->xov_prog, 0u, T));
                 }
             }
-            return fills.flush();
+            return FSMG_OK;
         };
-        GEMMCK(chain_fills());
+        if (l == 0 && prep_here) {
+            GEMMCK(chain_fills());
+            GEMMCK(token_prep_launch(h, h->prep_nsup, h->prep_nqry, true, &fills.r));
+            fills.r.count = 0;
+        }
+        {
+            ScopedTimer tm(h, "gemm_zx");
+            GemmArgs g{};
+            if (l == 0) { g.A = h->P + h->off_emb; g.lda = h->Ep; g.gather = h->X; g.K = h->Ep; }
+            else { g.A = h->Hs[l - 1] + (size_t)B * Hp; g.lda = Hp; g.K = Hp; }
+            g.B = h->P + h->off_kx[l]; g.ldb = G4;
+            g.C = h->Z[l]; g.ldc = G4; g.M = (int)rows; g.N = G4;
+            g.bias = h->P + h->off_b[l]; g.ksplit = 1;
+            GEMMCK(gemm(h, mainl, OP_KC, OP_XC, g));
+        }
+        if (!(l == 0 && prep_here)) {
+            GEMMCK(chain_fills());
+            GEMMCK(fills.flush());
+        }
         if (l == 0) GEMMCK(settle_pending(h));
         if (xov && top) {
             HIPCK(h, hipEventRecord(h->ev_fork, s));
diff --git a/few-shot-music-generation_amd/csrc/api_handle.hip b/few-shot-music-generation_amd/csrc/api_handle.hip
--- a/few-shot-music-generation_amd/csrc/api_handle.hip
+++ b/few-shot-music-generation_amd/csrc/api_handle.hip
@@ -157,6 +157,7 @@
         if (const char* e = std::getenv("FSMG_MAX_SPLIT")) h->max_split = std::max(1, std::atoi(e));
         if (const char* e = std::getenv("FSMG_XCD_OVERLAP")) h->xov = std::atoi(e) != 0;
         if (const char* e = std::getenv("FSMG_XOV_PARTS")) h->xov_parts = std::max(1, std::min(7, std::atoi(e)));
+        if (const char* e = std::getenv("FSMG_LEAN_STEP")) h->lean_step = std::max(0, std::min(15, std::atoi(e)));
         if (const char* e = std::getenv("FSMG_EAGER")) h->eager = (e[0] != '0');
         if (const char* e = std::getenv("FSMG_MERGE_DK")) h->merge_dk = (e[0] != '0');
         if (const char* e = std::getenv("FSMG_UPD_SPLIT")) h->upd_split = (e[0] != '0');
@@ -381,6 +382,7 @@
         }
     }
     else if (!std::strcmp(what, "tail_aside")) h->tail_aside = value != 0;
+    else if (!std::strcmp(what, "lean_step")) h->lean_step = (int)std::max<int64_t>(0, std::min<int64_t>(value, 15));
     else if (!std::strcmp(what, "fused_softmax")) h->fused_softmax = value != 0;
 
     else if (!std::strcmp(what, "xov_selfcheck")) h->xov_selfcheck_left = (int)std::max<int64_t>(0, std::min<int64_t>(value, 1 << 30));
diff --git a/few-shot-music-generation_amd/csrc/api_step.hip b/few-shot-music-generation_amd/csrc/api_step.hip
--- a/few-shot-music-generation_amd/csrc/api_step.hip
+++ b/few-shot-music-generation_amd/csrc/api_step.hip
@@ -29,6 +29,8 @@
     if (pass_reads_cs(h, B, true) && (rc = ensure_cs(h)) != FSMG_OK) return rc;
     if (h->tok_table_open && (rc = reset_tok_table(h)) != FSMG_OK) return rc;
     h->tok_table_open = true;
+    h->upd_follows = with_update;
+    h->gsq_ready = false;
     if ((rc = stage()) != FSMG_OK) return rc;
     const int n_sup = N * K, n_qry = N * Q;
     h->bucket0_recorded = false;
diff --git a/few-shot-music-generation_amd/csrc/api_update.hip b/few-shot-music-generation_amd/csrc/api_update.hip
--- a/few-shot-music-generation_amd/csrc/api_update.hip
+++ b/few-shot-music-generation_amd/csrc/api_update.hip
@@ -66,10 +66,15 @@
     const int64_t skip = slices ? round_up((int64_t)h->V1 * h->Ep, FLAT_ALIGN) : 0;
     const int64_t n = h->n_flat - skip;
     const int nb = sqnorm_blocks(n);
-    HIPCK(h, launch_sqnorm_partials(s, h->G + skip, n, h->partials));
+    const bool by_product = h->gsq_ready && h->gsq_skip == skip && (lean_bits(h) & 4);
+    h->gsq_ready = false;
+    h->gsq_used = by_product ? 1 : 0;
+    double* const partials = by_product ? h->gsq() : h->partials;
+    if (!by_product) HIPCK(h, launch_sqnorm_partials(s, h->G + skip, n, partials));
+    else if (h->gsq_prefix > 0) HIPCK(h, launch_sqnorm_partials(s, h->G + skip, std::min<int64_t>(n, (int64_t)h->gsq_prefix * SQNORM_CHUNK), partials));
     UpdateArgs a{};
     a.p = h->P; a.m = h->M; a.v = h->Vv; a.g = h->G; a.n = h->n_flat;
-    a.partials = h->partials; a.n_partials = nb; a.tail = h->G + h->n_flat; a.use_slices = slices ? 1 : 0;
+    a.partials = partials; a.n_partials = nb; a.tail = h->G + h->n_flat; a.use_slices = slices ? 1 : 0;
     a.grad_scale = grad_scale; a.lr = h->cfg.lr; a.n_decay = h->cfg.n_decay; a.clip = h->cfg.max_grad_norm;
     a.step = h->d_step; a.gnorm_out = h->d_gnorm; a.err_flag = h->d_err;
     const bool split = h->upd_split && h->eager_call && h->aux != nullptr && !h->timing && h->off_w > 0 && h->off_w < h->n_flat;
diff --git a/few-shot-music-generation_amd/csrc/elementwise.hip b/few-shot-music-generation_amd/csrc/elementwise.hip
--- a/few-shot-music-generation_amd/csrc/elementwise.hip
+++ b/few-shot-music-generation_amd/csrc/elementwise.hip
@@ -38,20 +38,20 @@
     if (blockIdx.x == 0 && threadIdx.x < (n & 3)) p[(n4 << 2) + threadIdx.x] = word;
 }
 
-constexpr int SQ_CHUNK = 256 * 16;
+constexpr int SQ_CHUNK = SQNORM_CHUNK;
+__device__ __forceinline__ void multi_fill_body(const MultiOp& o) {
+    if (o.cond != nullptr && *o.cond == 0) return;
+    uint32_t* p = (uint32_t*)o.dst;
+    const uint32_t word = o.word;
+    const long long n = o.n, n4 = n >> 2;
+    const uint4 w4 = make_uint4(word, word, word, word);
+    for (long long i = (long long)blockIdx.x * 256 + threadIdx.x; i < n4; i += (long long)gridDim.x * 256)
+        reinterpret_cast<uint4*>(p)[i] = w4;
+    if (blockIdx.x == 0 && threadIdx.x < (n & 3)) p[(n4 << 2) + threadIdx.x] = word;
+}
 __global__ __launch_bounds__(256) void k_multi_op(const MultiOps r) {
     const MultiOp& o = r.op[blockIdx.y];
-    if (o.kind == MULTI_FILL) {
-        if (o.cond != nullptr && *o.cond == 0) return;
-        uint32_t* p = (uint32_t*)o.dst;
-        const uint32_t word = o.word;
-        const long long n = o.n, n4 = n >> 2;
-        const uint4 w4 = make_uint4(word, word, word, word);
-        for (long long i = (long long)blockIdx.x * 256 + threadIdx.x; i < n4; i += (long long)gridDim.x * 256)
-            reinterpret_cast<uint4*>(p)[i] = w4;
-        if (blockIdx.x == 0 && threadIdx.x < (n & 3)) p[(n4 << 2) + threadIdx.x] = word;
-        return;
-    }
+    if (o.kind == MULTI_FILL) { multi_fill_body(o); return; }
     __shared__ double sh[4];
     if (o.kind == MULTI_MEAN) {
         if (blockIdx.x != 0) return;
@@ -163,9 +163,9 @@
     }
 }
 
-__global__ void k_token_prep(const int* __restrict__ support, int n_support, const int* __restrict__ query,
-                             int n_query, int T, int vocab, int start_word, int* __restrict__ X,
-                             int* __restrict__ Y, int* __restrict__ err_flag, int* __restrict__ tok_first, int* __restrict__ tok_count) {
+__device__ __forceinline__ void token_prep_body(const int* __restrict__ support, int n_support, const int* __restrict__ query,
+                                                int n_query, int T, int vocab, int start_word, int* __restrict__ X,
+                                                int* __restrict__ Y, int* __restrict__ err_flag, int* __restrict__ tok_first, int* __restrict__ tok_count) {
     __shared__ int s_key[512], s_cnt[512], s_min[512];
     const int B = n_support + n_query;
     const long long total = (long long)B * T;
@@ -209,6 +209,19 @@
     }
 }
 
+__global__ void k_token_prep(const int* __restrict__ support, int n_support, const int* __restrict__ query,
+                             int n_query, int T, int vocab, int start_word, int* __restrict__ X,
+                             int* __restrict__ Y, int* __restrict__ err_flag, int* __restrict__ tok_first, int* __restrict__ tok_count) {
+    token_prep_body(support, n_support, query, n_query, T, vocab, start_word, X, Y, err_flag, tok_first, tok_count);
+}
+__global__ __launch_bounds__(256) void k_token_prep_fills(const int* __restrict__ support, int n_support, const int* __restrict__ query,
+                                                         int n_query, int T, int vocab, int start_word, int* __restrict__ X,
+                                                         int* __restrict__ Y, int* __restrict__ err_flag, int* __restrict__ tok_first,
+                                                         int* __restrict__ tok_count, const MultiOps r) {
+    if (blockIdx.y != 0) { multi_fill_body(r.op[blockIdx.y - 1]); return; }
+    token_prep_body(support, n_support, query, n_query, T, vocab, start_word, X, Y, err_flag, tok_first, tok_count);
+}
+
 __global__ void k_gather_rows(const int* __restrict__ table, const int* __restrict__ idx, int n_rows, int T, int n_songs,
                               int* __restrict__ out, int* __restrict__ err_flag) {
     const long long total = (long long)n_rows * T;
@@ -360,11 +373,11 @@
     if (lane == 0) ce[row] = m + logf(s) - tgt_logit[row];
 }
 
-__global__ __launch_bounds__(256) void k_ce_finish(const float2* __restrict__ part, int nparts,
-                                                   const int* __restrict__ tgt, int rows, float inv_n, float* E, int ld,
-                                                   float* __restrict__ lse, float* __restrict__ ce, float* __restrict__ crow,
-                                                   const float* __restrict__ hs, float* __restrict__ hs_scaled, int hp,
-                                                   int* err_flag, unsigned long long* range_counter) {
+__device__ __forceinline__ void ce_finish_body(const float2* __restrict__ part, int nparts,
+                                               const int* __restrict__ tgt, int rows, float inv_n, float* E, int ld,
+                                               float* __restrict__ lse, float* __restrict__ ce, float* __restrict__ crow,
+                                               const float* __restrict__ hs, float* __restrict__ hs_scaled, int hp,
+                                               int* err_flag, unsigned long long* range_counter) {
     const int lane = threadIdx.x & 63, row = blockIdx.x * 4 + (threadIdx.x >> 6);
     if (blockIdx.x == 0 && threadIdx.x < 32) crow[rows + threadIdx.x] = 0.0f;
     if (row >= rows) return;
@@ -398,6 +411,22 @@
     }
 }
 
+__global__ __launch_bounds__(256) void k_ce_finish(const float2* __restrict__ part, int nparts,
+                                                   const int* __restrict__ tgt, int rows, float inv_n, float* E, int ld,
+                                                   float* __restrict__ lse, float* __restrict__ ce, float* __restrict__ crow,
+                                                   const float* __restrict__ hs, float* __restrict__ hs_scaled, int hp,
+                                                   int* err_flag, unsigned long long* range_counter) {
+    ce_finish_body(part, nparts, tgt, rows, inv_n, E, ld, lse, ce, crow, hs, hs_scaled, hp, err_flag, range_counter);
+}
+__global__ __launch_bounds__(256) void k_ce_finish_fills(const float2* __restrict__ part, int nparts,
+                                                         const int* __restrict__ tgt, int rows, float inv_n, float* E, int ld,
+                                                         float* __restrict__ lse, float* __restrict__ ce, float* __restrict__ crow,
+                                                         const float* __restrict__ hs, float* __restrict__ hs_scaled, int hp,
+                                                         int* err_flag, unsigned long long* range_counter, const MultiOps r) {
+    if (blockIdx.y != 0) { multi_fill_body(r.op[blockIdx.y - 1]); return; }
+    ce_finish_body(part, nparts, tgt, rows, inv_n, E, ld, lse, ce, crow, hs, hs_scaled, hp, err_flag, range_counter);
+}
+
 __global__ __launch_bounds__(256) void k_scale_rows(float* C, const float* __restrict__ row_scale, long long n4, int n_per_row4) {
     for (long long i = (long long)blockIdx.x * 256 + threadIdx.x; i < n4; i += (long long)gridDim.x * 256) {
         const float c = row_scale[i / n_per_row4];
@@ -457,9 +486,19 @@
 
 
 constexpr int EMBED_HEAVY = 48;
+__device__ __forceinline__ void sqnorm_chunk_body(const float* __restrict__ x, long long n, double* __restrict__ partials, int chunk);
 __global__ __launch_bounds__(256) void k_embed_grad_chunks(const int* __restrict__ X, int n, const float* __restrict__ dX, int Ep,
-                                                           float* __restrict__ part, const int* __restrict__ tok_count, const SumPartialsArgs sp) {
+                                                           float* __restrict__ part, const int* __restrict__ tok_count, const SumPartialsArgs sp,
+                                                           const SqChunksArgs sq) {
     if (blockIdx.x == (unsigned)((n + 255) / 256)) { sum_partials_body(sp.partials, sp.n, sp.dst, sp.flag_src, sp.ce, sp.ce_n, sp.loss_out); return; }
+    if (blockIdx.x > (unsigned)((n + 255) / 256)) {
+        int j = (int)blockIdx.x - (n + 255) / 256 - 1;
+        for (int k = 0; k < sq.nranges; ++k) {
+            if (j < sq.count[k]) { sqnorm_chunk_body(sq.x, sq.n, sq.partials, sq.first[k] + j); return; }
+            j -= sq.count[k];
+        }
+        return;
+    }
     __shared__ unsigned long long mask[4];
     __shared__ __attribute__((aligned(16))) float wsum[4][1024];
     const int base = blockIdx.x * 256, tid = threadIdx.x, lane = tid & 63, wave = tid >> 6, i = base + tid;
@@ -593,11 +632,99 @@
     if (tok_first != nullptr && tid == 0) { tok_first[tok] = 0x7FFFFFFF; tok_count[tok] = 0; }
 }
 
+template <int NC>
+__global__ __launch_bounds__(256) void k_embed_grad_wave(const int* __restrict__ X, int n, const float* __restrict__ dX,
+                                                         int Ep, float* __restrict__ dEmb, int* __restrict__ tok_first, int* __restrict__ tok_count,
+                                                         const float* __restrict__ part) {
+    const int lane = threadIdx.x & 63, r = blockIdx.x * 4 + (threadIdx.x >> 6);
+    if (r >= n) return;
+    const int x0 = (r + lane < n) ? X[r + lane] : -1;
+    const int tok = __shfl(x0, 0, 64);
+    const int nf4 = Ep >> 2;
+    const int first = tok_first[tok], want = tok_count[tok];
+    float4 v[NC];
+    {
+        const float4* src = reinterpret_cast<const float4*>(dX + (long long)r * Ep);
+#pragma unroll
+        for (int c = 0; c < NC; ++c) v[c] = (lane + 64 * c < nf4) ? src[lane + 64 * c] : make_float4(0.f, 0.f, 0.f, 0.f);
+    }
+    if (first != r) return;
+    float4 acc[NC];
+#pragma unroll
+    for (int c = 0; c < NC; ++c) acc[c] = make_float4(0.f, 0.f, 0.f, 0.f);
+    if (part != nullptr && want > EMBED_HEAVY) {
+        int found = 0;
+        for (int base = r & ~255; base < n && found < want; base += 256) {
+            int hit0 = -1;
+#pragma unroll
+            for (int g = 0; g < 4; ++g) {
+                const int i = base + 64 * g + lane;
+                const unsigned long long bal = __ballot((i < n) && (X[i] == tok));
+                found += __popcll(bal);
+                if (hit0 < 0 && bal) hit0 = 64 * g + __ffsll((long long)bal) - 1;
+            }
+            if (hit0 >= 0) {
+                const float4* src = reinterpret_cast<const float4*>(part + (long long)(base + hit0) * Ep);
+#pragma unroll
+                for (int c = 0; c < NC; ++c)
+                    if (lane + 64 * c < nf4) { const float4 w = src[lane + 64 * c]; acc[c].x += w.x; acc[c].y += w.y; acc[c].z += w.z; acc[c].w += w.w; }
+            }
+        }
+    } else {
+#pragma unroll
+        for (int c = 0; c < NC; ++c) { acc[c].x += v[c].x; acc[c].y += v[c].y; acc[c].z += v[c].z; acc[c].w += v[c].w; }
+        auto add_rows = [&](unsigned long long bal, int base) {
+            while (bal) {
+                int bits[4];
+#pragma unroll
+                for (int k = 0; k < 4; ++k) { bits[k] = bal ? __ffsll((long long)bal) - 1 : -1; bal &= bal - 1; }
+                float4 w[4][NC];
+#pragma unroll
+                for (int k = 0; k < 4; ++k) {
+                    const float4* src = reinterpret_cast<const float4*>(dX + (long long)(base + max(bits[k], 0)) * Ep);
+#pragma unroll
+                    for (int c = 0; c < NC; ++c) w[k][c] = (bits[k] >= 0 && lane + 64 * c < nf4) ? src[lane + 64 * c] : make_float4(0.f, 0.f, 0.f, 0.f);
+                }
+#pragma unroll
+                for (int k = 0; k < 4; ++k)
+                    if (bits[k] >= 0) {
+#pragma unroll
+                        for (int c = 0; c < NC; ++c) { acc[c].x += w[k][c].x; acc[c].y += w[k][c].y; acc[c].z += w[k][c].z; acc[c].w += w[k][c].w; }
+                    }
+            }
+        };
+        unsigned long long bal = __ballot(x0 == tok) & ~1ull;
+        int found = 1 + __popcll(bal);
+        add_rows(bal, r);
+        constexpr int EMBED_SCAN = 32;
+        for (int base = r + 64; base < n && found < want; base += 64 * EMBED_SCAN) {
+            int xv[EMBED_SCAN];
+#pragma unroll
+            for (int g = 0; g < EMBED_SCAN; ++g) xv[g] = (base + 64 * g + lane < n) ? X[base + 64 * g + lane] : -1;
+#pragma unroll
+            for (int g = 0; g < EMBED_SCAN; ++g) {
+                bal = __ballot(xv[g] == tok);
+                found += __popcll(bal);
+                add_rows(bal, base + 64 * g);
+            }
+        }
+    }
+    float4* dst = reinterpret_cast<float4*>(dEmb + (long long)tok * Ep);
+#pragma unroll
+    for (int c = 0; c < NC; ++c)
+        if (lane + 64 * c < nf4) dst[lane + 64 * c] = acc[c];
+    if (lane == 0) { tok_first[tok] = 0x7FFFFFFF; tok_count[tok] = 0; }
+}
+
+__device__ __forceinline__ void sqnorm_chunk_body(const float* __restrict__ x, long long n, double* __restrict__ partials, int chunk);
 __global__ __launch_bounds__(256) void k_sqnorm_partials(const float* __restrict__ x, long long n,
                                                          double* __restrict__ partials) {
+    sqnorm_chunk_body(x, n, partials, blockIdx.x);
+}
+__device__ __forceinline__ void sqnorm_chunk_body(const float* __restrict__ x, long long n, double* __restrict__ partials, int chunk) {
     __shared__ double sh[4];
     const int tid = threadIdx.x, lane = tid & 63, wave = tid >> 6;
-    const long long base = (long long)blockIdx.x * SQ_CHUNK;
+    const long long base = (long long)chunk * SQ_CHUNK;
     double s = 0.0;
 #pragma unroll
     for (int i = 0; i < 4; ++i) {
@@ -612,7 +739,7 @@
     s = wave_sum_d(s);
     if (lane == 0) sh[wave] = s;
     __syncthreads();
-    if (tid == 0) partials[blockIdx.x] = (sh[0] + sh[1]) + (sh[2] + sh[3]);
+    if (tid == 0) partials[chunk] = (sh[0] + sh[1]) + (sh[2] + sh[3]);
 }
 
 __global__ __launch_bounds__(256) void k_adam_update(const UpdateArgs a) {
@@ -803,12 +930,28 @@
 
 }
 
+static long long fill_blocks(const MultiOps& r) {
+    long long bx = 1;
+    for (int k = 0; k < r.count; ++k) {
+        if (r.op[k].kind != MULTI_FILL) return -1;
+        bx = std::max(bx, (r.op[k].n / 4 + 255) / 256);
+    }
+    return std::min<long long>(bx, 1024);
+}
+
 hipError_t launch_token_prep(hipStream_t s, const int* support, int n_support, const int* query, int n_query,
-                             int T, int vocab, int start_word, int* X, int* Y, int* err_flag, int* tok_first, int* tok_count) {
+                             int T, int vocab, int start_word, int* X, int* Y, int* err_flag, int* tok_first, int* tok_count, const MultiOps* fills) {
     const long long total = (long long)(n_support + n_query) * T;
-    if (total <= 0) return hipSuccess;
+    if (total <= 0) return fills != nullptr ? launch_multi_op(s, *fills) : hipSuccess;
     int blocks = (int)((total + 255) / 256);
     if (blocks > 1024) blocks = 1024;
+    if (fills != nullptr && fills->count > 0) {
+        const long long bx = fill_blocks(*fills);
+        if (bx < 0) return hipErrorInvalidValue;
+        hipLaunchKernelGGL(k_token_prep_fills, dim3((int)std::max<long long>(blocks, bx), 1 + fills->count), dim3(256), 0, s, support, n_support, query,
+                           n_query, T, vocab, start_word, X, Y, err_flag, tok_first, tok_count, *fills);
+        return hipGetLastError();
+    }
     hipLaunchKernelGGL(k_token_prep, dim3(blocks), dim3(256), 0, s, support, n_support, query, n_query, T, vocab,
                        start_word, X, Y, err_flag, tok_first, tok_count);
     return hipGetLastError();
@@ -837,9 +980,16 @@
 
 hipError_t launch_ce_finish(hipStream_t s, const float2* part, int nparts, const int* tgt, int rows, float inv_n,
                             float* E, int ld, float* lse, float* ce, float* crow, const float* hs, float* hs_scaled, int hp,
-                            int* err_flag, long long* range_counter) {
-    if (rows <= 0) return hipSuccess;
+                            int* err_flag, long long* range_counter, const MultiOps* fills) {
+    if (rows <= 0) return fills != nullptr ? launch_multi_op(s, *fills) : hipSuccess;
     if ((hp & 3) != 0 || err_flag == nullptr || range_counter == nullptr) return hipErrorInvalidValue;
+    if (fills != nullptr && fills->count > 0) {
+        const long long bx = fill_blocks(*fills);
+        if (bx < 0) return hipErrorInvalidValue;
+        hipLaunchKernelGGL(k_ce_finish_fills, dim3((int)std::max<long long>((rows + 3) / 4, bx), 1 + fills->count), dim3(256), 0, s, part, nparts, tgt, rows,
+                           inv_n, E, ld, lse, ce, crow, hs, hs_scaled, hp, err_flag, (unsigned long long*)range_counter, *fills);
+        return hipGetLastError();
+    }
     hipLaunchKernelGGL(k_ce_finish, dim3((rows + 3) / 4), dim3(256), 0, s, part, nparts, tgt, rows, inv_n, E, ld, lse, ce, crow,
                        hs, hs_scaled, hp, err_flag, (unsigned long long*)range_counter);
     return hipGetLastError();
@@ -860,17 +1010,27 @@
 }
 
 hipError_t launch_embed_grad(hipStream_t s, const int* X, int n, const float* dX, int Ep, float* dEmb, int* tok_first, int* tok_count, float* part,
-                             const SumPartialsArgs* sum) {
+                             const SumPartialsArgs* sum, bool wave_per_row, const SqChunksArgs* sq) {
     if (n <= 0) return sum != nullptr ? hipErrorInvalidValue : hipSuccess;
     if (Ep > 1024) return hipErrorInvalidValue;
     if (tok_first == nullptr || tok_count == nullptr || (Ep & 3) != 0 || ((uintptr_t)dX & 15) != 0) part = nullptr;
     if (part == nullptr && sum != nullptr) return hipErrorInvalidValue;
+    if (sq != nullptr && (sum == nullptr || sq->nranges < 0 || sq->nranges > SQ_MAX_RANGES)) return hipErrorInvalidValue;
     if (part != nullptr) {
         SumPartialsArgs sp{};
+        SqChunksArgs sc{};
         if (sum != nullptr) sp = *sum;
-        hipLaunchKernelGGL(k_embed_grad_chunks, dim3((n + 255) / 256 + (sum != nullptr ? 1 : 0)), dim3(256), 0, s, X, n, dX, Ep, part, tok_count, sp);
-    }
-    hipLaunchKernelGGL(k_embed_grad, dim3(n), dim3(256), 0, s, X, n, dX, Ep, dEmb, tok_first, tok_count, part);
+        if (sq != nullptr) sc = *sq;
+        hipLaunchKernelGGL(k_embed_grad_chunks, dim3((n + 255) / 256 + (sum != nullptr ? 1 : 0) + sc.total), dim3(256), 0, s, X, n, dX, Ep, part, tok_count, sp, sc);
+    }
+    if (wave_per_row && tok_first != nullptr && tok_count != nullptr && (Ep & 3) == 0 && (((uintptr_t)dX | (uintptr_t)dEmb | (uintptr_t)part) & 15) == 0) {
+        const dim3 grid((n + 3) / 4), block(256);
+        if (Ep <= 256) hipLaunchKernelGGL(k_embed_grad_wave<1>, grid, block, 0, s, X, n, dX, Ep, dEmb, tok_first, tok_count, part);
+        else if (Ep <= 512) hipLaunchKernelGGL(k_embed_grad_wave<2>, grid, block, 0, s, X, n, dX, Ep, dEmb, tok_first, tok_count, part);
+        else hipLaunchKernelGGL(k_embed_grad_wave<4>, grid, block, 0, s, X, n, dX, Ep, dEmb, tok_first, tok_count, part);
+    } else {
+        hipLaunchKernelGGL(k_embed_grad, dim3(n), dim3(256), 0, s, X, n, dX, Ep, dEmb, tok_first, tok_count, part);
+    }
     return hipGetLastError();
 }
 
diff --git a/few-shot-music-generation_amd/csrc/fsmg_kernels.h b/few-shot-music-generation_amd/csrc/fsmg_kernels.h
--- a/few-shot-music-generation_amd/csrc/fsmg_kernels.h
+++ b/few-shot-music-generation_amd/csrc/fsmg_kernels.h
@@ -176,7 +176,8 @@
 hipError_t launch_lstm_bwd_xcd(hipStream_t s, const LstmBwdXcdArgs& a);
 
 enum { MULTI_FILL = 0, MULTI_REDUCE = 1, MULTI_MEAN = 2 };
-constexpr int MULTI_MAX_OPS = 16;
+constexpr int MULTI_MAX_OPS = 24;
+constexpr int SQNORM_CHUNK = 256 * 16;
 struct MultiOp { int kind; void* dst; const void* src; long long n; long long stride; int nslab; uint32_t word; const int* cond; double* sq;
                  const float* row_scale; int row_len;  };
 struct MultiOps { MultiOp op[MULTI_MAX_OPS]; int count; };
@@ -186,20 +187,24 @@
 hipError_t launch_copy_words(hipStream_t s, void* dst, const void* src, long long n_words);
 hipError_t launch_fill32_if(hipStream_t s, const int* cond, void* p, uint32_t word, long long n_words);
 hipError_t launch_token_prep(hipStream_t s, const int* support, int n_support, const int* query, int n_query,
-                             int T, int vocab, int start_word, int* X, int* Y, int* err_flag, int* tok_first = nullptr, int* tok_count = nullptr);
+                             int T, int vocab, int start_word, int* X, int* Y, int* err_flag, int* tok_first = nullptr, int* tok_count = nullptr,
+                             const MultiOps* fills = nullptr);
 hipError_t launch_ce_rows(hipStream_t s, const float* logits, int ld, int rows, int n_vocab, const int* tgt,
                           float* lse, float* ce, float* dlogits, float inv_n);
 constexpr float CE_SUM_MIN = 8.0e-27f, CE_SUM_MAX = 1.0e30f, CE_TGT_MIN = 1.0e-30f;
 hipError_t launch_ce_finish(hipStream_t s, const float2* part, int nparts, const int* tgt, int rows, float inv_n,
                             float* E, int ld, float* lse, float* ce, float* crow, const float* hs, float* hs_scaled, int hp,
-                            int* err_flag, long long* range_counter);
+                            int* err_flag, long long* range_counter, const MultiOps* fills = nullptr);
 hipError_t launch_scale_rows(hipStream_t s, float* C, const float* row_scale, int M, int N);
 hipError_t launch_ce_combine(hipStream_t s, const float2* part, int nparts, const float* tgt_logit, int rows, float* ce);
 hipError_t launch_loss_reduce(hipStream_t s, const float* ce, int T, int B, int rows_per_group, int ngroups,
                               float* out);
 struct SumPartialsArgs { const double* partials; int n; float* dst; const int* flag_src; const float* ce; int ce_n; float* loss_out; };
+constexpr int SQ_MAX_RANGES = 8;
+struct SqChunksArgs { const float* x; long long n; double* partials; int nranges; int total; int first[SQ_MAX_RANGES]; int count[SQ_MAX_RANGES]; };
 hipError_t launch_embed_grad(hipStream_t s, const int* X, int n, const float* dX, int Ep, float* dEmb, int* tok_first = nullptr, int* tok_count = nullptr,
-                             float* part = nullptr, const SumPartialsArgs* sum = nullptr);
+                             float* part = nullptr, const SumPartialsArgs* sum = nullptr, bool wave_per_row = false,
+                             const SqChunksArgs* sq = nullptr);
 int sqnorm_blocks(long long n);
 hipError_t launch_sqnorm_partials(hipStream_t s, const float* x, long long n, double* partials);
 
diff --git a/few-shot-music-generation_amd/csrc/fsmg_model.h b/few-shot-music-generation_amd/csrc/fsmg_model.h
--- a/few-shot-music-generation_amd/csrc/fsmg_model.h
+++ b/few-shot-music-generation_amd/csrc/fsmg_model.h
@@ -176,6 +176,18 @@
     int xov_strikes = 0;
     bool xov_last = false;
     int xov_parts = 3;
+    int lean_step = 15;
+    bool upd_follows = false;
+    bool gsq_on = false;
+    bool gsq_ready = false;
+    int64_t gsq_skip = 0;
+    int gsq_prefix = 0;
+    int gsq_used = 0, gsq_extra = 0;
+    std::vector<char> gsq_cov;
+    double* gsq() const { return partials + (partials_cap - 8 - fsmg::sqnorm_blocks(n_flat)); }
+    bool prep_deferred = false;
+    int prep_nsup = 0, prep_nqry = 0;
+    bool bwd_fills_early = false;
     int* xov_prog = nullptr;
     static constexpr int XOV_CTL = 8192;
     int* xov_ctl = nullptr;
@@ -350,6 +362,19 @@
         if (n <= 0) return FSMG_OK;
         if (row_scale != nullptr && (sq != nullptr || row_len <= 0 || ((n | stride | (long long)row_len) & 3) != 0))
             return fail(h, FSMG_ERR_STATE, "internal: a row-scaled slab sum needs n, stride and row_len multiples of 4 and no squared-norm partials");
+        if (h->gsq_on && sq == nullptr && row_scale == nullptr && out >= h->G + h->gsq_skip && out + n <= h->G + h->n_flat) {
+            const long long o0 = out - (h->G + h->gsq_skip);
+            const long long a0 = (o0 + SQNORM_CHUNK - 1) / SQNORM_CHUNK * SQNORM_CHUNK, a1 = (o0 + n) / SQNORM_CHUNK * SQNORM_CHUNK;
+            if (a0 < a1) {
+                for (long long c = a0 / SQNORM_CHUNK; c < a1 / SQNORM_CHUNK; ++c) h->gsq_cov[(size_t)c] = 1;
+                h->gsq_on = false;
+                int rc = reduce(slabs, stride, nslab, out, a0 - o0);
+                if (rc == FSMG_OK) rc = reduce(slabs + (a0 - o0), stride, nslab, out + (a0 - o0), a1 - a0, h->gsq() + a0 / SQNORM_CHUNK);
+                if (rc == FSMG_OK) rc = reduce(slabs + (a1 - o0), stride, nslab, out + (a1 - o0), o0 + n - a1);
+                h->gsq_on = true;
+                return rc;
+            }
+        }
         const int rc = room(1); if (rc != FSMG_OK) return rc;
         MultiOp& o = r.op[r.count++];
         o = MultiOp{}; o.kind = MULTI_REDUCE; o.dst = out; o.src = slabs; o.stride = stride; o.nslab = nslab; o.n = n; o.sq = sq;
@@ -441,9 +466,12 @@
 int stage_tokens(fsmg_model* h, const int32_t* support, int n_sup, const int32_t* query, int n_qry, int on_device);
 int reset_tok_table(fsmg_model* h);
 int token_prep(fsmg_model* h, int n_sup, int n_qry, bool train = false);
+inline int lean_bits(const fsmg_model* h) { return h->timing ? 0 : h->lean_step; }
 enum { HEAD_LOSS = 0, HEAD_LOGITS = 1, HEAD_NONE = 2 };
 int forward(fsmg_model* h, int B, int rows_per_group, int ngroups, float* loss_out, bool want_dlogits, int head = HEAD_LOSS);
 GemmArgs dw_args(fsmg_model* h, int B);
+bool backward_xov(fsmg_model* h, int B, GemmArgs& gdw, int& dw_split);
+int backward_early_fills(fsmg_model* h, int B, OpBatch& fills, bool* added);
 int backward(fsmg_model* h, int B, int part = 0);
 int repack_recurrent_weights(fsmg_model* h, hipStream_t s, const StepIncArgs* inc, bool* inc_done);
 int repack_recurrent_weights(fsmg_model* h, hipStream_t s);
```
